# emdgroup/baybe

Measured on AMD Instinct MI355X. Metric: acquisition candidates scored/sec (1e6 discrete grid, n_train=512, qLogEI), higher is better.
Workload: dtype f64; 1 GPU; 1000000 x 20 discrete grid per GPU, n_train=512, Matern-5/2 ARD, qLogEI S=512, fixed-theta, top-8 to host; global_rows=1000000, parallelism=row-shard x1, collective=none

## Files before the change

### baybe_amd/_lib.py

```python

from __future__ import annotations

import ctypes as C
import os
from pathlib import Path

_LIB_NAME = "libbaybe_hip.so"
_lib = None

c_double_p = C.POINTER(C.c_double)
c_int64_p = C.POINTER(C.c_int64)


class HipUnavailableError(RuntimeError):
    """The HIP extension (or a HIP device) is not available; nothing else can run the path."""


class HipError(RuntimeError):
    """A libbaybe_hip call failed."""


class ModelDesc(C.Structure):

    _fields_ = [
# ... 33 lines not shown
    "bbh_create": (C.c_int, [C.c_int, C.POINTER(C.c_void_p)]),
    "bbh_destroy": (C.c_int, [C.c_void_p]),
    "bbh_last_error": (C.c_char_p, [C.c_void_p]),
    "bbh_set_stream": (C.c_int, [C.c_void_p, C.c_void_p]),
    "bbh_version": (C.c_int, []),
    "bbh_selftest": (C.c_int, [C.c_void_p]),
    "bbh_set_rff_weights": (C.c_int, [C.c_void_p, C.POINTER(C.c_double), C.c_int32, C.c_int32]),
    "bbh_set_model": (
        C.c_int,
        [C.c_void_p, C.POINTER(ModelDesc), C.c_int64, c_double_p, c_double_p, c_double_p, c_double_p],
    ),
    "bbh_set_model_ex": (
        C.c_int,
        [C.c_void_p, C.POINTER(ModelDesc), C.c_int64, c_double_p, c_double_p, c_double_p, c_double_p,
         C.POINTER(C.c_uint8), C.c_int, C.c_double, C.c_double],
    ),
    "bbh_set_slice_rows": (C.c_int, [C.c_void_p, C.c_int64]),
    "bbh_trim": (C.c_int, [C.c_void_p, C.c_int64]),
    "bbh_theta_len": (C.c_int64, [C.c_void_p]),
    "bbh_get_standardization": (C.c_int, [C.c_void_p, c_double_p, c_double_p]),
    "bbh_fit_value_grad": (C.c_int, [C.c_void_p, c_double_p, c_double_p, c_double_p]),
    "bbh_factorize": (C.c_int, [C.c_void_p, c_double_p, c_double_p]),
    "bbh_posterior": (C.c_int, [C.c_void_p, C.c_void_p, C.c_int64, C.c_int64, C.c_void_p, C.c_void_p]),
    "bbh_posterior_unfused": (C.c_int, [C.c_void_p, C.c_void_p, C.c_int64, C.c_int64, C.c_void_p, C.c_void_p]),
    "bbh_posterior_joint": (C.c_int, [C.c_void_p, c_double_p, C.c_int64, c_double_p, c_double_p]),
    "bbh_set_mean_columns": (C.c_int, [C.c_void_p, c_double_p, C.c_int64]),
    "bbh_posterior_columns": (C.c_int, [C.c_void_p, C.c_void_p, C.c_int64, C.c_int64, C.c_void_p]),
    "bbh_posterior_columns_sm": (C.c_int, [C.c_void_p, C.c_void_p, C.c_int64, C.c_int64, C.c_void_p]),
    "bbh_train_posterior_mean": (C.c_int, [C.c_void_p, c_double_p]),
    "bbh_qlogei_q1": (
        C.c_int,
        [C.c_void_p, C.c_void_p, C.c_void_p, C.c_int64, c_double_p, C.c_int64, C.c_double, C.c_double,
         C.c_void_p, C.c_void_p],
    ),
    "bbh_qlogei_q1_topk": (
        C.c_int,
        [C.c_void_p, C.c_void_p, C.c_void_p, C.c_int64, c_double_p, C.c_int64, C.c_double, C.c_double,
         C.c_void_p, C.c_void_p, C.c_int64, c_double_p, c_int64_p],
    ),
    "bbh_score_qlogei": (
        C.c_int,
        [C.c_void_p, C.c_void_p, C.c_int64, C.c_int64, c_double_p, C.c_int64, C.c_double, C.c_double, C.c_void_p,
         C.c_void_p, C.c_void_p, C.c_void_p],
    ),
    "bbh_pending_set": (C.c_int, [C.c_void_p, c_double_p, C.c_int64, c_double_p, c_double_p]),
    "bbh_cross_cov": (C.c_int, [C.c_void_p, C.c_void_p, C.c_int64, C.c_int64, C.c_void_p]),
    "bbh_qlogei_pending": (
        C.c_int,
        [C.c_void_p, C.c_void_p, C.c_void_p, C.c_void_p, C.c_int64, c_double_p, C.c_int64, C.c_double,
         C.c_double, C.c_void_p, C.c_void_p],
    ),
    "bbh_qlognehvi": (
        C.c_int,
        [C.c_void_p, C.c_int32, C.c_int64, C.POINTER(C.c_void_p), C.POINTER(C.c_void_p), c_double_p, c_double_p,
         C.c_int64, c_int64_p, c_double_p, c_double_p, C.c_void_p, C.c_void_p],
    ),
    "bbh_qlognehvi_sm": (
        C.c_int,
        [C.c_void_p, C.c_int32, C.c_int64, C.POINTER(C.c_void_p), C.POINTER(C.c_void_p), c_double_p, c_double_p,
         C.c_int64, c_int64_p, c_double_p, c_double_p, C.c_void_p, C.c_void_p],
    ),
    "bbh_qlogei_pending_big": (
        C.c_int,
        [C.c_void_p, C.c_void_p, C.c_void_p, C.c_void_p, C.c_int64, C.c_int64, c_double_p, c_double_p, c_double_p, C.c_int64,
         C.c_double, C.c_double, C.c_void_p, C.c_void_p],
    ),
    "bbh_mc_acq_q1": (
        C.c_int,
        [C.c_void_p, C.c_int32, C.c_void_p, C.c_void_p, C.c_int64, c_double_p, C.c_int64, C.c_double, C.c_double,
         C.c_double, C.c_void_p, C.c_void_p],
    ),
    "bbh_mc_acq_pending": (
        C.c_int,
        [C.c_void_p, C.c_int32, C.c_void_p, C.c_void_p, C.c_void_p, C.c_int64, c_double_p, C.c_int64, C.c_double,
         C.c_double, C.c_double, C.c_void_p, C.c_void_p],
    ),
    "bbh_mc_acq_obj_q1": (
        C.c_int,
        [C.c_void_p, C.c_int32, C.POINTER(ObjectiveProg), C.c_void_p, C.c_void_p, C.c_int64, c_double_p, C.c_int64, C.c_double,
         C.c_double, C.c_void_p, C.c_void_p],
    ),
    "bbh_mc_acq_obj_pending": (
        C.c_int,
        [C.c_void_p, C.c_int32, C.POINTER(ObjectiveProg), C.c_void_p, C.c_void_p, C.c_void_p, C.c_int64, C.c_int64, c_double_p,
         c_double_p, c_double_p, C.c_int64, C.c_double, C.c_double, C.c_void_p, C.c_void_p],
    ),
    "bbh_analytic_acq": (
        C.c_int,
        [C.c_void_p, C.c_int32, C.c_void_p, C.c_void_p, C.c_int64, C.c_double, C.c_double, C.c_double, C.c_int32,
         C.c_void_p, C.c_void_p],
    ),
    "bbh_pareto_frequency": (C.c_int, [C.c_void_p, c_double_p, C.c_int64, C.c_int64, C.c_int32, c_double_p, c_int64_p]),
    "bbh_pareto_frequency_dev": (C.c_int, [C.c_void_p, C.c_void_p, C.c_int64, C.c_int64, C.c_int32, c_double_p, c_int64_p]),
    "bbh_best_frequency_dev": (C.c_int, [C.c_void_p, C.c_void_p, C.c_int64, C.c_int64, c_int64_p]),
    "bbh_sample_best_dev": (C.c_int, [C.c_void_p, C.c_void_p, C.c_int64, C.c_int64, C.c_void_p]),
    "bbh_nei_q1": (C.c_int, [C.c_void_p, C.c_int32, C.c_void_p, C.c_void_p, C.c_int64, c_double_p, C.c_int64, C.c_void_p, C.c_double,
                             C.c_void_p, C.c_void_p]),
    "bbh_score_nei": (C.c_int, [C.c_void_p, C.c_int32, C.c_void_p, C.c_int64, C.c_int64, C.c_void_p, c_double_p, C.c_int64, C.c_void_p,
                                C.c_double, C.c_void_p, C.c_void_p]),
    "bbh_scalarized_best_dev": (C.c_int, [C.c_void_p, C.c_void_p, C.c_int64, C.c_int64, C.c_int32, c_double_p, c_double_p, c_double_p,
                                          C.c_void_p]),
    "bbh_scalarized_best_frequency_dev": (C.c_int, [C.c_void_p, C.c_void_p, C.c_int64, C.c_int64, C.c_int32, c_double_p, c_double_p,
                                                    c_double_p, c_int64_p]),
    "bbh_nparego_q1": (
        C.c_int,
        [C.c_void_p, C.c_int32, C.c_int64, C.POINTER(C.c_void_p), C.POINTER(C.c_void_p), c_double_p, C.c_void_p, C.c_int64,
         c_double_p, c_double_p, c_double_p, C.c_void_p, C.c_void_p, C.c_void_p],
    ),
    "bbh_qnehvi_cells": (
        C.c_int,
        [C.c_void_p, C.c_int32, C.c_int64, C.POINTER(C.c_void_p), C.POINTER(C.c_void_p), c_double_p, c_double_p,
         C.c_int64, C.c_void_p, C.c_void_p],
    ),
    "bbh_qnehvi_sm": (
        C.c_int,
        [C.c_void_p, C.c_int32, C.c_int64, C.POINTER(C.c_void_p), C.POINTER(C.c_void_p), c_double_p, c_double_p,
         C.c_int64, c_int64_p, c_double_p, c_double_p, C.c_void_p, C.c_void_p],
    ),
    "bbh_nehvi_samples": (C.c_int, [C.c_void_p, c_double_p, C.c_int64, C.c_int64, C.c_double, C.c_int32, C.c_int32, C.c_void_p, C.c_int32]),
    "bbh_nehvi_samples_dev": (C.c_int, [C.c_void_p, C.c_void_p, C.c_int64, C.c_void_p, C.c_int64, C.c_int64, C.c_double, C.c_int32, C.c_int32,
                                        C.c_void_p, C.c_int32]),
    "bbh_cells_build_dev": (C.c_int, [C.c_void_p, C.c_void_p, C.c_int64, C.c_int64, C.c_int32, c_double_p, c_int64_p, c_int64_p]),
    "bbh_cells_read_dev": (C.c_int, [C.c_void_p, c_int64_p, c_double_p, c_double_p]),
    "bbh_qlognehvi_cells": (
        C.c_int,
        [C.c_void_p, C.c_int32, C.c_int64, C.POINTER(C.c_void_p), C.POINTER(C.c_void_p), c_double_p, c_double_p,
         C.c_int64, C.c_void_p, C.c_void_p],
    ),
    "bbh_cells_create": (C.c_int, [c_double_p, C.c_int64, C.c_int64, C.c_int32, c_double_p, C.POINTER(C.c_void_p), c_int64_p]),
    "bbh_cells_get": (C.c_int, [C.c_void_p, c_int64_p, c_double_p, c_double_p]),
    "bbh_cells_destroy": (C.c_int, [C.c_void_p]),
    "bbh_sobol_scramble": (C.c_int, [c_int64_p, c_int64_p, C.c_int64]),
    "bbh_sobol_draw": (C.c_int, [c_int64_p, c_int64_p, C.c_int64, C.c_int64, c_double_p]),
    "bbh_sobol_normal": (C.c_int, [c_int64_p, C.c_uint64, C.c_int64, C.c_int64, c_double_p]),
    "bbh_sobol_normal_dev": (C.c_int, [C.c_void_p, c_int64_p, C.c_uint64, C.c_int64, C.c_int64, C.c_void_p]),
    "bbh_content_key": (C.c_uint64, [C.POINTER(C.c_void_p), c_int64_p, C.c_int32, C.c_int32]),
    "bbh_argmax": (C.c_int, [C.c_void_p, C.c_void_p, C.c_int64, c_double_p, c_int64_p]),
    "bbh_topk": (C.c_int, [C.c_void_p, C.c_void_p, C.c_int64, C.c_int64, c_double_p, c_int64_p]),
    "bbh_fps_prepare": (C.c_int, [C.c_void_p, C.c_void_p, C.c_int64, C.c_int32, C.c_int64, c_double_p, c_double_p, C.c_void_p, C.c_int64,
                                  C.c_void_p, C.c_int64]),
    "bbh_fps_farthest_pair": (C.c_int, [C.c_void_p, C.c_void_p, C.c_int64, C.c_int32, C.c_int64, C.c_void_p, c_double_p, c_int64_p,
                                        c_int64_p]),
    "bbh_fps_greedy": (C.c_int, [C.c_void_p, C.c_void_p, C.c_int64, C.c_int32, C.c_int64, C.c_void_p, c_int64_p, C.c_int64, C.c_int64,
                                 C.c_int64, c_int64_p, c_double_p, c_int64_p]),
    "bbh_comm_unique_id": (C.c_int, [C.c_void_p, C.c_int64]),
    "bbh_comm_init": (C.c_int, [C.c_void_p, C.c_int32, C.c_int32, C.c_void_p, C.c_int64]),
    "bbh_comm_destroy": (C.c_int, [C.c_void_p]),
    "bbh_allgather_topk": (C.c_int, [C.c_void_p, C.c_void_p, C.c_int64, C.c_int64, C.c_int64, c_double_p, c_int64_p]),
    "bbh_allgather_argmax": (
        C.c_int,
        [C.c_void_p, C.c_void_p, C.c_int64, C.c_int64, C.c_void_p, C.c_int64, c_double_p, c_int64_p, c_double_p],
    ),
    "bbh_last_posterior_form": (C.c_int, [C.c_void_p]),
    "bbh_last_nei_form": (C.c_int, [C.c_void_p]),
    "bbh_last_fit_form": (C.c_int, [C.c_void_p]),
    "bbh_timing_enable": (C.c_int, [C.c_void_p, C.c_int]),
    "bbh_timing_read": (C.c_int, [C.c_void_p, c_double_p, c_int64_p, C.c_int]),
    "bbh_timing_read_family": (C.c_int, [C.c_void_p, C.c_int32, c_double_p, c_int64_p, C.c_int]),
    "bbh_flow_trace_read": (C.c_int, [C.c_void_p, C.c_void_p, C.c_void_p, C.c_int]),
    "bbh_tiles_trace_read": (C.c_int, [C.c_void_p, C.c_void_p, C.c_int]),
}


def library_path() -> Path:
    env = os.environ.get("BAYBE_AMD_LIB")
    return Path(env) if env else Path(__file__).resolve().parent / _LIB_NAME


def load_library():
    global _lib
    if _lib is not None:
        return _lib
    import torch

    path = library_path()
    if not path.exists():
        raise HipUnavailableError(
            f"{path} not found: build it with `python -c 'import __graft_entry__ as g; g.build()'` "
            f"or `make -C baybe_amd/csrc`. There is no CPU fallback for this path."
        )
    try:
        lib = C.CDLL(str(path))
    except OSError as ex:
        raise HipUnavailableError(f"cannot load {path}: {ex}") from ex
    for name, (restype, argtypes) in SIGNATURES.items():
        fn = getattr(lib, name)
        fn.restype = restype
        fn.argtypes = argtypes
    _lib = lib
    return lib


def is_available() -> bool:
    try:
        lib = load_library()
    except (HipUnavailableError, AttributeError):
        return False
    h = C.c_void_p()
    rc = lib.bbh_create(0, C.byref(h))
    if rc != 0:
        return False
    lib.bbh_destroy(h)
    return True
```

### baybe_amd/csrc/bbh_api.hip

```cpp
#include <math.h>
#include <stdlib.h>
#include <string.h>

#include <algorithm>
#include <map>
#include <mutex>

#include "bbh_common.h"

static const char* kNoHandle = "bbh: null handle";

extern "C" int bbh_version(void) { return 100; }

static bbh_switches bbh_read_switches() {
  enum how { NOT, IS, SET, INT, MB };
  typedef bbh_switches S;
  static const struct {
    const char* name;
    how parse;
    char c;
    bool S::*flag;
    int S::*num;
  } table[] = {
      {"BBH_PIPELINE", NOT, '0', &S::use_pipeline, nullptr},
      {"BBH_MEAN_VALU", NOT, '0', &S::use_mean_valu, nullptr},
      {"BBH_KVCACHE", NOT, '0', &S::use_kvcache, nullptr},
      {"BBH_KV_GLOBAL", NOT, '0', nullptr, &S::kv_global_mode},
      {"BBH_KV_LDS", INT, 0, nullptr, &S::kv_lds_blocks},
      {"BBH_COOP", INT, 0, nullptr, &S::coop_mode},
      {"BBH_COOP_SMALL", NOT, '0', &S::coop_small, nullptr},
      {"BBH_COOPG_CROSS", NOT, '0', &S::coopg_cross_on, nullptr},
      {"BBH_SMALL", NOT, '0', &S::small_on, nullptr},
      {"BBH_SMALL_FORCE", IS, '1', &S::small_force, nullptr},
      {"BBH_COLUMNS_COOP", NOT, '0', &S::columns_coop, nullptr},
      {"BBH_COLUMNS_NT", INT, 0, nullptr, &S::columns_nt},
      {"BBH_PENDING_LDS", NOT, '0', &S::pending_lds_form, nullptr},
      {"BBH_PENDING_SLICES", INT, 0, nullptr, &S::pending_slices},
      {"BBH_QBIG_WS_MB", MB, 0, nullptr, &S::qbig_ws_mb},
      {"BBH_Q1_SLICED", NOT, '0', &S::q1_sliced, nullptr},
      {"BBH_NEHVI_LOG", IS, '1', &S::nehvi_log, nullptr},
      {"BBH_NEHVI_SLICES", INT, 0, nullptr, &S::nehvi_slices},
      {"BBH_NEHVI_PK", NOT, '0', &S::nehvi_pk, nullptr},
      {"BBH_NEI_FUSED", NOT, '0', &S::nei_fused, nullptr},
      {"BBH_SELECT", NOT, '0', &S::select_on, nullptr},
      {"BBH_SELECT_MAPPED", NOT, '0', &S::select_mapped, nullptr},
      {"BBH_FIT_GRAPH", NOT, '0', &S::fit_graph_mode, nullptr},
      {"BBH_FIT_OVERLAP", NOT, '0', &S::fit_overlap, nullptr},
      {"BBH_FIT_SMALL", NOT, '0', &S::fit_small, nullptr},
      {"BBH_FIT_FLOW", INT, 0, nullptr, &S::fit_flow},
      {"BBH_FLOW_SPIN", INT, 0, nullptr, &S::flow_spin_limit},
      {"BBH_FIT_POST1", NOT, '0', &S::fit_post1, nullptr},
      {"BBH_FIT_TAIL1", NOT, '0', &S::fit_tail1, nullptr},
      {"BBH_POTRF_TILES", NOT, '0', &S::potrf_tiles, nullptr},
      {"BBH_POTRF_REG", NOT, '0', &S::potrf_register_form, nullptr},
      {"BBH_TILE_SPIN", INT, 0, nullptr, &S::tile_spin_limit},
      {"BBH_TILE_ACQ", IS, '0', &S::tile_d_sc1, nullptr},
      {"BBH_TILE_WT", NOT, '0', &S::tile_wt, nullptr},
      {"BBH_TILE_MT", NOT, '0', &S::tile_mt, nullptr},
      {"BBH_TILE_MT", IS, 'p', &S::tile_mt_partial, nullptr},
      {"BBH_TILE_GRAM", NOT, '0', &S::tile_gram, nullptr},
      {"BBH_TILE_GRAM_THETA", IS, 'c', &S::tile_gram_theta_copy, nullptr},
      {"BBH_SETMODEL_UPLOAD", IS, 'c', &S::setmodel_upload_copy, nullptr},
      {"BBH_SETMODEL_SYNC", NOT, '0', &S::setmodel_sync, nullptr},
      {"BBH_SETMODEL_SYNC", IS, 'p', &S::setmodel_sync_poll, nullptr},
      {"BBH_SETMODEL_TRACE", SET, 0, &S::setmodel_trace, nullptr},
      {"BBH_SETMODEL_TRACE", IS, '2', &S::setmodel_trace_quiet, nullptr},
      {"BBH_FIT_TRACE", SET, 0, &S::fit_trace, nullptr},
      {"BBH_TILE_TRACE", SET, 0, &S::tile_trace, nullptr},
      {"BBH_FLOW_TRACE", SET, 0, &S::flow_trace, nullptr},
      {"BBH_TILE_STAMPS", SET, 0, &S::tile_stamps, nullptr},
  };
  bbh_switches sw;
  for (const auto& row : table) {
    const char* e = getenv(row.name);
    if (!e) continue;
    long long v = 1;
    if (row.parse == NOT) v = e[0] != row.c;
    if (row.parse == IS) v = e[0] == row.c;
    if (row.parse == INT) v = atoi(e);
    if (row.parse == MB) v = std::min<long long>(std::max(1LL, atoll(e)), INT_MAX);
    if (row.flag) sw.*row.flag = v != 0;
    if (row.num) sw.*row.num = (int)v;
  }
  return sw;
}

hipError_t bbh_allow_lds(int device, const void* kernel, size_t bytes) {
  if (bytes <= BBH_LDS_DEFAULT_LIMIT) return hipSuccess;
  hipError_t e = device < 0 ? hipGetDevice(&device) : hipSuccess;
  if (e != hipSuccess) return e;
  static std::mutex mu;
  static std::map<std::pair<const void*, int>, size_t> granted;
  std::lock_guard<std::mutex> lock(mu);
  size_t& have = granted[{kernel, device}];
  if (bytes <= have) return hipSuccess;
  e = hipFuncSetAttribute(kernel, hipFuncAttributeMaxDynamicSharedMemorySize, (int)bytes);
  if (e == hipSuccess) have = bytes;
  return e;
}

extern "C" int bbh_create(int device_id, bbh_handle** out) {
  if (!out) return -1;
  *out = nullptr;
  int count = 0;
  if (hipGetDeviceCount(&count) != hipSuccess || count <= 0) return -10;
  if (device_id < 0 || device_id >= count) return -11;
  if (hipSetDevice(device_id) != hipSuccess) return -12;
  bbh_handle* h = new bbh_handle();
  h->device = device_id;
  {
    int cus = 0;
    if (hipDeviceGetAttribute(&cus, hipDeviceAttributeMultiprocessorCount, device_id) == hipSuccess && cus > 0) h->num_cu = cus;
  }
  {
    int v = 0;
    if (hipDeviceGetAttribute(&v, hipDeviceAttributeMaxSharedMemoryPerBlock, device_id) == hipSuccess && v > 0) h->lds_per_block = (size_t)v;
  }
  h->sw = bbh_read_switches();
  *out = h;
  return 0;
}

extern "C" int bbh_destroy(bbh_handle* h) {
  if (!h) return -1;
  hipSetDevice(h->device);
  if (h->stream)
    hipStreamSynchronize(h->stream);
  else
    hipDeviceSynchronize();
  for (auto& sp : h->pending_events) {
    hipEventDestroy(sp.e0);
    hipEventDestroy(sp.e1);
  }
  bbh_comm_destroy(h);
  bbh_select_destroy(h);
  bbh_nehvi_destroy(h);
  bbh_sobol_destroy(h);
  bbh_fps_destroy(h);
  bbh_flow_destroy(h);
  bbh_free_model_public(h);
  if (h->d_ws) hipFree(h->d_ws);
  if (h->fit_stream) {
    hipStreamSynchronize(h->fit_stream);
    hipStreamDestroy(h->fit_stream);
  }
  if (h->side_stream) {
    hipStreamSynchronize(h->side_stream);
    hipStreamDestroy(h->side_stream);
  }
  for (auto& e : h->side_events)
    if (e) hipEventDestroy(e);
  if (h->d_rstream) hipFree(h->d_rstream);
  if (h->d_rsmall) hipFree(h->d_rsmall);
  if (h->d_tileflags) hipFree(h->d_tileflags);
  if (h->d_kvcache) hipFree(h->d_kvcache);
  if (h->d_slab_flags) hipFree(h->d_slab_flags);
  if (h->d_z) hipFree(h->d_z);
  if (h->h_zstage) hipHostFree(h->h_zstage);
  if (h->z_evt) hipEventDestroy(h->z_evt);
  if (h->d_red) hipFree(h->d_red);
  if (h->d_redi) hipFree(h->d_redi);
  delete h;
  return 0;
}

extern "C" const char* bbh_last_error(bbh_handle* h) { return h ? h->err.c_str() : kNoHandle; }

extern "C" int bbh_set_stream(bbh_handle* h, void* hip_stream) {
  if (!h) return -1;
  h->stream = (hipStream_t)hip_stream;
  return 0;
}

__global__ void bbh_selftest_kernel(const double* A, const double* B, double* C) {
  const int l = threadIdx.x;
  d4 acc = {0.0, 0.0, 0.0, 0.0};
  for (int ks = 0; ks < 2; ks++) {
    const double a = A[(l & 15) * 8 + 4 * ks + (l >> 4)];
    const double b = B[(4 * ks + (l >> 4)) * 16 + (l & 15)];
    acc = mfma_f64(a, b, acc);
  }
  for (int r = 0; r < 4; r++) C[((l >> 4) + 4 * r) * 16 + (l & 15)] = acc[r];
}

extern "C" int bbh_selftest(bbh_handle* h) {
  if (!h) return -1;
  BBH_HIP_TRY(h, hipSetDevice(h->device));
  double hA[16 * 8], hB[8 * 16], hC[256], ref[256];
  for (int i = 0; i < 16; i++)
    for (int k = 0; k < 8; k++) hA[i * 8 + k] = (double)(3 * i + 7 * k + 1) - 0.5 * (double)(i * k);
  for (int k = 0; k < 8; k++)
    for (int j = 0; j < 16; j++) hB[k * 16 + j] = (double)(5 * k - 2 * j) + 0.25 * (double)(k * j + j);
  for (int i = 0; i < 16; i++)
    for (int j = 0; j < 16; j++) {
      double s = 0.0;
      for (int k = 0; k < 8; k++) s += hA[i * 8 + k] * hB[k * 16 + j];
      ref[i * 16 + j] = s;
    }
  int rc = bbh_ensure_ws(h, sizeof(double) * 1024);
  if (rc) return rc;
  double* dA = h->d_ws;
  double* dB = dA + 128;
  double* dC = dB + 128;
  BBH_HIP_TRY(h, hipMemcpyAsync(dA, hA, sizeof(hA), hipMemcpyHostToDevice, h->stream));
  BBH_HIP_TRY(h, hipMemcpyAsync(dB, hB, sizeof(hB), hipMemcpyHostToDevice, h->stream));
  hipLaunchKernelGGL(bbh_selftest_kernel, dim3(1), dim3(64), 0, h->stream, dA, dB, dC);
  BBH_HIP_TRY(h, hipMemcpyAsync(hC, dC, sizeof(hC), hipMemcpyDeviceToHost, h->stream));
  BBH_HIP_TRY(h, hipStreamSynchronize(h->stream));
  for (int e = 0; e < 256; e++)
    if (fabs(hC[e] - ref[e]) > 1e-9 * (1.0 + fabs(ref[e]))) {
      h->err = "bbh_selftest: v_mfma_f64_16x16x4_f64 fragment layout mismatch at element " + std::to_string(e);
      return -20;
    }
  return 0;
}

static int check_post_args(bbh_handle* h, const double* X_dev, int64_t N, int64_t ldx) {
  if (!h->factorized) {
    h->err = "posterior requested before bbh_factorize";
    return -1;
  }
  if (N < 0 || (N > 0 && !X_dev) || ldx < h->desc.d) {
    h->err = "posterior: bad arguments (need ldx >= d)";
    return -1;
  }
  if (h->dn > 126) {
    h->err = "fused posterior supports at most 126 numerical columns";
    return -1;
  }
  return 0;
}

extern "C" int bbh_posterior(bbh_handle* h, const double* X_dev, int64_t N, int64_t ldx, double* mean_dev,
                             double* var_dev) {
  if (!h) return -1;
  int rc = check_post_args(h, X_dev, N, ldx);
  if (rc) return rc;
  BBH_HIP_TRY(h, hipSetDevice(h->device));
  return bbh_launch_fused(h, X_dev, N, ldx, mean_dev, var_dev, nullptr, true);
}

extern "C" int bbh_posterior_unfused(bbh_handle* h, const double* X_dev, int64_t N, int64_t ldx, double* mean_dev,
                                     double* var_dev) {
  if (!h) return -1;
  int rc = check_post_args(h, X_dev, N, ldx);
  if (rc) return rc;
  BBH_HIP_TRY(h, hipSetDevice(h->device));
  return bbh_launch_unfused(h, X_dev, N, ldx, mean_dev, var_dev);
}

extern "C" int bbh_cross_cov(bbh_handle* h, const double* X_dev, int64_t N, int64_t ldx, double* cross_dev) {
  if (!h) return -1;
  int rc = check_post_args(h, X_dev, N, ldx);
  if (rc) return rc;
  if (h->p < 1 || !cross_dev) {
    h->err = "bbh_cross_cov: no pending points set";
    return -1;
  }
  BBH_HIP_TRY(h, hipSetDevice(h->device));
  return bbh_launch_fused(h, X_dev, N, ldx, nullptr, nullptr, cross_dev, false);
}

extern "C" int bbh_train_posterior_mean(bbh_handle* h, double* mean_host) {
  if (!h) return -1;
  if (!h->factorized || !mean_host) {
    h->err = "bbh_train_posterior_mean: model not factorised";
    return -1;
  }
  BBH_HIP_TRY(h, hipSetDevice(h->device));
  const int64_t n = h->n, d = h->desc.d;
  int rc = 0;
  double* own = nullptr;
  if (bbh_materialised_only(h))
    BBH_HIP_TRY(h, hipMalloc((void**)&own, sizeof(double) * (size_t)(n * d + n)));
  else if ((rc = bbh_ensure_ws(h, sizeof(double) * (size_t)(n * d + n))))
    return rc;
  double* dX = own ? own : h->d_ws;
  double* dm = dX + n * d;
  hipError_t e = hipMemcpyAsync(dX, h->xraw_host.data(), sizeof(double) * n * d, hipMemcpyHostToDevice, h->stream);
  if (e == hipSuccess) rc = bbh_launch_fused(h, dX, n, d, dm, nullptr, nullptr, false);
  if (e == hipSuccess && !rc) e = hipMemcpyAsync(mean_host, dm, sizeof(double) * n, hipMemcpyDeviceToHost, h->stream);
  if (e == hipSuccess) e = hipStreamSynchronize(h->stream);
  if (own) hipFree(own);
  if (rc) return rc;
  BBH_HIP_TRY(h, e);
  return 0;
}

extern "C" int bbh_set_slice_rows(bbh_handle* h, int64_t rows) {
  if (!h || rows < 0) return -1;
  h->slice_rows = rows;
  return 0;
}

extern "C" int bbh_trim(bbh_handle* h, int64_t keep_bytes) {
  if (!h || keep_bytes < 0) return -1;
  BBH_HIP_TRY(h, hipSetDevice(h->device));
  BBH_HIP_TRY(h, hipStreamSynchronize(h->stream));
  bbh_fps_reset(h);
  if (h->d_ws && h->ws_bytes > (size_t)keep_bytes) {
    hipFree(h->d_ws);
    h->d_ws = nullptr;
    h->ws_bytes = 0;
  }
  if (h->d_kvcache && h->kvcache_bytes > (size_t)keep_bytes) {
    hipFree(h->d_kvcache);
    h->d_kvcache = nullptr;
    h->kvcache_bytes = 0;
  }
  if (h->have_model && sizeof(double) * (size_t)h->np * (size_t)h->np * 6 > (size_t)keep_bytes) bbh_free_model_public(h);
  return 0;
}

extern "C" int bbh_last_posterior_form(bbh_handle* h) { return h ? h->last_form : -1; }
extern "C" int bbh_last_fit_form(bbh_handle* h) { return h ? h->last_fit_form : -1; }

extern "C" int bbh_timing_enable(bbh_handle* h, int enable) {
  if (!h) return -1;
  h->timing = enable < 0 ? 0 : enable;
  return 0;
}

extern "C" int bbh_timing_read_family(bbh_handle* h, int32_t family, double* ms_total, int64_t* launches, int reset) {
  if (!h) return -1;
  if (family < 0 || family >= BBH_TIMED_FAMILIES) {
    h->err = "bbh_timing_read_family: unknown kernel family";
    return -1;
  }
  BBH_HIP_TRY(h, hipSetDevice(h->device));
  for (auto& sp : h->pending_events) {
    BBH_HIP_TRY(h, hipEventSynchronize(sp.e1));
    float ms = 0.f;
    BBH_HIP_TRY(h, hipEventElapsedTime(&ms, sp.e0, sp.e1));
    h->timed_ms[sp.family] += (double)ms;
    h->timed_launches[sp.family] += 1;
    hipEventDestroy(sp.e0);
    hipEventDestroy(sp.e1);
  }
  h->pending_events.clear();
  if (ms_total) *ms_total = h->timed_ms[family];
  if (launches) *launches = h->timed_launches[family];
  if (reset) {
    h->timed_ms[family] = 0.0;
    h->timed_launches[family] = 0;
  }
  return 0;
}

extern "C" int bbh_timing_read(bbh_handle* h, double* fused_ms_total, int64_t* fused_launches, int reset) {
  return bbh_timing_read_family(h, BBH_TIMED_POSTERIOR, fused_ms_total, fused_launches, reset);
}
```

### baybe_amd/csrc/bbh_common.h

```cpp
#pragma once

#include <hip/hip_runtime.h>
#include <limits.h>
#include <stdint.h>

#include <string>
#include <vector>

#include "../../include/baybe_hip.h"

typedef double d4 __attribute__((ext_vector_type(4)));

#define BBH_WAVE 64
#define BBH_TB 16
#define BBH_PAD 64
#define BBH_MEANCOLS 16
#define BBH_SQRT3 1.7320508075688772
#define BBH_SQRT5 2.23606797749979

__device__ __forceinline__ d4 mfma_f64(double a, double b, d4 c) {
  return __builtin_amdgcn_mfma_f64_16x16x4f64(a, b, c, 0, 0, 0);
}

#define BBH_HIP_TRY(h, expr)                                                              \
  do {                                                                                    \
    hipError_t _e = (expr);                                                               \
    if (_e != hipSuccess) {                                                               \
      (h)->err = std::string(#expr) + ": " + hipGetErrorString(_e);                       \
      return -2;                                                                          \
    }                                                                                     \
  } while (0)

#define BBH_MAX_FACTORS 4
struct bbh_kern_spec {
  int F;
  int combine;
  int grp[BBH_MAX_FACTORS];
  int kind[BBH_MAX_FACTORS];
  int ls_off[BBH_MAX_FACTORS];
  int fos_off;
  int use_os;
  int jb;
  int alpha_off;
  int per_off;
};
__host__ __device__ inline double bbh_powi(double x, int n) {
  double acc = 1.0;
  for (int i = 0; i < n; i++) acc *= x;
  return acc;
}
__host__ __device__ inline double bbh_piecewise(int q, int jb, double r2, bool want_g) {
  const double r = sqrt(r2 > 1e-30 ? r2 : 1e-30);
  if (!(r < 1.0)) return 0.0;
  const double j = (double)(jb + q), u = 1.0 - r;
  if (!want_g) {
    double P = 1.0;
    if (q == 1) P = fma(j + 1.0, r, 1.0);
    if (q == 2) P = fma(fma((j * j + 4.0 * j + 3.0) / 3.0, r, j + 2.0), r, 1.0);
    if (q == 3)
      P = fma(fma(fma((j * j * j + 9.0 * j * j + 23.0 * j + 15.0) / 15.0, r, (6.0 * j * j + 36.0 * j + 45.0) / 15.0), r, j + 3.0), r, 1.0);
    return bbh_powi(u, jb + 2 * q) * P;
  }
  const double m = bbh_powi(u, jb + 2 * q - 1);
  if (q == 0) return r2 > 1e-30 ? j * m / r : 0.0;
  if (q == 1) return (j + 1.0) * (j + 2.0) * m;
  if (q == 2) return (j + 3.0) * (j + 4.0) * fma(j + 1.0, r, 1.0) / 3.0 * m;
  return (j + 5.0) * (j + 6.0) * fma(fma(j * j + 4.0 * j + 3.0, r, 3.0 * j + 6.0), r, 3.0) / 15.0 * m;
}
#define BBH_KIND_IS_DOT(kind) ((kind) >= BBH_KERNEL_LINEAR && (kind) <= BBH_KERNEL_POLY4)
#define BBH_KIND_IS_POLY(kind) ((kind) >= BBH_KERNEL_POLY1 && (kind) <= BBH_KERNEL_POLY4)
#define BBH_KIND_HAS_ALPHA(kind) ((kind) == BBH_KERNEL_RQ || BBH_KIND_IS_POLY(kind))
__host__ __device__ __forceinline__ double bbh_metric_term(int kind, double xa, double xb, double invw) {
  if (BBH_KIND_IS_DOT(kind)) return (xa * invw) * (xb * invw);
  const double df = (xa - xb) * invw;
  return df * df;
}
__host__ __device__ __forceinline__ double bbh_metric_term_f(const bbh_kern_spec& ks, const double* theta, int f, int j, int dn,
                                                             double xa, double xb, double invw) {
  if (ks.kind[f] == BBH_KERNEL_PERIODIC) {
    const double sn = sin(M_PI * (xa - xb) / theta[ks.per_off + f * dn + j]);
    return sn * sn * invw;
  }
  return bbh_metric_term(ks.kind[f], xa, xb, invw);
}
__host__ __device__ __attribute__((noinline)) inline double bbh_kbase(int kind, double r2, int jb, double alpha = 1.0) {
  if (kind == BBH_KERNEL_LINEAR) return r2;
  if (BBH_KIND_IS_POLY(kind)) return bbh_powi(r2 + alpha, kind - BBH_KERNEL_POLY1 + 1);
  if (kind == BBH_KERNEL_PERIODIC) return exp(-2.0 * r2);
  if (kind == BBH_KERNEL_RBF) return exp(-0.5 * r2);
  if (kind == BBH_KERNEL_RQ) return exp(-alpha * log1p(r2 / (2.0 * alpha)));
  if (kind >= BBH_KERNEL_PIECEWISE0 && kind <= BBH_KERNEL_PIECEWISE3) return bbh_piecewise(kind - BBH_KERNEL_PIECEWISE0, jb, r2, false);
  const double r = sqrt(r2);
  if (kind == BBH_KERNEL_MATERN52) return (1.0 + BBH_SQRT5 * r + (5.0 / 3.0) * r2) * exp(-BBH_SQRT5 * r);
  if (kind == BBH_KERNEL_MATERN32) return (1.0 + BBH_SQRT3 * r) * exp(-BBH_SQRT3 * r);
  return exp(-r);
}
__device__ __forceinline__ double bbh_gfun(int kind, double r2, int jb, double alpha) {
  if (kind == BBH_KERNEL_LINEAR) return -2.0;
  if (BBH_KIND_IS_POLY(kind)) return -2.0 * (double)(kind - BBH_KERNEL_POLY1 + 1) * bbh_powi(r2 + alpha, kind - BBH_KERNEL_POLY1);
  if (kind == BBH_KERNEL_PERIODIC) return 2.0 * exp(-2.0 * r2);
  if (kind == BBH_KERNEL_RBF) return exp(-0.5 * r2);
  if (kind == BBH_KERNEL_RQ) return exp(-(alpha + 1.0) * log1p(r2 / (2.0 * alpha)));
  if (kind >= BBH_KERNEL_PIECEWISE0) return bbh_piecewise(kind - BBH_KERNEL_PIECEWISE0, jb, r2, true);
  const double r = sqrt(r2);
  if (kind == BBH_KERNEL_MATERN52) return (5.0 / 3.0) * (1.0 + BBH_SQRT5 * r) * exp(-BBH_SQRT5 * r);
  if (kind == BBH_KERNEL_MATERN32) return 3.0 * exp(-BBH_SQRT3 * r);
  return r > 0.0 ? exp(-r) / r : 0.0;
}


template <class GRP>
__host__ __device__ __forceinline__ double bbh_combine(int F, int combine, const GRP& grp, const double* u) {
  if (combine == 0) {
    double acc = 1.0;
#pragma unroll
    for (int f = 0; f < BBH_MAX_FACTORS; f++)
      if (f < F) acc *= u[f];
    return acc;
  }
  if (combine == 1) {
    double acc = 0.0;
#pragma unroll
    for (int f = 0; f < BBH_MAX_FACTORS; f++)
      if (f < F) acc += u[f];
    return acc;
  }
  double acc = 0.0;
#pragma unroll
  for (int g = 0; g < BBH_MAX_FACTORS; g++) {
    double term = 1.0;
    bool used = false;
#pragma unroll
    for (int f = 0; f < BBH_MAX_FACTORS; f++)
      if (f < F && grp[f] == g) {
        term *= u[f];
        used = true;
      }
    if (used) acc += term;
  }
  return acc;
}
template <class GRP>
__host__ __device__ __forceinline__ double bbh_combine_weight(int F, int combine, const GRP& grp, const double* u, int f) {
  if (combine == 1) return 1.0;
  double w = 1.0;
#pragma unroll
  for (int g = 0; g < BBH_MAX_FACTORS; g++)
    if (g < F && g != f && (combine == 0 || grp[g] == grp[f])) w *= u[g];
  return w;
}
__device__ __forceinline__ double bbh_kcomp(const bbh_kern_spec& ks, const double* __restrict__ theta,
                                            const double (&r2)[BBH_MAX_FACTORS]) {
  if (ks.F <= 1) return bbh_kbase(ks.kind[0], r2[0], ks.jb, ks.alpha_off >= 0 ? theta[ks.alpha_off] : 1.0);
  double u[BBH_MAX_FACTORS] = {1.0, 1.0, 1.0, 1.0};
#pragma unroll
  for (int f = 0; f < BBH_MAX_FACTORS; f++)
    if (f < ks.F)
      u[f] = theta[ks.fos_off + f] * bbh_kbase(ks.kind[f], r2[f], ks.jb, ks.alpha_off >= 0 ? theta[ks.alpha_off + f] : 1.0);
  return bbh_combine(ks.F, ks.combine, ks.grp, u);
}

struct bbh_switches {
  bool use_pipeline = true;
  bool use_mean_valu = true;
  bool use_kvcache = true;
  int kv_global_mode = -1;
  int kv_lds_blocks = -1;
  int coop_mode = 1;
  bool coop_small = true;
  bool coopg_cross_on = true;
  bool small_on = true;
  bool small_force = false;
  bool columns_coop = true;
  int columns_nt = 2;
  bool pending_lds_form = false;
  int pending_slices = INT_MIN;
  int qbig_ws_mb = 0;
  bool q1_sliced = true;
  bool nehvi_log = false;
  int nehvi_slices = INT_MIN;
  bool nehvi_pk = true;
  bool nei_fused = true;
  bool select_on = true;
  bool select_mapped = true;
  bool fit_graph_mode = false;
  bool fit_overlap = true;
  bool fit_small = true;
  int fit_flow = 1;
  int flow_spin_limit = 1 << 17;
  bool fit_post1 = true;
  bool fit_tail1 = true;
  bool potrf_tiles = true;
  bool potrf_register_form = false;
  int tile_spin_limit = 1 << 17;
  bool tile_d_sc1 = false;
  bool tile_wt = true;
  bool tile_mt = true;
  bool tile_mt_partial = false;
  bool tile_gram = true;
  bool tile_gram_theta_copy = false;
  bool setmodel_upload_copy = false;
  bool setmodel_sync = true;
  bool setmodel_sync_poll = false;
  bool setmodel_trace = false;
  bool setmodel_trace_quiet = false;
  bool fit_trace = false;
  bool tile_trace = false;
  bool flow_trace = false;
  bool tile_stamps = false;
};

struct bbh_handle {
  int device = 0;
  bbh_switches sw;
  hipStream_t stream = nullptr;
  std::string err;

  bbh_model_desc desc{};
  std::string model_sig;
  bool have_model = false;
  bool factorized = false;
  int64_t n = 0;
  int64_t np = 0;
  int64_t nb = 0;
  int dn = 0;
  int kd = 0;
  int T = 1;
  bool hadamard = false;
  int F = 1;
  std::vector<int> numcol;
  std::vector<double> lo, hi;
  double ybar = 0.0, ysd = 1.0;
  std::vector<double> theta;
  std::vector<double> ystd_host;
  std::vector<double> xn_host;
  std::vector<int> task_host;
  std::vector<double> xcenter;

  double* d_xnT = nullptr;
  int* d_task = nullptr;
  double* d_nmask = nullptr;
  double* d_pendT = nullptr;
  double* d_colA = nullptr;
  int64_t colA_elems = 0;
  std::vector<double> nmask_host;
  double* d_ystd = nullptr;
  double* d_theta = nullptr;
  double* d_K = nullptr;
  double* d_X = nullptr;
  double* d_M = nullptr;
  double* d_Mpart = nullptr;
  double* d_Q = nullptr;
  double* d_Q2 = nullptr;
  double* d_D = nullptr;
  double* d_tmp = nullptr;
  double* d_r = nullptr;
  double* d_t = nullptr;
  double* d_alpha = nullptr;
  double* d_u = nullptr;
  double* d_w = nullptr;
  double* d_q = nullptr;
  double* d_partial = nullptr;
  double* d_out = nullptr;
  int* d_info = nullptr;
  double* d_trainfrag = nullptr;
  double* d_rfrag = nullptr;
  double* d_meanB = nullptr;
  double* d_sclofs = nullptr;
  int* d_numcol = nullptr;
  double* d_tasktbl = nullptr;
  int* d_taskext = nullptr;
  int64_t rfrag_elems = 0;
  int64_t* d_pass_off = nullptr;
  int* d_pass_w = nullptr;
  int npass = 0;
  int pass_w_last = 0;
  double* d_kvcache = nullptr;
  size_t kvcache_bytes = 0;
  int* d_slab_flags = nullptr;
  size_t lds_per_block = 65536;
  int num_cu = 256;
  int wmax = 16;
  hipStream_t side_stream = nullptr;
  hipStream_t fit_stream = nullptr;
  bool fit_small_ready = false, fit_small_failed = false;
  bool tiles_ready = false, tiles_gave_up = false;
  int tile_spin_limit_set = -1;
  int tiles_per_device = 0;
  int* d_tileflags = nullptr;
  int tile_epoch = 0;
  hipGraphExec_t fit_exec = nullptr;
  bool fit_graph_failed = false;
  double *pin_theta = nullptr, *pin_out = nullptr;
  int* pin_info = nullptr;
  hipEvent_t side_events[2] = {nullptr, nullptr};
  bool coop_ready = false;
  bool coopg_ready = false;
  double* d_trainfrag_f = nullptr;
  double* d_sclofs_f = nullptr;
  int64_t tf_f_elems = 0;
  bool coop2_ready = false;
  double* d_rstream = nullptr;
  int64_t rstream_frags = 0;
  int coop_g0 = 0;
  int last_form = -1;
  int last_fit_form = -1;
  int last_nei_form = -1;
  int64_t nb_ext = 0;
  int p = 0;
  std::vector<double> pend_host;
  std::vector<double> pend_mean;
  std::vector<double> pend_cov;
  std::vector<double> xraw_host;
  double* d_beta = nullptr;
  double* d_colfrag = nullptr;
  int64_t colfrag_elems = 0;
  int64_t ncols = 0;
  const double* fuse_qz = nullptr;
  int fuse_S = 0;
  double fuse_best_f = 0.0, fuse_sign = 1.0;
  const uint8_t* fuse_alive = nullptr;
  double* fuse_scores = nullptr;
  double* d_ws = nullptr;
  size_t ws_bytes = 0;
  double* d_z = nullptr;
  size_t z_bytes = 0;
  double* h_zstage = nullptr;
  size_t zstage_bytes = 0;
  hipEvent_t z_evt = nullptr;
  double* d_red = nullptr;
  int64_t* d_redi = nullptr;
  void* comm_state = nullptr;
  double* d_rsmall = nullptr;
  int small_nb = 0;
  int64_t slice_rows = 0;
  void* flow_state = nullptr;
  bool flow_gave_up = false;
  bool skip_x_memset = false;
  bool flow_in_flight = false;
  long long* d_tiledbg = nullptr;
  int tiledbg_n = 0;
  int tiles_did_mt = 0;
  int tiles_mt_asked = 0;
  bool potrf_tiles_ran = false;
  bool info_clean = false;
  void* rff_state = nullptr;
  std::vector<double> rff_w_host;
  int rff_w_dn = 0, rff_w_D = 0;
  void* nehvi_state = nullptr;
  void* select_state = nullptr;
  void* sobol_state = nullptr;
  void* fps_state = nullptr;
  int timing = 0;
  hipEvent_t ev0 = nullptr, ev1 = nullptr;
  double timed_ms[BBH_TIMED_FAMILIES] = {};
  int64_t timed_launches[BBH_TIMED_FAMILIES] = {};
  struct TimedSpan {
    hipEvent_t e0, e1;
    int family;
  };
  std::vector<TimedSpan> pending_events;
};

struct bbh_timed_scope {
  bbh_handle* h;
  hipEvent_t e0 = nullptr, e1 = nullptr;
  int family;
  bbh_timed_scope(bbh_handle* h_, int family_, bool wanted = true) : h(h_), family(family_) {
    if ((h->timing == 1 || ((h->timing >> 1) >> family_ & 1)) && wanted) {
      hipEventCreate(&e0);
      hipEventCreate(&e1);
      hipEventRecord(e0, h->stream);
    }
  }
  ~bbh_timed_scope() {
    if (e0) {
      hipEventRecord(e1, h->stream);
      h->pending_events.push_back({e0, e1, family});
    }
  }
};

inline int64_t bbh_round_up(int64_t x, int64_t m) { return (x + m - 1) / m * m; }

#define BBH_LDS_DEFAULT_LIMIT ((size_t)48 * 1024)
__attribute__((visibility("hidden"))) hipError_t bbh_allow_lds(int device, const void* kernel, size_t bytes);

struct bbh_nehvi_state {
  int64_t S = 0, total = 0, cap = 0;
  int m = 0;
  double* d_slots = nullptr;
  size_t slot_bytes = 0;
  double* d_pack = nullptr;
  size_t pack_bytes = 0;
  int* d_cnt = nullptr;
  int64_t cnt_cap = 0;
  double* d_ref = nullptr;
  int64_t* h_status = nullptr;
  const int64_t* off() const { return (const int64_t*)d_pack; }
  const double* lo() const { return d_pack + (S + 1); }
  const double* ll() const { return lo() + S * cap * m; }
  const double* len() const { return ll() + S * cap * m; }
};

void bbh_gemm(hipStream_t s, bool transA, bool transB, int64_t M, int64_t N, int64_t K, double alpha,
              const double* A, int64_t lda, int64_t strideA, const double* B, int64_t ldb,
              int64_t strideB, double beta, double* C, int64_t ldc, int64_t strideC, int batch);
void bbh_potrf_trtri(bbh_handle* h);
bool bbh_potrf_trtri_from_inputs(bbh_handle* h, const double* theta_any, const double* theta_host, const void* mt_args = nullptr);
void bbh_potrf_tiles_mark_unusable(int device);
void bbh_ensure_side_stream(bbh_handle* h);
void bbh_matvec(hipStream_t s, const double* A, int64_t lda, int64_t rows, int64_t cols,
                const double* x, double* y);
void bbh_matvec_t(hipStream_t s, const double* A, int64_t lda, int64_t rows, int64_t cols,
                  const double* x, double* y);

int bbh_upload_theta(bbh_handle* h, const double* theta_host);
void bbh_launch_gram(bbh_handle* h, double jitter, double jitter_latent);
bool bbh_fit_small_launch(bbh_handle* h, double jitter, const double* theta_dev, double* out_dev, int* info_dev);
bbh_kern_spec bbh_kern_spec_of(const bbh_handle* h);
int bbh_hadamard_offset(const bbh_handle* h);
double bbh_prior_base(const bbh_handle* h);
bool bbh_materialised_only(const bbh_handle* h);
bool bbh_has_dot_kind(const bbh_handle* h);
int bbh_launch_unfused_ext(bbh_handle* h, const double* X_dev, int64_t N, int64_t ldx, double* mean_dev, double* var_dev,
                           double* cross_dev);

int bbh_pack_operands(bbh_handle* h);
int bbh_launch_fused(bbh_handle* h, const double* X_dev, int64_t N, int64_t ldx, double* mean_dev,
                     double* var_dev, double* cross_dev, bool with_var);
int bbh_launch_unfused(bbh_handle* h, const double* X_dev, int64_t N, int64_t ldx, double* mean_dev,
                       double* var_dev);

int bbh_ensure_ws(bbh_handle* h, size_t bytes);
void* bbh_stage_pinned(bbh_handle* h, size_t bytes);
int bbh_stage_done(bbh_handle* h);
int bbh_upload_z(bbh_handle* h, const double* z_host, size_t count);
void bbh_select_destroy(bbh_handle* h);
void bbh_nehvi_destroy(bbh_handle* h);
void bbh_sobol_destroy(bbh_handle* h);
void bbh_fps_destroy(bbh_handle* h);
void bbh_fps_reset(bbh_handle* h);
void bbh_flow_destroy(bbh_handle* h);
bool bbh_fit_flow_launch(bbh_handle* h, const double* theta_dev, double* out_dev, int* info_dev, bool tail_only, const double* theta_host = nullptr,
                         bool split = false, int skip_mt = 0, bool prepare_only = false);
bool bbh_fit_flow_mt_args(bbh_handle* h, void* pd_mt_args_out);
bool bbh_fit_flow_eligible(bbh_handle* h);
void bbh_fit_flow_reset(bbh_handle* h);
void bbh_free_model_public(bbh_handle* h);
inline bool bbh_is_rff(const bbh_handle* h) { return h->desc.kernel_kind == BBH_KERNEL_RFF; }
int bbh_rff_setup(bbh_handle* h);
int bbh_rff_fit_enqueue(bbh_handle* h);
int bbh_rff_factorize(bbh_handle* h);
int bbh_rff_posterior_launch(bbh_handle* h, const double* X_dev, int64_t N, int64_t ldx, double* mean_dev, double* var_dev, double* cross_dev);
int bbh_rff_pending_set(bbh_handle* h, const double* Xpend_host, int64_t p, double* mean_p_host, double* cov_pp_host);
int bbh_rff_posterior_joint(bbh_handle* h, const double* Xq_host, int64_t q, double* mean_host, double* cov_host);
void bbh_rff_destroy(bbh_handle* h);
// ... 1 lines not shown
```

### baybe_amd/csrc/bbh_coop.h

```cpp
#pragma once
#define BBH_CANDREG 1
#include "bbh_fused.h"

#define BBH_COOP_ROUNDS 8
#define BBH_COOP_KV_TILE (2 * 4 * 256)
#ifndef BBH_COOP_WAVES
#define BBH_COOP_WAVES 2
#endif
#ifndef BBH_COOP_PAIRS
#define BBH_COOP_PAIRS 4
#endif
#ifndef BBH_COOP_ABLATE_BARRIER
#define BBH_COOP_ABLATE_BARRIER 0
#endif
#ifndef BBH_COOP_ABLATE_MEM
#define BBH_COOP_ABLATE_MEM 0
#endif
#ifndef BBH_COOP_ABLATE_PRO
#define BBH_COOP_ABLATE_PRO 0
#endif
#ifndef BBH_COOP_ABLATE_LOADS
#define BBH_COOP_ABLATE_LOADS 0
#endif
#ifndef BBH_COOP_ABLATE_CHAIN
#define BBH_COOP_ABLATE_CHAIN 0
#endif
#ifndef BBH_COOP_ABLATE_KV
#define BBH_COOP_ABLATE_KV 0
#endif

typedef double d2 __attribute__((ext_vector_type(2)));
template <int IMM>
__device__ __forceinline__ void coop_gload2(d2& dst, const double* sbase, unsigned voff) {
  static_assert(IMM >= 0 && IMM + 16 <= 4096, "13-bit signed immediate offset");
  asm volatile("global_load_dwordx4 %0, %1, %2 offset:%3" : "=v"(dst) : "v"(voff), "s"(sbase), "n"(IMM));
}
template <int N>
__device__ __forceinline__ void coop_vmwait2(d2& slot) {
  asm volatile("s_waitcnt vmcnt(%1)" : "+v"(slot) : "n"(N));
}
template <int IMM>
__device__ __forceinline__ void coop_gload(double& dst, const double* sbase, unsigned voff) {
  static_assert(IMM >= 0 && IMM < 4096, "13-bit signed immediate offset");
  asm volatile("global_load_dwordx2 %0, %1, %2 offset:%3" : "=v"(dst) : "v"(voff), "s"(sbase), "n"(IMM));
}
template <int N>
__device__ __forceinline__ void coop_vmwait(double& slot) {
  asm volatile("s_waitcnt vmcnt(%1)" : "+v"(slot) : "n"(N));
}

struct CoopArgs {
  FusedArgs f;
  const double* rstream;
  int64_t frags;
  int g0;
};

__host__ __device__ constexpr int coop_frags_before(int G) { return 16 * (G * BBH_COOP_ROUNDS - (G * (G - 1)) / 2); }

template <int G, int KD, int KVF, bool PRODUCE, int NT, bool OPEN = false>
__device__ __forceinline__ void coop_group(const WaveCtx (&c)[NT], const double* rs, const double* tfn, const bbh_lds_double* kv_cur,
                                           bbh_lds_double* kv_mine_next, const bbh_lds_double* alpha_next, int tbn, int cw,
                                           d4 (&acc)[NT][BBH_COOP_ROUNDS], d2 (&ring)[BBH_COOP_PAIRS], double (&accm)[NT]) {
  constexpr int NP = BBH_COOP_PAIRS;
  constexpr int CNT = BBH_COOP_ROUNDS - G;
  constexpr int FULL = CNT - 1;
  constexpr int TOT = 16 * CNT;
  constexpr int REM = OPEN ? (1 << 20) : coop_frags_before(BBH_COOP_ROUNDS) - coop_frags_before(G + 1);
  constexpr int HOSTS = 12 * FULL;
  constexpr int STEPS = NT * BBH_KV_STEPS;
  const unsigned lane8 = (unsigned)c[0].l * 8u, lane16 = (unsigned)c[0].l * 16u;
  double tfv[KD];
  d4 dsa[NT], dsb[NT];
  KvState<BBH_KV_NU> P;
  double kv[NT][4], kvx[NT][4], kvn[NT][4], alv[4];
  if constexpr (PRODUCE) {
    static_for<0, KD>([&](auto kc) __attribute__((always_inline)) {
      constexpr int k = decltype(kc)::value;
      coop_gload<(k % 8) * 512>(tfv[k], tfn + (k / 8) * 512, lane8);
    });
  }
#pragma unroll
  for (int t = 0; t < NT; t++)
#pragma unroll
    for (int r = 0; r < 4; r++) kv[t][r] = kv_cur[t * BBH_COOP_KV_TILE + r * 64];
  __builtin_amdgcn_sched_barrier(0);
  static_for<0, 4>([&](auto ic) __attribute__((always_inline)) {
    constexpr int i = decltype(ic)::value;
    if constexpr (i < 3) {
#pragma unroll
      for (int t = 0; t < NT; t++)
#pragma unroll
        for (int r = 0; r < 4; r++) kvx[t][r] = kv_cur[t * BBH_COOP_KV_TILE + (i + 1) * 256 + r * 64];
    } else if constexpr (PRODUCE) {
#pragma unroll
      for (int r = 0; r < 4; r++) alv[r] = alpha_next[4 * r];
    }
    static_for<0, 4>([&](auto rc) __attribute__((always_inline)) {
      constexpr int r = decltype(rc)::value;
      static_for<0, CNT>([&](auto sc) __attribute__((always_inline)) {
        constexpr int s = decltype(sc)::value;
        constexpr int f = (i * 4 + r) * CNT + s;
        constexpr int pr = f / 2;
        if constexpr (f % 2 == 0 && !BBH_COOP_ABLATE_LOADS) {
          constexpr int BEHIND = ((TOT + REM) / 2 - 1 - pr) < (NP - 1) ? ((TOT + REM) / 2 - 1 - pr) : (NP - 1);
          coop_vmwait2<BEHIND + ((PRODUCE && pr < NP) ? KD : 0)>(ring[pr % NP]);
        }
#if BBH_COOP_ABLATE_CHAIN
        static_for<0, NT>([&](auto tc_) __attribute__((always_inline)) {
          constexpr int t = decltype(tc_)::value;
          if constexpr (s == 0) {
            if (cw >= i) acc[t][f % 8] = mfma_f64(kv[t][r], ring[pr % NP][f % 2], acc[t][f % 8]);
          } else {
            acc[t][f % 8] = mfma_f64(kv[t][r], ring[pr % NP][f % 2], acc[t][f % 8]);
          }
        });
#else
        static_for<0, NT>([&](auto tc_) __attribute__((always_inline)) {
          constexpr int t = decltype(tc_)::value;
          if constexpr (s == 0) {
            if (cw >= i) acc[t][G] = mfma_f64(kv[t][r], ring[pr % NP][f % 2], acc[t][G]);
          } else {
            acc[t][G + s] = mfma_f64(kv[t][r], ring[pr % NP][f % 2], acc[t][G + s]);
          }
        });
#endif
        if constexpr (f % 2 == 1 && 2 * (pr + NP) < TOT + REM && !BBH_COOP_ABLATE_LOADS) {
          constexpr int np = pr + NP;
          coop_gload2<(np % 4) * 1024>(ring[pr % NP], BBH_COOP_ABLATE_MEM ? rs : rs + (np / 4) * 512, lane16);
        }
        if constexpr (PRODUCE && i >= 1 && s >= 1 && !BBH_COOP_ABLATE_KV) {
          constexpr int m = ((i - 1) * 4 + r) * FULL + (s - 1);
          static_for<(m * STEPS) / HOSTS, ((m + 1) * STEPS) / HOSTS>([&](auto st) __attribute__((always_inline)) {
            constexpr int tile = decltype(st)::value / BBH_KV_STEPS, micro = decltype(st)::value % BBH_KV_STEPS;
            kv_micro<KVF, BBH_KV_NU, micro>(P, c[tile], tbn, 0, dsa[tile], dsb[tile], kvn[tile]);
          });
        }
        __builtin_amdgcn_sched_barrier(0);
      });
      if constexpr (PRODUCE && i == 0 && r == 3) {
        coop_vmwait<NP>(tfv[KD - 1]);
        __builtin_amdgcn_sched_barrier(0);
        if constexpr (!BBH_COOP_ABLATE_KV) {
          static_for<0, NT>([&](auto tc_) __attribute__((always_inline)) {
            constexpr int t = decltype(tc_)::value;
            kvp_dist<KD>(c[t], tfv, dsa[t], dsb[t]);
          });
        }
      }
    });
    if constexpr (i < 3) {
#pragma unroll
      for (int t = 0; t < NT; t++)
#pragma unroll
        for (int r = 0; r < 4; r++) kv[t][r] = kvx[t][r];
    }
  });
  if constexpr (PRODUCE) {
#pragma unroll
    for (int t = 0; t < NT; t++)
#pragma unroll
      for (int r = 0; r < 4; r++) {
        if constexpr (BBH_COOP_ABLATE_KV) kvn[t][r] = tfv[r];
        kv_mine_next[t * BBH_COOP_KV_TILE + r * 64] = kvn[t][r];
        accm[t] = fma(kvn[t][r], alv[r], accm[t]);
      }
  }
}

template <int KD, int KVF, int NT, int GMIN = 0>
__global__ __launch_bounds__(256, (GMIN >= 6 ? 5 : GMIN >= 4 ? 4 : BBH_COOP_WAVES)) void bbh_coop_posterior_kernel(const CoopArgs ca) {
  const FusedArgs& a = ca.f;
  extern __shared__ __attribute__((aligned(16))) double s_mem[];
  const int l = threadIdx.x & 63, w = __builtin_amdgcn_readfirstlane(threadIdx.x >> 6);
  const int cnd = l & 15, q = l >> 4;
  double* s_alpha = s_mem;
  double* s_kv = s_alpha + 16 * a.nb;
  double* s_red = s_kv + NT * BBH_COOP_KV_TILE;
  const int64_t tile0 = (int64_t)blockIdx.x * (16 * NT);

  WaveCtx c[NT];
  int tcs[NT];
  int xcol[KD];
  double xval[NT][KD], xscl[KD], xofs[KD];
  const double* xr[NT];
  double tfv0[KD];
  kvp_load<KD>(a.trainfrag + l, w, tfv0);
#pragma unroll
  for (int t = 0; t < NT; t++) {
    const int64_t row = (tile0 + 16 * t + cnd < a.N) ? tile0 + 16 * t + cnd : a.N - 1;
    xr[t] = a.X + row * a.ldx;
  }
  if (a.numcol_identity) {
#pragma unroll
    for (int k = 0; k < KD; k++) xcol[k] = (4 * k + q < a.dn) ? 4 * k + q : a.dn - 1;
  } else {
#pragma unroll
    for (int k = 0; k < KD; k++) xcol[k] = a.numcol[(4 * k + q < a.dn) ? 4 * k + q : a.dn - 1];
  }
#pragma unroll
  for (int k = 0; k < KD; k++) {
    const int dimc = (4 * k + q < a.dn) ? 4 * k + q : a.dn - 1;
#pragma unroll
    for (int t = 0; t < NT; t++) xval[t][k] = xr[t][xcol[k]];
    xscl[k] = a.scl[dimc];
    xofs[k] = a.ofs[dimc];
  }
  if (!(BBH_COOP_ABLATE_PRO & 1))
    for (int s = threadIdx.x; s < 16 * a.nb; s += 256) s_alpha[s] = a.meanB[(int64_t)s * 16];
#pragma unroll
  for (int t = 0; t < NT; t++) {
    double nbsum = 0.0;
#pragma unroll
    for (int k = 0; k < KD; k++) {
      const int dim = 4 * k + q;
      double v = 0.0;
      if (dim < a.dn) {
        v = (BBH_COOP_ABLATE_PRO & 2) ? 0.01 * (double)(dim + cnd) : fma(xval[t][k], xscl[k], xofs[k]);
        nbsum = fma(v, v, nbsum);
      }
      c[t].cf[k] = v;
    }
    nbsum += __shfl_xor(nbsum, 16, 64);
    nbsum += __shfl_xor(nbsum, 32, 64);
#pragma unroll
    for (int k = 0; k < KD; k++) {
      if (4 * k + q == a.dn) c[t].cf[k] = 1.0;
      if (4 * k + q == a.dn + 1) c[t].cf[k] = nbsum;
    }
    int tc = 0;
    if constexpr ((KVF & 1) != 0) {
      if (a.task_col >= 0) {
        tc = (int)xr[t][a.task_col];
        tc = tc < 0 ? 0 : (tc >= a.T ? a.T - 1 : tc);
      }
    }
    tcs[t] = tc;
    c[t].tf = a.trainfrag + l;
    c[t].candl = nullptr;
    c[t].mb = nullptr;
    c[t].tbl = a.tasktbl;
    c[t].taskext = a.taskext;
    c[t].kvc = nullptr;
    c[t].kvl = (bbh_lds_double*)nullptr;
    c[t].nl = 0;
    c[t].ncache = 0;
    c[t].al = (const bbh_lds_double*)nullptr;
    c[t].kd = KD;
    c[t].kind = a.kind;
    c[t].T = a.T;
    c[t].tc = tc;
    c[t].q = q;
    c[t].l = l;
    c[t].dn = a.dn;
  }

  bbh_lds_double* kvb = (bbh_lds_double*)(s_kv + l);
  const bbh_lds_double* alq = (const bbh_lds_double*)(s_alpha + q);
  const int g0 = ca.g0;
  double accm[NT];
  d4 acc[NT][BBH_COOP_ROUNDS];
#pragma unroll
  for (int t = 0; t < NT; t++) {
    accm[t] = 0.0;
#pragma unroll
    for (int s = 0; s < BBH_COOP_ROUNDS; s++) acc[t][s] = (d4){0.0, 0.0, 0.0, 0.0};
  }
  const double* rs = ca.rstream + (int64_t)w * ca.frags * 64;
  d2 ring[BBH_COOP_PAIRS];
  static_for<0, BBH_COOP_PAIRS>([&](auto ic) __attribute__((always_inline)) {
    constexpr int i = decltype(ic)::value;
    coop_gload2<(i % 4) * 1024>(ring[i], rs + (i / 4) * 512, (unsigned)l * 16u);
  });
  {
    double tfv[KD], kv0[NT][4];
    if constexpr (BBH_COOP_ABLATE_PRO & 4) {
      for (int t = 0; t < NT; t++)
        for (int r = 0; r < 4; r++) kv0[t][r] = 0.5 + 0.001 * (double)(l + r);
    } else {
#pragma unroll
      for (int k = 0; k < KD; k++) tfv[k] = tfv0[k];
#pragma unroll
      for (int t = 0; t < NT; t++) {
        d4 dsa, dsb;
        kvp_dist<KD>(c[t], tfv, dsa, dsb);
        kv_all<KVF>(c[t], w, dsa, dsb, kv0[t]);
      }
    }
    __syncthreads();
#pragma unroll
    for (int t = 0; t < NT; t++)
#pragma unroll
      for (int r = 0; r < 4; r++) {
        kvb[t * BBH_COOP_KV_TILE + ((g0 & 1) * 4 + w) * 256 + r * 64] = kv0[t][r];
        accm[t] = fma(kv0[t][r], alq[16 * w + 4 * r], accm[t]);
      }
  }
  __syncthreads();

  static_for<GMIN, BBH_COOP_ROUNDS>([&](auto gc) __attribute__((always_inline)) {
    constexpr int G = decltype(gc)::value;
    if (G >= g0) {
      const int cw = (G & 1) ? 3 - w : w;
      const int tbn = 4 * (G + 1 - g0) + w;
      constexpr bool PRODUCE = G + 1 < BBH_COOP_ROUNDS;
      coop_group<G, KD, KVF, PRODUCE, NT>(c, rs, a.trainfrag + (int64_t)tbn * KD * 64, kvb + (G & 1) * 4 * 256,
                                          kvb + (((G + 1) & 1) * 4 + w) * 256, alq + 16 * tbn, tbn, cw, acc, ring, accm);
      rs += (int64_t)16 * (BBH_COOP_ROUNDS - G) * 64;
#if !BBH_COOP_ABLATE_BARRIER
      if constexpr (PRODUCE) __syncthreads();
#endif
    }
  });

  if constexpr (BBH_COOP_ABLATE_PRO & 8) {
    double keep = 0.0;
#pragma unroll
    for (int t = 0; t < NT; t++) {
      keep += accm[t];
#pragma unroll
      for (int s = 0; s < BBH_COOP_ROUNDS; s++) keep += (acc[t][s][0] + acc[t][s][1]) + (acc[t][s][2] + acc[t][s][3]);
    }
    if (l == 0 && w == 0) a.var[tile0] = keep;
    return;
  }
#pragma unroll
  for (int t = 0; t < NT; t++) {
    double ss[4] = {0.0, 0.0, 0.0, 0.0};
#pragma unroll
    for (int s = 0; s < BBH_COOP_ROUNDS; s++)
#pragma unroll
      for (int r = 0; r < 4; r++) ss[r] = fma(acc[t][s][r], acc[t][s][r], ss[r]);
#pragma unroll
    for (int r = 0; r < 4; r++) {
      double v = ss[r];
      v += __shfl_xor(v, 1, 64);
      v += __shfl_xor(v, 2, 64);
      v += __shfl_xor(v, 4, 64);
      v += __shfl_xor(v, 8, 64);
      ss[r] = v;
    }
    double mp = accm[t];
    mp += __shfl_xor(mp, 16, 64);
    mp += __shfl_xor(mp, 32, 64);
    double* red_v = s_red + t * 128;
    double* red_m = red_v + 64;
    if (cnd == 0) {
#pragma unroll
      for (int r = 0; r < 4; r++) red_v[w * 16 + q + 4 * r] = ss[r];
    }
    if (q == 0) red_m[w * 16 + cnd] = mp;
  }
  __syncthreads();
  if (threadIdx.x < 16 * NT) {
    const int m = threadIdx.x & 15, t = threadIdx.x >> 4;
    const int64_t gi = tile0 + 16 * t + m;
    const double* red_v = s_red + t * 128;
    const double* red_m = red_v + 64;
    const double sv = (red_v[m] + red_v[16 + m]) + (red_v[32 + m] + red_v[48 + m]);
    const double sm = (red_m[m] + red_m[16 + m]) + (red_m[32 + m] + red_m[48 + m]);
    double pv = a.prior_scale, mc = a.mean_const;
    if constexpr ((KVF & 1) != 0) {
      int tcm = __shfl(tcs[0], m, 64);
      if constexpr (NT > 1) {
        const int tcm1 = __shfl(tcs[NT - 1], m, 64);
        tcm = t ? tcm1 : tcm;
      }
      pv = a.tasktbl[tcm * a.T + tcm];
      if (a.taskmean) mc = a.taskmean[tcm];
    }
    if (gi < a.N) {
      if (a.mean) a.mean[gi] = a.ybar + a.ysd * (mc + sm);
      if (a.var) a.var[gi] = a.ysd * a.ysd * (pv - sv);
    }
  }
}

bool bbh_coop_launch(int kd, int kind, bool has_tbl, dim3 grid, size_t lds, hipStream_t s, const CoopArgs& a, bool small_ok);
bool bbh_coop_launch_a(int kd, int kind, bool has_tbl, dim3 grid, size_t lds, hipStream_t s, const CoopArgs& a);
bool bbh_coop_launch_b(int kd, int kind, bool has_tbl, dim3 grid, size_t lds, hipStream_t s, const CoopArgs& a);
bool bbh_coop_launch_small(int kd, int kind, bool has_tbl, dim3 grid, size_t lds, hipStream_t s, const CoopArgs& a);

#define BBH_COOP_DISPATCH_KD(KDV, NTV)                                                                                        \
  if (kd == KDV) {                                                                                                       \
    const bool m52 = kind == BBH_KERNEL_MATERN52, rbf = kind == BBH_KERNEL_RBF, plain = kind == BBH_KERNEL_MATERN32 && !has_tbl; \
    if (!m52 && !rbf && !plain) return false;                                                                            \
    if (grid.x == 0) return true;                                                                                        \
    if (rbf && has_tbl)                                                       \
      hipLaunchKernelGGL((bbh_coop_posterior_kernel<KDV, 3, NTV>), grid, dim3(256), lds, s, a);                               \
    else if (rbf)                                                                                                        \
      hipLaunchKernelGGL((bbh_coop_posterior_kernel<KDV, 2, NTV>), grid, dim3(256), lds, s, a);                               \
    else if (kind == BBH_KERNEL_MATERN32)                                                                                \
      hipLaunchKernelGGL((bbh_coop_posterior_kernel<KDV, 4, NTV>), grid, dim3(256), lds, s, a);                               \
    else if (has_tbl)                                                                                                    \
      hipLaunchKernelGGL((bbh_coop_posterior_kernel<KDV, 1, NTV>), grid, dim3(256), lds, s, a);                               \
    else                                                                                                                 \
      hipLaunchKernelGGL((bbh_coop_posterior_kernel<KDV, 0, NTV>), grid, dim3(256), lds, s, a);                               \
    return true;                                                                                                         \
  }
```

### baybe_amd/csrc/bbh_fused.h

```cpp
#pragma once
#include <math.h>
#include <string.h>

#include <type_traits>

#include "bbh_common.h"

#define BBH_MAX_PASS 64
#ifndef BBH_W32_REMAINDERS
#define BBH_W32_REMAINDERS 0
#endif

__device__ __forceinline__ double bbh_kfun_p(int kind, double r2) {
  if (kind == BBH_KERNEL_RBF) return exp(-0.5 * r2);
  const double r = sqrt(r2);
  if (kind == BBH_KERNEL_MATERN52) return (1.0 + BBH_SQRT5 * r + (5.0 / 3.0) * r2) * exp(-BBH_SQRT5 * r);
  if (kind == BBH_KERNEL_MATERN32) return (1.0 + BBH_SQRT3 * r) * exp(-BBH_SQRT3 * r);
  return exp(-r);
}

struct FusedArgs {
  const double* X;
  int64_t N, ldx;
  const double* trainfrag;
  const double* rfrag;
  const double* meanB;
  const double* scl;
  const double* ofs;
  const int* numcol;
  const double* tasktbl;
  const double* taskmean;
  const int* taskext;
  double* mean;
  double* var;
  double* cross;
  const int64_t* pass_off;
  const int* pass_w;
  int npass;
  int kind, dn, kd, nb, nb_ext, task_col, T, p, with_var;
  double ybar, ysd, mean_const, prior_scale;
  const double* qz;
  int qS;
  double q_best_f, q_sign;
  const uint8_t* q_alive;
  double* q_scores;
  double* kvcache;
  int* slab_flags;
  int nslab, nxcc;
  int ncache;
  int64_t nblk;
  int nl;
  int has_tbl;
  int mean_valu;
  int numcol_identity;
};

typedef __attribute__((address_space(3))) double bbh_lds_double;

struct WaveCtx {
  const double* tf;
  const double* candl;
  const double* mb;
  const double* tbl;
  const int* taskext;
  double* kvc;
  bbh_lds_double* kvl;
  int nl, ncache;
  const bbh_lds_double* al;
  int kd, kind, T, tc, q, l, dn;
  double cf[16];
};

#ifndef BBH_CANDREG
#define BBH_CANDREG 0
#endif
#ifndef BBH_DIST_ASM
#define BBH_DIST_ASM 0
#endif
#ifndef BBH_MEAN_VALU_ONLY
#define BBH_MEAN_VALU_ONLY 0
#endif

template <bool HAS_TBL, int KIND>
__device__ __forceinline__ void compute_kv(const WaveCtx& c, int tb, double (&kv)[4]) {
  d4 da = {0.0, 0.0, 0.0, 0.0}, db = {0.0, 0.0, 0.0, 0.0};
  const double* tf = c.tf + (int64_t)tb * c.kd * 64;
  int k = 0;
  for (; k + 3 < c.kd; k += 4) {
    const double t0 = tf[k * 64], t1 = tf[(k + 1) * 64], t2 = tf[(k + 2) * 64], t3 = tf[(k + 3) * 64];
    const double c0 = c.candl[k * 64], c1 = c.candl[(k + 1) * 64], c2 = c.candl[(k + 2) * 64],
                 c3 = c.candl[(k + 3) * 64];
    da = mfma_f64(t0, c0, da);
    db = mfma_f64(t1, c1, db);
    da = mfma_f64(t2, c2, da);
    db = mfma_f64(t3, c3, db);
  }
  for (; k < c.kd; k++) da = mfma_f64(tf[k * 64], c.candl[k * 64], da);
#pragma unroll
  for (int r = 0; r < 4; r++) {
    const double r2 = fmax(da[r] + db[r], 0.0);
    double v;
    if (KIND == BBH_KERNEL_MATERN52) {
      const double rr = sqrt(r2);
      v = (1.0 + BBH_SQRT5 * rr + (5.0 / 3.0) * r2) * exp(-BBH_SQRT5 * rr);
    } else if (c.kind == BBH_KERNEL_MATERN12) {
      double d2 = r2;
      const bool nearp = r2 < 1e-2;
      if (__builtin_amdgcn_ballot_w64(nearp) != 0) {
        if (nearp) {
          const double* tfb = tf - c.l;
          const double* cb = c.candl - c.l;
          const int il = c.q + 4 * r, cl = c.l & 15;
          d2 = 0.0;
          for (int dim = 0; dim < c.dn; dim++) {
            const int o = (dim >> 2) * 64 + (dim & 3) * 16;
            const double df = cb[o + cl] + 0.5 * tfb[o + il];
            d2 = fma(df, df, d2);
          }
        }
      }
      v = (r2 > 1e7) ? 0.0 : exp(-sqrt(d2));
    } else {
      v = bbh_kfun_p(c.kind, r2);
    }
    if (HAS_TBL) v *= c.tbl[c.tc * c.T + c.taskext[16 * tb + 4 * r + c.q]];
    kv[r] = v;
  }
}

template <int W, int D, int TT, bool HAS_TBL, bool DO_MEAN, int KIND>
__device__ __forceinline__ void diag_steps(const WaveCtx& c, const double* rf, int j0, d4 (&acc)[W], double (&ring)[D],
                                           d4& accm) {
  if constexpr (TT < W) {
    constexpr int TOTAL = 2 * W * (W + 1);
    constexpr int BASE = 4 * (TT * W - (TT * (TT - 1)) / 2);
    constexpr int CNT = W - TT;
    double kv[4];
    double mbv[4];
    if (DO_MEAN) {
#pragma unroll
      for (int r = 0; r < 4; r++) mbv[r] = c.mb[(int64_t)(4 * (j0 + TT) + r) * 64];
    }
    compute_kv<HAS_TBL, KIND>(c, j0 + TT, kv);
    if (DO_MEAN) {
#pragma unroll
      for (int r = 0; r < 4; r++) accm = mfma_f64(kv[r], mbv[r], accm);
      __builtin_amdgcn_sched_barrier(0);
    }
#pragma unroll
    for (int r = 0; r < 4; r++)
#pragma unroll
      for (int jj = 0; jj < CNT; jj++) {
        const int i = BASE + r * CNT + jj;
        acc[TT + jj] = mfma_f64(kv[r], ring[i % D], acc[TT + jj]);
        if (i + D < TOTAL) ring[i % D] = rf[(i + D) * 64];
        if (i % D == D - 1) __builtin_amdgcn_sched_barrier(0);
      }
    diag_steps<W, D, TT + 1, HAS_TBL, DO_MEAN, KIND>(c, rf, j0, acc, ring, accm);
  }
}

template <int W, int D, bool HAS_TBL, bool DO_MEAN, int KIND>
__device__ __forceinline__ void pass_body(const WaveCtx& c, const double* rf, int j0, double (&ss)[4], d4& accm) {
  static_assert((4 * W) % D == 0 && (2 * W * (W + 1)) % D == 0, "ring depth must divide the stream");
  d4 acc[W];
#pragma unroll
  for (int jj = 0; jj < W; jj++) acc[jj] = (d4){0.0, 0.0, 0.0, 0.0};
  double ring[D];
#pragma unroll
  for (int i = 0; i < D; i++) ring[i] = rf[i * 64];
  for (int tb = 0; tb < j0; tb++) {
    double kv[4];
    double mbv[4];
    if (DO_MEAN) {
#pragma unroll
      for (int r = 0; r < 4; r++) mbv[r] = c.mb[(int64_t)(4 * tb + r) * 64];
    }
    compute_kv<HAS_TBL, KIND>(c, tb, kv);
    if (DO_MEAN) {
#pragma unroll
      for (int r = 0; r < 4; r++) accm = mfma_f64(kv[r], mbv[r], accm);
      __builtin_amdgcn_sched_barrier(0);
    }
#pragma unroll
    for (int i = 0; i < 4 * W; i++) {
      acc[i % W] = mfma_f64(kv[i / W], ring[i % D], acc[i % W]);
      ring[i % D] = rf[(i + D) * 64];
      if (i % D == D - 1) __builtin_amdgcn_sched_barrier(0);
    }
    rf += 4 * W * 64;
  }
  diag_steps<W, D, 0, HAS_TBL, DO_MEAN, KIND>(c, rf, j0, acc, ring, accm);
#pragma unroll
  for (int jj = 0; jj < W; jj++)
#pragma unroll
    for (int r = 0; r < 4; r++) ss[r] = fma(acc[jj][r], acc[jj][r], ss[r]);
}

template <int KD>
__device__ __forceinline__ void kvp_load(const double* tf_lane, int tb, double (&tfv)[KD]) {
  const double* tf = tf_lane + (int64_t)tb * KD * 64;
#pragma unroll
  for (int k = 0; k < KD; k++) tfv[k] = tf[k * 64];
}
template <int KD>
__device__ __forceinline__ void kvp_load(const WaveCtx& c, int tb, double (&tfv)[KD]) {
  kvp_load<KD>(c.tf, tb, tfv);
}

#if BBH_DIST_ASM
__device__ __forceinline__ void mfma_f64_v0(d4& acc, double a, double b) {
  asm volatile("v_mfma_f64_16x16x4_f64 %0, %1, %2, 0" : "=&v"(acc) : "v"(a), "v"(b));
}
__device__ __forceinline__ void mfma_f64_v(d4& acc, double a, double b) {
  asm volatile("v_mfma_f64_16x16x4_f64 %0, %1, %2, %0" : "+v"(acc) : "v"(a), "v"(b));
}
#endif

template <int KD>
__device__ __forceinline__ void kvp_dist(const WaveCtx& c, const double (&tfv)[KD], d4& da, d4& db) {
#if BBH_CANDREG && !BBH_DIST_ASM
  da = (d4){0.0, 0.0, 0.0, 0.0};
  db = (d4){0.0, 0.0, 0.0, 0.0};
#pragma unroll
  for (int k = 0; k < KD; k += 2) {
    da = mfma_f64(tfv[k], c.cf[k], da);
    if (k + 1 < KD) db = mfma_f64(tfv[k + 1], c.cf[k + 1], db);
  }
#elif BBH_CANDREG
  static_assert(KD >= 2, "two accumulator chains");
  mfma_f64_v0(da, tfv[0], c.cf[0]);
  mfma_f64_v0(db, tfv[1], c.cf[1]);
#pragma unroll
  for (int k = 2; k < KD; k += 2) {
    mfma_f64_v(da, tfv[k], c.cf[k]);
    if (k + 1 < KD) mfma_f64_v(db, tfv[k + 1], c.cf[k + 1]);
  }
#else
  da = (d4){0.0, 0.0, 0.0, 0.0};
  db = (d4){0.0, 0.0, 0.0, 0.0};
#pragma unroll
  for (int k = 0; k < KD; k += 2) {
    da = mfma_f64(tfv[k], c.candl[k * 64], da);
    if (k + 1 < KD) db = mfma_f64(tfv[k + 1], c.candl[(k + 1) * 64], db);
  }
#endif
}

#define BBH_KV_STEPS 18
#ifndef BBH_KV_SQRT_NR
#define BBH_KV_SQRT_NR 1
#endif
#ifndef BBH_KV_NU
#define BBH_KV_NU 4
#endif
template <int NU>
struct KvState {
  double t[NU], y[NU], g[NU], h[NU], kf[NU], q[NU], tv[NU];
  int ki[NU], te[NU];
};

#define BBH_KV_EACH for (int u = 0; u < NU; u++)
template <int I, int N, class F>
__device__ __forceinline__ void static_for(F&& f) {
  if constexpr (I < N) {
    f(std::integral_constant<int, I>{});
    static_for<I + 1, N>(f);
  }
}

template <int KVF, int NU, int step>
__device__ __forceinline__ void kv_micro(KvState<NU>& P, const WaveCtx& c, int tb, int r0, const d4& da, const d4& db,
                                         double (&out)[4]) {
  constexpr bool HAS_TBL = (KVF & 1) != 0, RBFK = (KVF & 2) != 0;
  constexpr bool M32K = (KVF & 4) != 0;
  constexpr double KC1 = M32K ? 3.0 : 5.0, KC2 = M32K ? 0.0 : 1.0 / 3.0;
  constexpr double LOG2E = 1.4426950408889634074, LN2_HI = 6.93147180369123816490e-01,
                   LN2_LO = 1.90821492927058770002e-10;
  switch (step) {
    case 0:
#if BBH_DIST_ASM
      asm volatile("s_nop 15");
      asm volatile("s_nop 3");
#endif
#pragma unroll
      BBH_KV_EACH {
        const double r2 = da[r0 + u] + db[r0 + u];
        if (RBFK)
          P.g[u] = __builtin_fmin(__builtin_fmax(0.5 * r2, 0.0), 800.0);
        else
          P.t[u] = __builtin_fmax(KC1 * r2, 1e-300);
        if (HAS_TBL) P.te[u] = c.taskext[16 * tb + 4 * (r0 + u) + c.q];
      }
      break;
    case 1:
      if (RBFK) break;
#pragma unroll
      BBH_KV_EACH P.y[u] = __builtin_amdgcn_rsq(P.t[u]);
      break;
#if BBH_KV_SQRT_NR
    case 2:
      if (RBFK) break;
#pragma unroll
      BBH_KV_EACH P.g[u] = P.t[u] * P.y[u];
      break;
    case 3:
      if (RBFK) break;
#pragma unroll
      BBH_KV_EACH P.y[u] = fma(-P.g[u], P.y[u], 1.0);
      break;
    case 4:
      if (RBFK) break;
#pragma unroll
      BBH_KV_EACH P.h[u] = 0.5 * P.g[u];
      break;
    case 5: break;
    case 6:
      if (RBFK) break;
#pragma unroll
      BBH_KV_EACH P.g[u] = fma(P.h[u], P.y[u], P.g[u]);
      break;
#else
    case 2:
#pragma unroll
      BBH_KV_EACH P.g[u] = P.t[u] * P.y[u];
#pragma unroll
      BBH_KV_EACH P.h[u] = 0.5 * P.y[u];
      break;
    case 3:
#pragma unroll
      BBH_KV_EACH P.y[u] = fma(-P.h[u], P.g[u], 0.5);
      break;
    case 4:
#pragma unroll
      BBH_KV_EACH P.g[u] = fma(P.g[u], P.y[u], P.g[u]);
#pragma unroll
      BBH_KV_EACH P.h[u] = fma(P.h[u], P.y[u], P.h[u]);
      break;
    case 5:
#pragma unroll
      BBH_KV_EACH P.y[u] = fma(-P.g[u], P.g[u], P.t[u]);
      break;
    case 6:
#pragma unroll
      BBH_KV_EACH P.g[u] = __builtin_fmin(fma(P.y[u], P.h[u], P.g[u]), 800.0);
      break;
#endif
    case 7:
#pragma unroll
      BBH_KV_EACH P.kf[u] = __builtin_rint(P.g[u] * -LOG2E);
      if (!RBFK) {
#pragma unroll
        BBH_KV_EACH P.q[u] = M32K ? 1.0 : fma(P.g[u], KC2, 1.0);
      }
      break;
    case 8:
#pragma unroll
      BBH_KV_EACH P.t[u] = fma(P.kf[u], -LN2_HI, -P.g[u]);
      if (!RBFK) {
#pragma unroll
        BBH_KV_EACH P.q[u] = fma(P.q[u], P.g[u], 1.0);
      }
      break;
    case 9:
#pragma unroll
      BBH_KV_EACH P.t[u] = fma(P.kf[u], -LN2_LO, P.t[u]);
#pragma unroll
      BBH_KV_EACH {
        P.ki[u] = (int)P.kf[u];
        if (HAS_TBL) P.tv[u] = c.tbl[c.tc * c.T + P.te[u]];
      }
      break;
    case 10:
#pragma unroll
      BBH_KV_EACH P.h[u] = fma(2.4994304884701822e-08, P.t[u], 2.763229327960932e-07);
      break;
#define BBH_KV_HORNER2(CA, CB)                      \
  _Pragma("unroll") BBH_KV_EACH P.h[u] = fma(P.h[u], P.t[u], CA); \
  _Pragma("unroll") BBH_KV_EACH P.h[u] = fma(P.h[u], P.t[u], CB);
    case 11: BBH_KV_HORNER2(2.7557622530873466e-06, 2.4801486521427063e-05) break;
    case 12: BBH_KV_HORNER2(0.00019841269432679235, 0.001388888895122399) break;
    case 13: BBH_KV_HORNER2(0.00833333333355927, 0.04166666666649277) break;
    case 14: BBH_KV_HORNER2(0.1666666666666617, 0.5000000000000018) break;
    case 15: BBH_KV_HORNER2(1.0, 1.0) break;
#undef BBH_KV_HORNER2
    case 16:
      if (!RBFK) {
#pragma unroll
        BBH_KV_EACH P.h[u] *= P.q[u];
      }
      break;
    default:
#pragma unroll
      BBH_KV_EACH {
        double v = __builtin_ldexp(P.h[u], P.ki[u]);
        if (HAS_TBL) v *= P.tv[u];
        out[r0 + u] = v;
      }
      break;
  }
}
#undef BBH_KV_EACH

template <int KVF>
__device__ __forceinline__ void kv_all(const WaveCtx& c, int tb, const d4& da, const d4& db, double (&out)[4]) {
  KvState<4> P;
  static_for<0, BBH_KV_STEPS>([&](auto st) __attribute__((always_inline)) {
    kv_micro<KVF, 4, decltype(st)::value>(P, c, tb, 0, da, db, out);
  });
}

#ifndef BBH_RING
#define BBH_RING 8
#endif
#define BBH_NEXT_NONE 0
#define BBH_NEXT_COMPUTE 1
#define BBH_NEXT_LOAD 2
template <int W, int CNT, int TT, int KD, int KVF, bool DO_MEAN, int NEXT, int BASE, int REM>
__device__ __forceinline__ void kblock_p(const WaveCtx& c, const double* rf, int tb, const double (&kv)[4],
                                         double (&kvn)[4], d4 (&acc)[W], d4& accm, double (&ring)[BBH_RING], bool store) {
  constexpr int D = BBH_RING;
  constexpr int TOT = 4 * CNT;
  double tfv[KD];
  d4 dsa, dsb;
  double mbv[4];
  KvState<BBH_KV_NU> P;
  if (NEXT == BBH_NEXT_COMPUTE) kvp_load<KD>(c, tb + 1, tfv);
  if (NEXT == BBH_NEXT_LOAD) {
    if (tb + 1 < c.nl) {
#pragma unroll
      for (int rr = 0; rr < 4; rr++) kvn[rr] = c.kvl[(tb + 1) * 256 + rr * 64];
    } else {
#pragma unroll
      for (int rr = 0; rr < 4; rr++) kvn[rr] = c.kvc[(int64_t)(tb + 1) * 256 + rr * 64];
    }
  }
  if (store && tb < c.ncache) {
#pragma unroll
    for (int rr = 0; rr < 4; rr++) {
      if (tb < c.nl)
        c.kvl[tb * 256 + rr * 64] = kv[rr];
      else
        c.kvc[(int64_t)tb * 256 + rr * 64] = kv[rr];
    }
  }
  __builtin_amdgcn_sched_barrier(0);
  static_for<0, 4>([&](auto rc) __attribute__((always_inline)) {
    constexpr int r = decltype(rc)::value;
    if (DO_MEAN && r == 3) {
      if (BBH_MEAN_VALU_ONLY || c.al) {
#pragma unroll
        for (int rr = 0; rr < 4; rr++) mbv[rr] = c.al[16 * tb + 4 * rr];
      } else {
#pragma unroll
        for (int rr = 0; rr < 4; rr++) mbv[rr] = c.mb[(int64_t)(4 * tb + rr) * 64];
      }
    }
    static_for<0, CNT>([&](auto jc) __attribute__((always_inline)) {
      constexpr int jj = decltype(jc)::value;
      constexpr int i = r * CNT + jj;
      acc[TT + jj] = mfma_f64(kv[r], ring[(BASE + i) % D], acc[TT + jj]);
      if (i + D < TOT + REM) ring[(BASE + i) % D] = rf[(i + D) * 64];
      if constexpr (NEXT == BBH_NEXT_COMPUTE && (r == 1 || r == 2)) {
        if constexpr (BBH_KV_NU == 4) {
          constexpr int m = (r - 1) * CNT + jj;
          static_for<(m * BBH_KV_STEPS) / (2 * CNT), ((m + 1) * BBH_KV_STEPS) / (2 * CNT)>(
              [&](auto st) __attribute__((always_inline)) {
                kv_micro<KVF, BBH_KV_NU, decltype(st)::value>(P, c, tb + 1, 0, dsa, dsb, kvn);
              });
        } else {
          static_for<(jj * BBH_KV_STEPS) / CNT, ((jj + 1) * BBH_KV_STEPS) / CNT>(
              [&](auto st) __attribute__((always_inline)) {
                kv_micro<KVF, BBH_KV_NU, decltype(st)::value>(P, c, tb + 1, 2 * (r - 1), dsa, dsb, kvn);
              });
        }
      }
      __builtin_amdgcn_sched_barrier(0);
    });
    if (NEXT == BBH_NEXT_COMPUTE && r == 0) kvp_dist<KD>(c, tfv, dsa, dsb);
    if (DO_MEAN && r == 3) {
      if (BBH_MEAN_VALU_ONLY || c.al) {
#pragma unroll
        for (int rr = 0; rr < 4; rr++) accm[0] = fma(kv[rr], mbv[rr], accm[0]);
      } else {
#pragma unroll
        for (int rr = 0; rr < 4; rr++) accm = mfma_f64(kv[rr], mbv[rr], accm);
      }
    }
    __builtin_amdgcn_sched_barrier(0);
  });
}

template <int W, int TT, int KD, int KVF, bool DO_MEAN>
__device__ __forceinline__ void diag_steps_p(const WaveCtx& c, const double* rf, int j0, double (&kv)[4], d4 (&acc)[W],
                                             d4& accm, double (&ring)[BBH_RING], bool store) {
  if constexpr (TT < W) {
    double kvn[4];
    constexpr int NEXT = (TT + 1 < W) ? BBH_NEXT_COMPUTE : BBH_NEXT_NONE;
    constexpr int BASE = (4 * (TT * W - (TT * (TT - 1)) / 2)) % BBH_RING;
    constexpr int REM = 2 * (W - TT) * (W - TT - 1);
    kblock_p<W, W - TT, TT, KD, KVF, DO_MEAN, NEXT, BASE, REM>(c, rf, j0 + TT, kv, kvn, acc, accm, ring, store);
    if (NEXT) {
#pragma unroll
      for (int r = 0; r < 4; r++) kv[r] = kvn[r];
    }
    diag_steps_p<W, TT + 1, KD, KVF, DO_MEAN>(c, rf + 4 * (W - TT) * 64, j0, kv, acc, accm, ring, store);
  }
}

template <int W, int KD, int KVF, bool DO_MEAN>
__device__ __forceinline__ void pass_body_p(const WaveCtx& c, const double* rf, int j0, double (&ss)[4], d4& accm,
                                            bool cache) {
  d4 acc[W];
#pragma unroll
  for (int jj = 0; jj < W; jj++) acc[jj] = (d4){0.0, 0.0, 0.0, 0.0};
  double kv[4], kvn[4], ring[BBH_RING];
#pragma unroll
  for (int i = 0; i < BBH_RING; i++) ring[i] = rf[i * 64];
  if (cache && j0 > 0) {
#pragma unroll
    for (int r = 0; r < 4; r++) {
      if (c.nl > 0)
// ... 302 lines not shown
```

### baybe_amd/csrc/bbh_fused_coop_s.hip

```cpp
#include "bbh_coop.h"

#define BBH_COOP_SMALL_KD(KDV)                                                                              \
  if (kd == KDV) {                                                                                          \
    if (grid.x == 0) return true;                                                                           \
    if (a.g0 >= 6 && has_tbl)                                                                 \
      hipLaunchKernelGGL((bbh_coop_posterior_kernel<KDV, 1, 1, 6>), grid, dim3(256), lds, s, a);             \
    else if (a.g0 >= 6)                                                                                     \
      hipLaunchKernelGGL((bbh_coop_posterior_kernel<KDV, 0, 1, 6>), grid, dim3(256), lds, s, a);             \
    else if (has_tbl)                                                                                       \
      hipLaunchKernelGGL((bbh_coop_posterior_kernel<KDV, 1, 1, 4>), grid, dim3(256), lds, s, a);             \
    else                                                                                                    \
      hipLaunchKernelGGL((bbh_coop_posterior_kernel<KDV, 0, 1, 4>), grid, dim3(256), lds, s, a);             \
    return true;                                                                                            \
  }

bool bbh_coop_launch_small(int kd, int kind, bool has_tbl, dim3 grid, size_t lds, hipStream_t s, const CoopArgs& a) {
  if (kind != BBH_KERNEL_MATERN52) return false;
  BBH_COOP_SMALL_KD(2)
  BBH_COOP_SMALL_KD(4)
  BBH_COOP_SMALL_KD(6)
  BBH_COOP_SMALL_KD(8)
  return false;
}
```

### baybe_amd/csrc/bbh_model.hip

```cpp
#include <math.h>
#include <stdio.h>
#include <stdlib.h>
#include <string.h>

#include <chrono>

#include "bbh_common.h"

struct bbh_scatter_args {
  const unsigned char* src;
  unsigned char* dst[4];
  size_t off[4], bytes[4];
  unsigned char* zero;
  size_t zero_bytes;
  int* flag;
  int flag_value;
};
__global__ __launch_bounds__(256) void bbh_scatter_kernel(const bbh_scatter_args a) {
  const int r = blockIdx.y;
  const size_t i = ((size_t)blockIdx.x * 256 + threadIdx.x) * 8;
  if (a.flag && r == 0 && blockIdx.x == 0 && threadIdx.x == 0) __hip_atomic_store(a.flag, a.flag_value, __ATOMIC_RELAXED, __HIP_MEMORY_SCOPE_SYSTEM);
  if (r == 4) {
    if (i + 8 <= a.zero_bytes) *(unsigned long long*)(a.zero + i) = 0ull;
    return;
// ... 172 lines not shown
  {
    double uf[BBH_MAX_FACTORS] = {1.0, 1.0, 1.0, 1.0};
    for (int f = 0; f < ks.F; f++) uf[f] = (ks.F > 1 ? theta[ks.fos_off + f] : 1.0) * kf[f];
    for (int f = 0; f < ks.F; f++) wf[f] = ks.F > 1 ? bbh_combine_weight(ks.F, ks.combine, ks.grp, uf, f) : 1.0;
  }
  const double kb = bbh_kcomp(ks, theta, r2);
  double* prow = partial + ((int64_t)(a * gridDim.y + blockIdx.y) * 4 + wave) * nslots;
  {
    double v = (a == bb) ? G * nmask[a] : 0.0;
#pragma unroll
    for (int o = 32; o > 0; o >>= 1) v += __shfl_down(v, o, 64);
    if (lane == 0) {
      prow[TH_NOISE] = hoff >= 0 ? 0.0 : v;
      if (hoff >= 0)
        for (int t = 0; t < T; t++) {
          prow[hoff + t] = (t == ta) ? v : 0.0;
          prow[hoff + T + t] = 0.0;
        }
    }
  }
  {
    double v = ks.use_os ? G * kb * Bab : 0.0;
#pragma unroll
    for (int o = 32; o > 0; o >>= 1) v += __shfl_down(v, o, 64);
    if (lane == 0) {
      prow[TH_OS] = v;
      prow[TH_MEAN] = 0.0;
    }
  }
  for (int f = 0; f < ks.F; f++) {
    const double fos = ks.F > 1 ? theta[ks.fos_off + f] : 1.0;
    const double Gg = G * bbh_gfun(ks.kind[f], r2[f], ks.jb, al[f]) * os * Bab * wf[f] * fos;
    for (int j = 0; j < dn; j++) {
      const double l = theta[ks.ls_off[f] + j];
      const double xa = xnT[(int64_t)j * np + a], xb = xnT[(int64_t)j * np + bb];
      double v, vp = 0.0;
      if (ks.kind[f] == BBH_KERNEL_PERIODIC) {
        const double pl = theta[ks.per_off + f * dn + j], u = M_PI * (xa - xb) / pl, sn = sin(u);
        v = Gg * sn * sn / (l * l);
        vp = Gg * sin(2.0 * u) * M_PI * (xa - xb) / (l * pl * pl);
      } else {
        v = Gg * (BBH_KIND_IS_DOT(ks.kind[f]) ? xa * xb : (xa - xb) * (xa - xb)) / (l * l * l);
      }
#pragma unroll
      for (int o = 32; o > 0; o >>= 1) v += __shfl_down(v, o, 64);
      if (lane == 0) prow[ks.ls_off[f] + j] = v;
      if (ks.per_off >= 0) {
#pragma unroll
        for (int o = 32; o > 0; o >>= 1) vp += __shfl_down(vp, o, 64);
        if (lane == 0) prow[ks.per_off + f * dn + j] = vp;
      }
    }
    if (ks.F > 1) {
      double v = G * os * Bab * wf[f] * kf[f];
#pragma unroll
      for (int o = 32; o > 0; o >>= 1) v += __shfl_down(v, o, 64);
      if (lane == 0) prow[ks.fos_off + f] = v;
    }
    if (ks.alpha_off >= 0) {
      double v = 0.0;
      if (ks.kind[f] == BBH_KERNEL_RQ) {
        const double u = r2[f] / (2.0 * al[f]);
        v = G * os * Bab * wf[f] * fos * kf[f] * (u / (1.0 + u) - log1p(u));
      } else if (BBH_KIND_IS_POLY(ks.kind[f])) {
        const int pw = ks.kind[f] - BBH_KERNEL_POLY1 + 1;
        v = G * os * Bab * wf[f] * fos * (double)pw * bbh_powi(r2[f] + al[f], pw - 1);
      }
#pragma unroll
      for (int o = 32; o > 0; o >>= 1) v += __shfl_down(v, o, 64);
      if (lane == 0) prow[ks.alpha_off + f] = v;
    }
  }
  if (T > 1) {
    const double gk = G * kb * os;
    for (int c = 0; c < T * T; c++) {
      double v = (c == ta * T + tb) ? gk : 0.0;
#pragma unroll
      for (int o = 32; o > 0; o >>= 1) v += __shfl_down(v, o, 64);
      if (lane == 0) prow[TH_LS + dn + c] = v;
    }
  }
}

__global__ __launch_bounds__(256) void bbh_grad_reduce_kernel(const double* __restrict__ partial, int64_t rows,
                                                              int nslots, int mean_lo, int mean_hi,
                                                              double* __restrict__ out) {
  __shared__ double sm[4];
  const int slot = blockIdx.x;
  if (slot == TH_MEAN || (slot >= mean_lo && slot < mean_hi)) return;
  double v = 0.0;
  for (int64_t r = threadIdx.x; r < rows; r += 256) v += partial[r * nslots + slot];
  v = bbh_block_sum_256(v, sm);
  if (threadIdx.x == 0) out[1 + slot] = v;
}

static bool bbh_has_rq(const bbh_handle* h) {
  if (h->F <= 1) return BBH_KIND_HAS_ALPHA(h->desc.kernel_kind);
  for (int f = 0; f < h->F; f++)
    if (BBH_KIND_HAS_ALPHA(h->desc.factor_kind[f])) return true;
  return false;
}

bool bbh_has_dot_kind(const bbh_handle* h) {
  if (h->F <= 1) return BBH_KIND_IS_DOT(h->desc.kernel_kind);
  for (int f = 0; f < h->F; f++)
    if (BBH_KIND_IS_DOT(h->desc.factor_kind[f])) return true;
  return false;
}

static bool bbh_has_periodic(const bbh_handle* h) {
  if (h->F <= 1) return h->desc.kernel_kind == BBH_KERNEL_PERIODIC;
  for (int f = 0; f < h->F; f++)
    if (h->desc.factor_kind[f] == BBH_KERNEL_PERIODIC) return true;
  return false;
}

static int64_t bbh_theta_len_of(const bbh_handle* h) {
  return 3 + h->dn + (h->T > 1 ? (int64_t)h->T * h->T : 0) + (h->hadamard ? 2 * (int64_t)h->T : 0) +
         (h->F > 1 ? (int64_t)(h->F - 1) * h->dn + h->F : 0) + (bbh_has_rq(h) ? h->F : 0) +
         (bbh_has_periodic(h) ? (int64_t)h->F * h->dn : 0);
}

extern "C" int64_t bbh_theta_len(bbh_handle* h) {
  if (!h || !h->have_model) return -1;
  return bbh_theta_len_of(h);
}

bbh_kern_spec bbh_kern_spec_of(const bbh_handle* h) {
  bbh_kern_spec ks{};
  ks.F = h->F;
  ks.combine = h->desc.combine;
  for (int f = 0; f < BBH_MAX_FACTORS; f++) {
    const int g = h->desc.combine == 0 ? 0 : h->desc.combine == 1 ? f : h->desc.factor_group[f];
    ks.grp[f] = (g < 0 || g >= BBH_MAX_FACTORS) ? 0 : g;
  }
  ks.use_os = h->desc.use_outputscale;
  ks.jb = h->dn / 2 + 1;
  const int base = 3 + h->dn + (h->T > 1 ? h->T * h->T : 0) + (h->hadamard ? 2 * h->T : 0);
  for (int f = 0; f < BBH_MAX_FACTORS; f++) {
    ks.kind[f] = (f == 0 || h->F <= 1) ? h->desc.kernel_kind : h->desc.factor_kind[f];
    ks.ls_off[f] = (f == 0 || f >= h->F) ? 3 : base + (f - 1) * h->dn;
  }
  ks.fos_off = h->F > 1 ? base + (h->F - 1) * h->dn : -1;
  ks.alpha_off = bbh_has_rq(h) ? base + (h->F > 1 ? (h->F - 1) * h->dn + h->F : 0) : -1;
  ks.per_off = bbh_has_periodic(h) ? base + (h->F > 1 ? (h->F - 1) * h->dn + h->F : 0) + (bbh_has_rq(h) ? h->F : 0) : -1;
  return ks;
}

int bbh_hadamard_offset(const bbh_handle* h) { return h->hadamard ? 3 + h->dn + h->T * h->T : -1; }

static void bbh_reset_model_state(bbh_handle* h) {
  h->coopg_ready = false;
  h->coop_ready = false;
  h->coop2_ready = false;
  h->small_nb = 0;
  if (h->fit_exec) hipGraphExecDestroy(h->fit_exec);
  h->fit_exec = nullptr;
  h->fit_graph_failed = false;
  h->ncols = 0;
  h->have_model = false;
  h->factorized = false;
}

static void bbh_free_model(bbh_handle* h) {
  void* ptrs[] = {h->d_xnT,   h->d_task,    h->d_ystd,      h->d_theta, h->d_K,     h->d_X,       h->d_M,
                  h->d_Q,     h->d_Q2,      h->d_D,         h->d_tmp,   h->d_r,     h->d_t,       h->d_alpha,
                  h->d_u,     h->d_w,       h->d_q,         h->d_partial, h->d_out, h->d_info,    h->d_trainfrag,
                  h->d_rfrag, h->d_meanB,   h->d_sclofs,    h->d_numcol, h->d_tasktbl, h->d_taskext, h->d_beta, h->d_pass_off, h->d_pass_w, h->d_nmask, h->d_colfrag, h->d_pendT, h->d_colA, h->d_Mpart, h->d_trainfrag_f, h->d_sclofs_f};
  for (void* p : ptrs)
    if (p) hipFree(p);
  bbh_rff_destroy(h);
  h->d_xnT = h->d_ystd = h->d_theta = h->d_K = h->d_X = h->d_M = h->d_Q = h->d_Q2 = h->d_D = h->d_tmp = nullptr;
  h->d_r = h->d_t = h->d_alpha = h->d_u = h->d_w = h->d_q = h->d_partial = h->d_out = nullptr;
  h->d_trainfrag = h->d_rfrag = h->d_meanB = h->d_sclofs = h->d_tasktbl = h->d_beta = nullptr;
  h->d_task = h->d_info = h->d_numcol = h->d_taskext = h->d_pass_w = nullptr;
  h->d_pass_off = nullptr;
  h->d_nmask = nullptr;
  h->d_pendT = h->d_colA = h->d_Mpart = nullptr;
  h->d_trainfrag_f = h->d_sclofs_f = nullptr;
  h->tf_f_elems = 0;
  h->coopg_ready = false;
  h->colA_elems = 0;
  if (h->fit_exec) hipGraphExecDestroy(h->fit_exec);
  h->fit_exec = nullptr;
  h->fit_graph_failed = false;
  if (h->pin_theta) hipHostFree(h->pin_theta);
  if (h->pin_out) hipHostFree(h->pin_out);
  if (h->pin_info) hipHostFree(h->pin_info);
  h->pin_theta = h->pin_out = nullptr;
  h->pin_info = nullptr;
  h->d_colfrag = nullptr;
  h->colfrag_elems = 0;
  h->ncols = 0;
  h->rfrag_elems = 0;
  h->have_model = false;
  h->factorized = false;
  h->model_sig.clear();
}

void bbh_free_model_public(bbh_handle* h) { bbh_free_model(h); }

extern "C" int bbh_set_model(bbh_handle* h, const bbh_model_desc* desc, int64_t n, const double* X_train_host,
                             const double* y_train_host, const double* lo_host, const double* hi_host) {
  return bbh_set_model_ex(h, desc, n, X_train_host, y_train_host, lo_host, hi_host, nullptr, 0, 0.0, 1.0);
}

extern "C" int bbh_set_model_ex(bbh_handle* h, const bbh_model_desc* desc, int64_t n, const double* X_train_host,
                                const double* y_train_host, const double* lo_host, const double* hi_host,
                                const uint8_t* noise_mask_host, int use_given_std, double ybar_in, double ysd_in) {
  if (!h) return -1;
  if (!desc || n < 1 || !X_train_host || !y_train_host || !lo_host || !hi_host) {
    h->err = "bbh_set_model: bad arguments";
    return -1;
  }
  if (desc->kernel_kind < 0 || desc->kernel_kind > BBH_KERNEL_RFF || desc->d < 1 || desc->n_tasks < 1 ||
      (desc->n_tasks > 1 && (desc->task_col < 0 || desc->task_col >= desc->d)) ||
      (desc->criterion != BBH_CRITERION_MLL && desc->criterion != BBH_CRITERION_LOO)) {
    h->err = "bbh_set_model: invalid model description";
    return -1;
  }
  if (desc->n_factors > 1) {
    bool ok = desc->n_factors <= BBH_MAX_FACTORS && (desc->combine == 0 || desc->combine == 1 || desc->combine == 2) &&
              desc->factor_kind[0] == desc->kernel_kind;
    for (int f = 0; ok && desc->combine == 2 && f < desc->n_factors; f++) ok = desc->factor_group[f] >= 0 && desc->factor_group[f] < BBH_MAX_FACTORS;
    for (int f = 0; ok && f < desc->n_factors; f++) ok = desc->factor_kind[f] >= 0 && desc->factor_kind[f] <= BBH_KERNEL_PERIODIC;
    if (!ok) {
      h->err = "bbh_set_model: invalid composite kernel (2..4 factors, combine 0 | 1 | 2 with factor_group in 0..3, factor_kind[0] == kernel_kind)";
      return -1;
    }
  }
  BBH_HIP_TRY(h, hipSetDevice(h->device));
  const bool sm_trace = h->sw.setmodel_trace, sm_quiet = h->sw.setmodel_trace_quiet;
  const auto sm_t0 = std::chrono::steady_clock::now();
  struct sm_rec { const char* what; double us; };
  sm_rec sm_log[16];
  int sm_n = 0;
  auto sm_stamp = [&](const char* what) {
    if (!sm_trace) return;
    const double us = std::chrono::duration<double, std::micro>(std::chrono::steady_clock::now() - sm_t0).count();
    if (sm_quiet) {
      if (sm_n < 16) sm_log[sm_n++] = {what, us};
    } else {
      fprintf(stderr, "bbh_set_model %-10s %8.1f us\n", what, us);
    }
  };
  struct sm_flush_t {
    sm_rec* log; int* n;
    ~sm_flush_t() {
      if (*n == 0) return;
      char buf[1024]; int o = 0;
      for (int k = 0; k < *n && o < 900; k++) o += snprintf(buf + o, sizeof(buf) - o, " %s %.1f", log[k].what, log[k].us);
      fprintf(stderr, "bbh_set_model stages (us):%s\n", buf);
    }
  } sm_flush{sm_log, &sm_n};
  {
    int dn_new = 0;
    const int tc0 = (desc->n_tasks > 1 || desc->task_col >= 0) ? desc->task_col : -1;
    for (int c = 0; c < desc->d; c++) dn_new += (c != tc0);
    char sig[256];
    snprintf(sig, sizeof(sig), "%lld/%d/%d/%d/%d/%d/%d/%d/%d/%d/%d:%d,%d,%d,%d:%d,%d,%d,%d", (long long)bbh_round_up(n, BBH_PAD), desc->d, dn_new,
             desc->criterion, desc->kernel_kind, desc->task_col, desc->n_tasks, desc->use_outputscale, desc->hadamard, desc->n_factors, desc->combine,
             desc->factor_kind[0], desc->factor_kind[1], desc->factor_kind[2], desc->factor_kind[3], desc->factor_scaled[0],
             desc->factor_scaled[1], desc->factor_scaled[2], desc->factor_scaled[3]);
    if (desc->kernel_kind == BBH_KERNEL_RFF) snprintf(sig + strlen(sig), sizeof(sig) - strlen(sig), ":rff%d", h->rff_w_D);
    if (desc->combine == 2)
      snprintf(sig + strlen(sig), sizeof(sig) - strlen(sig), ":g%d%d%d%d", desc->factor_group[0], desc->factor_group[1], desc->factor_group[2],
               desc->factor_group[3]);
    if (h->have_model && h->model_sig == sig) {
      bbh_reset_model_state(h);
    } else {
      bbh_free_model(h);
      h->model_sig = sig;
    }
  }
  sm_stamp("reset");
  h->desc = *desc;
  h->n = n;
  h->np = bbh_round_up(n, BBH_PAD);
  h->nb = h->np / BBH_TB;
  h->T = desc->n_tasks;
  h->hadamard = (desc->hadamard != 0 && desc->n_tasks > 1);
  h->F = desc->n_factors > 1 ? desc->n_factors : 1;
  const int d = desc->d;
  const int tc = (desc->n_tasks > 1 || desc->task_col >= 0) ? desc->task_col : -1;
  h->numcol.clear();
  h->lo.clear();
  h->hi.clear();
  for (int c = 0; c < d; c++)
    if (c != tc) {
      h->numcol.push_back(c);
      h->lo.push_back(lo_host[c]);
      h->hi.push_back(hi_host[c]);
      if (!(hi_host[c] > lo_host[c])) {
        h->err = "bbh_set_model: scaling bounds need hi > lo for every numerical column";
        return -1;
      }
    }
  h->dn = (int)h->numcol.size();
  if (h->dn < 1) {
    h->err = "bbh_set_model: no numerical column";
    return -1;
  }
  h->kd = (h->dn + 2 + 3) / 4;
  if (h->kd <= 2)
    h->kd = 2;
  else if (h->kd <= 4)
    h->kd = 4;
  else if (h->kd <= 6)
    h->kd = 6;
  else if (h->kd <= 8)
    h->kd = 8;
  else if (h->kd <= 12)
    h->kd = 12;
  else if (h->kd <= 16)
    h->kd = 16;
  double ybar = 0.0;
  for (int64_t i = 0; i < n; i++) ybar += y_train_host[i];
  ybar /= (double)n;
  double ss = 0.0;
  for (int64_t i = 0; i < n; i++) ss += (y_train_host[i] - ybar) * (y_train_host[i] - ybar);
  double sd = (n > 1) ? sqrt(ss / (double)(n - 1)) : NAN;
  if (!(sd >= 1e-8)) sd = 1.0;
  if (use_given_std) {
    ybar = ybar_in;
    sd = ysd_in;
    if (!(sd > 0.0)) {
      h->err = "bbh_set_model_ex: ysd must be positive";
      return -1;
    }
  }
  h->ybar = ybar;
  h->ysd = sd;
// ... 434 lines not shown
```

### baybe_amd/csrc/bbh_panel.hip

```cpp
#include "bbh_coop2.h"
#include "bbh_coopg.h"
#include "bbh_small.h"
#include "bbh_coopcols.h"

__global__ void bbh_pack_rfrag_kernel(const double* __restrict__ X, int64_t np, int j0, int W, double* __restrict__ out) {
  const int tb = blockIdx.x, r = blockIdx.y, l = threadIdx.x;
  const int j1 = j0 + W;
  const int lo = tb > j0 ? tb : j0;
  const int cnt = j1 - lo;
  int64_t off;
  if (tb <= j0)
    off = (int64_t)4 * W * tb;
  else
    off = (int64_t)4 * (W * (int64_t)j0 + (int64_t)(tb - j0) * j1 - ((int64_t)(j0 + tb - 1) * (tb - j0)) / 2);
  off += (int64_t)r * cnt;
  const int64_t k = 16 * (int64_t)tb + 4 * r + (l >> 4);
  for (int jb = lo; jb < j1; jb++) {
    const int64_t j = 16 * (int64_t)jb + (l & 15);
    out[(off + (jb - lo)) * 64 + l] = (k <= j) ? X[j * np + k] : 0.0;
  }
}

__global__ void bbh_pack_coop_kernel(const double* __restrict__ X, int64_t np, int g0, int64_t frags, double* __restrict__ out) {
  const int w = blockIdx.z, G = g0 + blockIdx.y, ir = blockIdx.x, l = threadIdx.x;
  const int i = ir >> 2, r = ir & 3;
  const int cnt = BBH_COOP_ROUNDS - G;
  const int64_t base = (int64_t)(coop_frags_before(G) - coop_frags_before(g0)) + (int64_t)ir * cnt;
  const int64_t k = 16 * (int64_t)(4 * (G - g0) + i) + 4 * r + (l >> 4);
  for (int s = 0; s < cnt; s++) {
    const int rho = G + s;
    const int64_t jb = 4 * (rho - g0) + ((rho & 1) ? 3 - w : w);
    const int64_t j = 16 * jb + (l & 15);
    const int64_t fr = base + s;
    out[((int64_t)w * frags + (fr & ~(int64_t)1)) * 64 + 2 * l + (fr & 1)] = (k <= j) ? X[j * np + k] : 0.0;
  }
}

__global__ void bbh_pack_coop2_kernel(const double* __restrict__ X, int64_t np, int g0, int64_t frags, double* __restrict__ out) {
  const int w = blockIdx.y, l = threadIdx.x;
  int64_t f = blockIdx.x;
  const int64_t fr = f;
  int tb = -1, jb = 0, r = 0;
  const int RA = BBH_COOP_ROUNDS - g0;
  bool done = false;
  for (int G = g0; G < BBH_COOP_ROUNDS && !done; G++) {
    const int cnt = BBH_COOP_ROUNDS - G;
    if (f < 16 * cnt) {
      const int ir = (int)(f / cnt), s = (int)(f % cnt), rho = G + s;
      tb = 4 * (G - g0) + (ir >> 2);
      r = ir & 3;
      jb = 4 * (rho - g0) + ((rho & 1) ? 3 - w : w);
      done = true;
    } else {
      f -= 16 * cnt;
    }
  }
  for (int kg = 0; kg < RA && !done; kg++) {
    if (f < 16 * BBH_COOP_ROUNDS) {
      const int ir = (int)(f / BBH_COOP_ROUNDS), s = (int)(f % BBH_COOP_ROUNDS);
      tb = 4 * kg + (ir >> 2);
      r = ir & 3;
      jb = 4 * (RA + s) + ((s & 1) ? 3 - w : w);
      done = true;
    } else {
      f -= 16 * BBH_COOP_ROUNDS;
    }
  }
  for (int G = 0; G < BBH_COOP_ROUNDS && !done; G++) {
    const int cnt = BBH_COOP_ROUNDS - G;
    if (f < 16 * cnt) {
      const int ir = (int)(f / cnt), s = (int)(f % cnt), rho = G + s;
      tb = 4 * (RA + G) + (ir >> 2);
      r = ir & 3;
      jb = 4 * (RA + rho) + ((rho & 1) ? 3 - w : w);
      done = true;
    } else {
      f -= 16 * cnt;
    }
  }
  double v = 0.0;
  if (done) {
    const int64_t k = 16 * (int64_t)tb + 4 * r + (l >> 4), j = 16 * (int64_t)jb + (l & 15);
    if (k <= j) v = X[j * np + k];
  }
  out[((int64_t)w * frags + (fr & ~(int64_t)1)) * 64 + 2 * l + (fr & 1)] = v;
}

__global__ void bbh_init_meanB_kernel(const double* __restrict__ alpha, int64_t np, int64_t rows, double* __restrict__ Bm) {
  const int64_t e = (int64_t)blockIdx.x * blockDim.x + threadIdx.x;
  if (e >= rows * 16) return;
  const int64_t i = e >> 4;
  const int c = (int)(e & 15);
  Bm[e] = (c == 0 && i < np) ? alpha[i] : 0.0;
}

__global__ void bbh_set_beta_kernel(const double* __restrict__ betaT, int64_t ldb, int64_t np, int p, double* __restrict__ Bm) {
  const int64_t i = (int64_t)blockIdx.x * blockDim.x + threadIdx.x;
  if (i >= np + 16) return;
  for (int j = 0; j < p; j++) {
    double v;
    if (i < np)
      v = -betaT[(int64_t)j * ldb + i];
    else
      v = (i - np == j) ? 1.0 : 0.0;
    Bm[i * 16 + 1 + j] = v;
  }
}

static void host_pack_trainfrag(const bbh_handle* h, const double* pts, int64_t cnt, int64_t tb0, int64_t tb1,
                                std::vector<double>& out, const double* ls = nullptr) {
  const int dn = h->dn, kd = h->kd;
  if (!ls) ls = h->theta.data() + 3;
  out.assign((size_t)(tb1 - tb0) * kd * 64, 0.0);
  std::vector<double> a(dn);
  for (int64_t tb = tb0; tb < tb1; tb++)
    for (int c16 = 0; c16 < 16; c16++) {
      const int64_t i = (tb - tb0) * 16 + c16;
      const bool real = i < cnt;
      double na = 0.0;
      if (real)
        for (int j = 0; j < dn; j++) {
          a[j] = (pts[i * dn + j] - h->xcenter[j]) / ls[j];
          na += a[j] * a[j];
        }
      for (int k = 0; k < kd; k++)
        for (int qq = 0; qq < 4; qq++) {
          const int dim = 4 * k + qq;
          double v = 0.0;
          if (real) {
            if (dim < dn)
              v = -2.0 * a[dim];
            else if (dim == dn)
              v = na;
            else if (dim == dn + 1)
              v = 1.0;
          } else if (dim == dn) {
            v = 1e8;
          }
          out[((size_t)(tb - tb0) * kd + k) * 64 + qq * 16 + c16] = v;
        }
    }
}

static int bbh_coopg_kd(const bbh_handle* h) {
  const bbh_kern_spec ks = bbh_kern_spec_of(h);
  int feats = h->dn + 2;
  for (int f = 0; f < ks.F; f++)
    if (ks.kind[f] == BBH_KERNEL_PERIODIC && 2 * h->dn + 1 > feats) feats = 2 * h->dn + 1;
  const int kd = (feats + 3) / 4;
  for (int c : {2, 4, 6, 8})
    if (kd <= c) return c;
  return 0;
}

static bool bbh_coopg_model(const bbh_handle* h) {
  if (!bbh_materialised_only(h) || h->sw.coop_mode <= 0 || !h->sw.use_pipeline) return false;
  if (h->nb > 4 * BBH_COOP_ROUNDS || h->nb % 4 != 0) return false;
  const bbh_kern_spec ks = bbh_kern_spec_of(h);
  for (int f = 0; f < ks.F; f++)
    if (ks.kind[f] == BBH_KERNEL_MATERN12 || ks.kind[f] == BBH_KERNEL_PIECEWISE0) return false;
  const int kd = bbh_coopg_kd(h);
  return kd > 0 && bbh_coopg_launch(kd, ks.F, dim3(0), 0, nullptr, CoopGArgs{});
}

static void host_pack_trainfrag_generic(const bbh_handle* h, const bbh_kern_spec& ks, int f, int kd, int64_t nblocks, std::vector<double>& out,
                                        const double* pts = nullptr, int64_t cnt = -1) {
  const int dn = h->dn, kind = ks.kind[f];
  const double* th = h->theta.data();
  const double* ls = th + ks.ls_off[f];
  if (!pts) {
    pts = h->xn_host.data();
    cnt = h->n;
  }
  out.assign((size_t)nblocks * kd * 64, 0.0);
  std::vector<double> row((size_t)4 * kd);
  for (int64_t tb = 0; tb < nblocks; tb++)
    for (int c16 = 0; c16 < 16; c16++) {
      const int64_t i = tb * 16 + c16;
      const bool real = i < cnt;
      std::fill(row.begin(), row.end(), 0.0);
      const double* x = real ? pts + i * dn : nullptr;
      if (kind == BBH_KERNEL_PERIODIC) {
        double c0 = 0.0;
        for (int j = 0; j < dn; j++) c0 += 0.5 / ls[j];
        if (real)
          for (int j = 0; j < dn; j++) {
            const double al = 2.0 * M_PI * x[j] / th[ks.per_off + f * dn + j];
            row[j] = -cos(al) * 0.5 / ls[j];
            row[dn + j] = -sin(al) * 0.5 / ls[j];
          }
        row[2 * dn] = real ? c0 : 1e8;
      } else if (BBH_KIND_IS_DOT(kind)) {
        if (real)
          for (int j = 0; j < dn; j++) row[j] = x[j] / ls[j];
        row[dn] = real ? 0.0 : 1e8;
      } else {
        double na = 0.0;
        if (real)
          for (int j = 0; j < dn; j++) {
            const double a = (x[j] - h->xcenter[j]) / ls[j];
            row[j] = -2.0 * a;
            na += a * a;
          }
        row[dn] = real ? na : 1e8;
        row[dn + 1] = real ? 1.0 : 0.0;
      }
      for (int k = 0; k < kd; k++)
        for (int qq = 0; qq < 4; qq++) out[((size_t)tb * kd + k) * 64 + qq * 16 + c16] = row[4 * k + qq];
    }
}

static void host_feature_map(const bbh_handle* h, const bbh_kern_spec& ks, int f, int kd, CoopGFeat* out) {
  const int dn = h->dn, kind = ks.kind[f];
  const double* th = h->theta.data();
  const double* ls = th + ks.ls_off[f];
  for (int e = 0; e < 4 * kd; e++) out[e] = CoopGFeat{0.0, 0.0, -1, 5};
  for (int j = 0; j < dn; j++) {
    const double rng = h->hi[j] - h->lo[j];
    if (kind == BBH_KERNEL_PERIODIC) {
      const double per = th[ks.per_off + f * dn + j];
      out[j] = CoopGFeat{2.0 * M_PI / (rng * per), -2.0 * M_PI * h->lo[j] / (rng * per), j, 1};
      out[dn + j] = CoopGFeat{2.0 * M_PI / (rng * per), -2.0 * M_PI * h->lo[j] / (rng * per), j, 2};
    } else if (BBH_KIND_IS_DOT(kind)) {
      out[j] = CoopGFeat{1.0 / (rng * ls[j]), -h->lo[j] / (rng * ls[j]), j, 0};
    } else {
      out[j] = CoopGFeat{1.0 / (rng * ls[j]), -(h->lo[j] / rng + h->xcenter[j]) / ls[j], j, 0};
    }
  }
  if (kind == BBH_KERNEL_PERIODIC) {
    out[2 * dn] = CoopGFeat{0.0, 1.0, -1, 3};
  } else {
    out[dn] = CoopGFeat{0.0, 1.0, -1, 3};
    out[dn + 1] = CoopGFeat{0.0, 0.0, -1, 4};
  }
}

int bbh_pack_operands(bbh_handle* h) {
  hipStream_t s = h->stream;
  const int64_t np = h->np, nb = h->nb;
  const int dn = h->dn, kd = h->kd, T = h->T;
  const double* th = h->theta.data();
  std::vector<int> widths;
  {
    h->wmax = 16;
    int64_t left = nb;
    while (left >= h->wmax) {
      widths.push_back(h->wmax);
      left -= h->wmax;
    }
    if (left > 0) widths.push_back((int)left);
  }
  if ((int)widths.size() > BBH_MAX_PASS) {
    h->err = "n_train too large for the fused kernel (max 16384)";
    return -5;
  }
  int64_t total_frags = 0;
  std::vector<int64_t> pass_off(widths.size());
  {
    int j0 = 0;
    for (size_t ps = 0; ps < widths.size(); ps++) {
      pass_off[ps] = total_frags * 64;
      const int W = widths[ps], j1 = j0 + W;
      total_frags += (int64_t)4 * W * j0;
      for (int tb = j0; tb < j1; tb++) total_frags += 4 * (j1 - tb);
      j0 = j1;
    }
  }
  if (!h->d_pass_off) BBH_HIP_TRY(h, hipMalloc((void**)&h->d_pass_off, sizeof(int64_t) * BBH_MAX_PASS));
  if (!h->d_pass_w) BBH_HIP_TRY(h, hipMalloc((void**)&h->d_pass_w, sizeof(int) * BBH_MAX_PASS));
  BBH_HIP_TRY(h, hipMemcpyAsync(h->d_pass_off, pass_off.data(), sizeof(int64_t) * pass_off.size(), hipMemcpyHostToDevice, s));
  BBH_HIP_TRY(h, hipMemcpyAsync(h->d_pass_w, widths.data(), sizeof(int) * widths.size(), hipMemcpyHostToDevice, s));
  h->npass = (int)widths.size();
  h->pass_w_last = widths.back();
  if (!h->d_rfrag || h->rfrag_elems != total_frags * 64) {
    if (h->d_rfrag) hipFree(h->d_rfrag);
    h->d_rfrag = nullptr;
    BBH_HIP_TRY(h, hipMalloc((void**)&h->d_rfrag, sizeof(double) * total_frags * 64));
    h->rfrag_elems = total_frags * 64;
  }
  if (!h->d_trainfrag) BBH_HIP_TRY(h, hipMalloc((void**)&h->d_trainfrag, sizeof(double) * (nb + 1) * kd * 64));
  if (!h->d_meanB) BBH_HIP_TRY(h, hipMalloc((void**)&h->d_meanB, sizeof(double) * (np + 16) * 16));
  if (!h->d_sclofs) BBH_HIP_TRY(h, hipMalloc((void**)&h->d_sclofs, sizeof(double) * 2 * dn));
  if (!h->d_numcol) BBH_HIP_TRY(h, hipMalloc((void**)&h->d_numcol, sizeof(int) * dn));
  if (!h->d_tasktbl) BBH_HIP_TRY(h, hipMalloc((void**)&h->d_tasktbl, sizeof(double) * T * T));
  if (!h->d_taskext) BBH_HIP_TRY(h, hipMalloc((void**)&h->d_taskext, sizeof(int) * (np + 16)));
  {
    int j0 = 0;
    for (size_t ps = 0; ps < widths.size(); ps++) {
      const int W = widths[ps];
      hipLaunchKernelGGL(bbh_pack_rfrag_kernel, dim3((unsigned)(j0 + W), 4), dim3(64), 0, s, h->d_X, np, j0, W,
                         h->d_rfrag + pass_off[ps]);
      j0 += W;
    }
  }
  h->small_nb = 0;
  if (h->sw.small_on && h->sw.use_pipeline && nb <= 8 && h->n >= 1) {
    const int NB = (int)((h->n + 15) / 16);
    const bool has_tbl0 = (T > 1) || h->desc.use_outputscale;
    if (bbh_small_launch(h->kd, h->desc.kernel_kind, has_tbl0, NB, 0, h->num_cu, nullptr, SmallArgs{})) {
      if (!h->d_rsmall) BBH_HIP_TRY(h, hipMalloc((void**)&h->d_rsmall, sizeof(double) * 36 * 4 * 64));
      hipLaunchKernelGGL(bbh_pack_small_kernel, dim3((unsigned)NB, (unsigned)NB, 4), dim3(64), 0, s, h->d_X, np, NB, h->d_rsmall);
      h->small_nb = NB;
    }
  }
  h->coop_ready = false;
  {
    const bool has_tbl0 = (T > 1) || h->desc.use_outputscale;
    if (h->sw.coop_mode > 0 && h->sw.use_pipeline && nb <= 4 * BBH_COOP_ROUNDS && nb % 4 == 0 &&
        bbh_coop_launch(h->kd, h->desc.kernel_kind, has_tbl0, dim3(0), 0, nullptr, CoopArgs{}, h->sw.coop_small)) {
      const int g0 = BBH_COOP_ROUNDS - (int)(nb / 4);
      const int64_t frags = coop_frags_before(BBH_COOP_ROUNDS) - coop_frags_before(g0);
      if (!h->d_rstream || h->rstream_frags != frags) {
        if (h->d_rstream) hipFree(h->d_rstream);
        h->d_rstream = nullptr;
        BBH_HIP_TRY(h, hipMalloc((void**)&h->d_rstream, sizeof(double) * 4 * frags * 64));
        h->rstream_frags = frags;
      }
      hipLaunchKernelGGL(bbh_pack_coop_kernel, dim3(16, (unsigned)(BBH_COOP_ROUNDS - g0), 4), dim3(64), 0, s, h->d_X, np, g0, frags,
                         h->d_rstream);
      h->coop_g0 = g0;
      h->coop_ready = true;
    }
  }
  h->coopg_ready = false;
  if (bbh_coopg_model(h)) {
    const bbh_kern_spec ks = bbh_kern_spec_of(h);
    const int g0 = BBH_COOP_ROUNDS - (int)(nb / 4);
    const int64_t frags = coop_frags_before(BBH_COOP_ROUNDS) - coop_frags_before(g0);
    if (!h->d_rstream || h->rstream_frags != frags) {
      if (h->d_rstream) hipFree(h->d_rstream);
      h->d_rstream = nullptr;
      BBH_HIP_TRY(h, hipMalloc((void**)&h->d_rstream, sizeof(double) * 4 * frags * 64));
      h->rstream_frags = frags;
    }
    hipLaunchKernelGGL(bbh_pack_coop_kernel, dim3(16, (unsigned)(BBH_COOP_ROUNDS - g0), 4), dim3(64), 0, s, h->d_X, np, g0, frags,
                       h->d_rstream);
    h->coop_g0 = g0;
    const int kdg = bbh_coopg_kd(h);
    const int64_t per = (nb + 1) * (int64_t)kdg * 64;
    if (!h->d_trainfrag_f || h->tf_f_elems != per * ks.F) {
      if (h->d_trainfrag_f) hipFree(h->d_trainfrag_f);
      if (h->d_sclofs_f) hipFree(h->d_sclofs_f);
      h->d_trainfrag_f = h->d_sclofs_f = nullptr;
      BBH_HIP_TRY(h, hipMalloc((void**)&h->d_trainfrag_f, sizeof(double) * per * ks.F));
      BBH_HIP_TRY(h, hipMalloc((void**)&h->d_sclofs_f, sizeof(CoopGFeat) * 4 * 8 * BBH_MAX_FACTORS));
      h->tf_f_elems = per * ks.F;
    }
    std::vector<double> tff;
    std::vector<CoopGFeat> feat((size_t)ks.F * 4 * kdg);
    for (int f = 0; f < ks.F; f++) {
      std::vector<double> one;
      host_pack_trainfrag_generic(h, ks, f, kdg, nb + 1, one);
      tff.insert(tff.end(), one.begin(), one.end());
      host_feature_map(h, ks, f, kdg, feat.data() + (size_t)f * 4 * kdg);
    }
    BBH_HIP_TRY(h, hipMemcpyAsync(h->d_trainfrag_f, tff.data(), sizeof(double) * tff.size(), hipMemcpyHostToDevice, s));
    BBH_HIP_TRY(h, hipMemcpyAsync(h->d_sclofs_f, feat.data(), sizeof(CoopGFeat) * feat.size(), hipMemcpyHostToDevice, s));
    BBH_HIP_TRY(h, hipStreamSynchronize(s));
    h->coopg_ready = true;
  }
  h->coop2_ready = false;
  {
    const bool has_tbl0 = (T > 1) || h->desc.use_outputscale;
    if (h->sw.coop_mode > 0 && h->sw.use_pipeline && nb > 4 * BBH_COOP_ROUNDS && nb <= 8 * BBH_COOP_ROUNDS && nb % 4 == 0 &&
        bbh_coop2_launch(h->kd, h->desc.kernel_kind, has_tbl0, dim3(0), 0, nullptr, CoopArgs{})) {
      const int g0 = 2 * BBH_COOP_ROUNDS - (int)(nb / 4);
      const int64_t frags = coop2_frags(g0);
      if (!h->d_rstream || h->rstream_frags != frags) {
        if (h->d_rstream) hipFree(h->d_rstream);
        h->d_rstream = nullptr;
        BBH_HIP_TRY(h, hipMalloc((void**)&h->d_rstream, sizeof(double) * 4 * frags * 64));
        h->rstream_frags = frags;
      }
      hipLaunchKernelGGL(bbh_pack_coop2_kernel, dim3((unsigned)frags, 4), dim3(64), 0, s, h->d_X, np, g0, frags, h->d_rstream);
      h->coop_g0 = g0;
      h->coop2_ready = true;
    }
  }
  std::vector<double> tf;
  host_pack_trainfrag(h, h->xn_host.data(), h->n, 0, nb + 1, tf);
  BBH_HIP_TRY(h, hipMemcpyAsync(h->d_trainfrag, tf.data(), sizeof(double) * tf.size(), hipMemcpyHostToDevice, s));
  std::vector<double> so(2 * dn);
  for (int j = 0; j < dn; j++) {
    const double rng = h->hi[j] - h->lo[j];
    so[j] = 1.0 / (rng * th[3 + j]);
    so[dn + j] = -(h->lo[j] / rng + h->xcenter[j]) / th[3 + j];
  }
  BBH_HIP_TRY(h, hipMemcpyAsync(h->d_sclofs, so.data(), sizeof(double) * 2 * dn, hipMemcpyHostToDevice, s));
  BBH_HIP_TRY(h, hipMemcpyAsync(h->d_numcol, h->numcol.data(), sizeof(int) * dn, hipMemcpyHostToDevice, s));
  const double os = h->desc.use_outputscale ? th[2] : 1.0;
  std::vector<double> tbl((size_t)T * T, os);
  if (T > 1)
    for (int i = 0; i < T * T; i++) tbl[i] = os * th[3 + dn + i];
  BBH_HIP_TRY(h, hipMemcpyAsync(h->d_tasktbl, tbl.data(), sizeof(double) * T * T, hipMemcpyHostToDevice, s));
  std::vector<int> te(np + 16, 0);
  for (int64_t i = 0; i < h->n; i++) te[i] = h->task_host[i];
  BBH_HIP_TRY(h, hipMemcpyAsync(h->d_taskext, te.data(), sizeof(int) * (np + 16), hipMemcpyHostToDevice, s));
  hipLaunchKernelGGL(bbh_init_meanB_kernel, dim3((unsigned)(((np + 16) * 16 + 255) / 256)), dim3(256), 0, s, h->d_alpha,
                     np, np + 16, h->d_meanB);
  BBH_HIP_TRY(h, hipStreamSynchronize(s));
  h->nb_ext = nb;
  h->p = 0;
  return 0;
}

void bbh_fill_fused_args(bbh_handle* h, FusedArgs& a, const double* X_dev, int64_t N, int64_t ldx) {
  a.numcol_identity = 0;
  a.X = X_dev;
  a.N = N;
  a.ldx = ldx;
  a.trainfrag = h->d_trainfrag;
  a.rfrag = h->d_rfrag;
  a.meanB = h->d_meanB;
  a.scl = h->d_sclofs;
  a.ofs = h->d_sclofs + h->dn;
  a.numcol = h->d_numcol;
  a.tasktbl = h->d_tasktbl;
  a.taskmean = h->hadamard ? h->d_theta + bbh_hadamard_offset(h) + h->T : nullptr;
  a.taskext = h->d_taskext;
  a.mean = nullptr;
  a.var = nullptr;
  a.cross = nullptr;
  a.pass_off = h->d_pass_off;
  a.pass_w = h->d_pass_w;
  a.npass = h->npass;
  a.kind = h->desc.kernel_kind;
  a.dn = h->dn;
  a.kd = h->kd;
  a.nb = (int)h->nb;
  a.nb_ext = (int)h->nb;
  a.task_col = h->desc.task_col;
  a.T = h->T;
  a.p = 0;
  a.with_var = 0;
  a.ybar = h->ybar;
  a.ysd = h->ysd;
  a.mean_const = h->theta[1];
  a.prior_scale = h->desc.use_outputscale ? h->theta[2] : 1.0;
  a.qz = nullptr;
  a.qS = 0;
  a.q_best_f = 0.0;
  a.q_sign = 1.0;
  a.q_alive = nullptr;
  a.q_scores = nullptr;
  a.kvcache = nullptr;
  a.slab_flags = nullptr;
  a.nslab = 0;
  a.nxcc = 1;
  a.ncache = 0;
  a.nblk = (N + 63) / 64;
}

int bbh_launch_fused(bbh_handle* h, const double* X_dev, int64_t N, int64_t ldx, double* mean_dev, double* var_dev,
                     double* cross_dev, bool with_var) {
  if (N <= 0) return 0;
  if (bbh_is_rff(h)) return bbh_rff_posterior_launch(h, X_dev, N, ldx, mean_dev, with_var ? var_dev : nullptr, cross_dev);
  const bool coopg = h->coopg_ready && with_var && h->p == 0 && !cross_dev && !h->fuse_qz && h->sw.use_mean_valu;
  const bool coopg_cross = h->coopg_ready && !with_var && !h->fuse_qz && h->sw.coopg_cross_on;
  if (bbh_materialised_only(h) && !coopg && !coopg_cross)
    return bbh_launch_unfused_ext(h, X_dev, N, ldx, mean_dev, with_var ? var_dev : nullptr, cross_dev);
  FusedArgs a;
  bbh_fill_fused_args(h, a, X_dev, N, ldx);
  a.mean = mean_dev;
  a.var = var_dev;
  a.cross = cross_dev;
  a.nb_ext = (int)h->nb_ext;
  a.p = h->p;
  a.with_var = with_var ? 1 : 0;
  if (h->fuse_qz && with_var) {
    a.qz = h->fuse_qz;
    a.qS = h->fuse_S;
    a.q_best_f = h->fuse_best_f;
    a.q_sign = h->fuse_sign;
    a.q_alive = h->fuse_alive;
    a.q_scores = h->fuse_scores;
  }
  const bool has_tbl = (h->T > 1) || h->desc.use_outputscale;
  const bool m52 = (a.kind == BBH_KERNEL_MATERN52);
  const bool rbf = (a.kind == BBH_KERNEL_RBF), m32 = (a.kind == BBH_KERNEL_MATERN32);
  a.has_tbl = has_tbl ? 1 : 0;
  a.numcol_identity = 1;
  for (int j = 0; j < h->dn; j++)
    if (h->numcol[j] != j) a.numcol_identity = 0;
  const int kdp = ((m52 || ((rbf || m32) && !has_tbl)) && h->sw.use_pipeline && (h->kd == 2 || h->kd == 4 || h->kd == 6 || h->kd == 8 || h->kd == 12 || h->kd == 16)) ? h->kd : 0;
  dim3 grid((unsigned)a.nblk), block(256);
  a.mean_valu = (kdp && h->p == 0 && !cross_dev && h->sw.use_mean_valu && h->nb <= 256) ? 1 : 0;
  size_t lds = sizeof(double) * (4 * h->kd * 64 + (a.qz ? a.qS : 0) + (a.mean_valu ? 16 * h->nb : 0));
  a.nl = 0;
  if (kdp && with_var && h->npass > 1 && h->sw.use_kvcache) {
    a.ncache = (int)(h->nb - h->pass_w_last);
    const size_t lds_wg = h->lds_per_block / 2;
    const size_t budget = lds_wg > lds ? lds_wg - lds : 0;
    int nl = (int)(budget / (4 * 256 * sizeof(double)));
    if (h->sw.kv_lds_blocks >= 0 && nl > h->sw.kv_lds_blocks) nl = h->sw.kv_lds_blocks;
    a.nl = nl < a.ncache ? nl : a.ncache;
    const int rest = a.ncache - a.nl;
    const bool global_part = h->sw.kv_global_mode == 1 || (h->sw.kv_global_mode < 0 && rest >= 24);
    if (!global_part) a.ncache = a.nl;
    lds += sizeof(double) * 4 * 256 * (size_t)a.nl;
  }
  if (a.ncache > a.nl) {
    a.nslab = 2 * 8 * h->num_cu;
    a.nxcc = (h->num_cu % 8 == 0 && h->num_cu >= 64) ? 8 : 1;
    const size_t need = sizeof(double) * (size_t)a.nslab * (size_t)(a.ncache - a.nl) * 256;
    if (need > h->kvcache_bytes) {
      if (h->d_kvcache) BBH_HIP_TRY(h, hipFree(h->d_kvcache));
      h->d_kvcache = nullptr;
      h->kvcache_bytes = 0;
      BBH_HIP_TRY(h, hipMalloc((void**)&h->d_kvcache, need));
      h->kvcache_bytes = need;
    }
    if (!h->d_slab_flags) {
      BBH_HIP_TRY(h, hipMalloc((void**)&h->d_slab_flags, sizeof(int) * (size_t)a.nslab));
      BBH_HIP_TRY(h, hipMemsetAsync(h->d_slab_flags, 0, sizeof(int) * (size_t)a.nslab, h->stream));
    }
    a.kvcache = h->d_kvcache;
    a.slab_flags = h->d_slab_flags;
  }
  bbh_timed_scope timed(h, with_var ? BBH_TIMED_POSTERIOR : BBH_TIMED_CROSS);
  if (coopg || coopg_cross) {
    const bbh_kern_spec ks = bbh_kern_spec_of(h);
    const double* th = h->theta.data();
    CoopGArgs g;
    g.c.f = a;
    g.c.f.mean_valu = 1;
    g.c.rstream = h->d_rstream;
    g.c.frags = h->rstream_frags;
    g.c.g0 = h->coop_g0;
    g.F = ks.F;
    g.combine = ks.combine;
    g.has_tbl = has_tbl ? 1 : 0;
    g.jb = ks.jb;
    g.has_dot = 0;
    for (int f = 0; f < BBH_MAX_FACTORS; f++) {
      g.kind[f] = ks.kind[f < ks.F ? f : 0];
      g.grp[f] = ks.grp[f];
      g.fos[f] = (ks.F > 1 && f < ks.F) ? th[ks.fos_off + f] : 1.0;
      g.alpha[f] = (ks.alpha_off >= 0 && f < ks.F) ? th[ks.alpha_off + f] : 1.0;
      if (f < ks.F && BBH_KIND_IS_DOT(ks.kind[f])) g.has_dot = 1;
    }
    g.prior_k0 = ks.F > 1 ? bbh_combine(ks.F, ks.combine, ks.grp, g.fos) : 1.0;
    const int kdg = bbh_coopg_kd(h);
    g.trainfrag_f = h->d_trainfrag_f;
    g.tf_stride = (h->nb + 1) * (int64_t)kdg * 64;
    g.feat = (const CoopGFeat*)h->d_sclofs_f;
    if (coopg_cross) {
      if (!bbh_coopg_cross_launch(kdg, ks.F, dim3((unsigned)((N + 63) / 64)), h->stream, g)) {
        h->err = "generic cross-covariance pass: no instantiation for this model although its operands were packed";
        return -6;
      }
      BBH_HIP_TRY(h, hipGetLastError());
      return 0;
    }
    const size_t clds = sizeof(double) * (16 * (size_t)h->nb + (2 * 4 * 256 + 128));
    bbh_coopg_launch(kdg, ks.F, dim3((unsigned)((N + 15) / 16)), clds, h->stream, g);
    h->last_form = 4;
    BBH_HIP_TRY(h, hipGetLastError());
    return 0;
  }
  const int64_t small_min_rows[9] = {0, 0, 0, 0, 0, 20000, 60000, 120000, 300000};
  if (h->small_nb > 0 && h->sw.small_on && with_var && h->p == 0 && !cross_dev && !a.qz && h->sw.use_mean_valu &&
      (h->sw.small_force || N >= small_min_rows[h->small_nb])) {
    SmallArgs sa;
    sa.f = a;
    sa.rsmall = h->d_rsmall;
    const int NB = h->small_nb;
    if (!bbh_small_launch(h->kd, a.kind, has_tbl, NB, (N + 15) / 16, h->num_cu, h->stream, sa)) {
      h->err = "register-resident posterior form: no instantiation for this model although its operands were packed";
      return -6;
    }
    h->last_form = 5;
    BBH_HIP_TRY(h, hipGetLastError());
    return 0;
  }
  const int kdc = (h->sw.use_pipeline && (h->kd == 2 || h->kd == 4 || h->kd == 6 || h->kd == 8 || h->kd == 12 || h->kd == 16)) ? h->kd : 0;
  const bool coop_mean_valu = h->p == 0 && !cross_dev && h->sw.use_mean_valu && h->nb <= 256;
  if (h->coop_ready && kdc && with_var && coop_mean_valu && !a.qz) {
    CoopArgs ca;
    ca.f = a;
    ca.rstream = h->d_rstream;
    ca.frags = h->rstream_frags;
    ca.g0 = h->coop_g0;
    const size_t clds = sizeof(double) * (16 * (size_t)h->nb + (2 * 4 * 256 + 128));
    const dim3 cgrid((unsigned)((N + 15) / 16));
    bbh_coop_launch(kdc, a.kind, has_tbl, cgrid, clds, h->stream, ca, h->sw.coop_small);
    h->last_form = 1;
    BBH_HIP_TRY(h, hipGetLastError());
    return 0;
  }
  if (h->coop2_ready && kdc && with_var && coop_mean_valu && !a.qz) {
    CoopArgs ca;
    ca.f = a;
    ca.rstream = h->d_rstream;
    ca.frags = h->rstream_frags;
    ca.g0 = h->coop_g0;
    const int ra = BBH_COOP_ROUNDS - ca.g0;
    const size_t clds = sizeof(double) * (16 * (size_t)h->nb + (size_t)(ra > 2 ? ra : 2) * 4 * 256 + 128);
    bbh_coop2_launch(kdc, a.kind, has_tbl, dim3((unsigned)((N + 15) / 16)), clds, h->stream, ca);
    h->last_form = 3;
    BBH_HIP_TRY(h, hipGetLastError());
    return 0;
  }
  if (with_var) h->last_form = 0;
  if (kdp == 2)
    bbh_fused_launch_kd2(a.kind, has_tbl, grid, block, lds, h->stream, a);
  else if (kdp == 4)
    bbh_fused_launch_kd4(a.kind, has_tbl, grid, block, lds, h->stream, a);
  else if (kdp == 6)
    bbh_fused_launch_kd6(a.kind, has_tbl, grid, block, lds, h->stream, a);
  else if (kdp == 8)
    bbh_fused_launch_kd8(a.kind, has_tbl, grid, block, lds, h->stream, a);
  else if (kdp == 12)
    bbh_fused_launch_kd12(a.kind, has_tbl, grid, block, lds, h->stream, a);
  else if (kdp == 16)
    bbh_fused_launch_kd16(a.kind, has_tbl, grid, block, lds, h->stream, a);
  else
    bbh_fused_launch_kd0(has_tbl, m52, grid, block, lds, h->stream, a);
  BBH_HIP_TRY(h, hipGetLastError());
  return 0;
}

#define BBH_KSTAR_CB 8
__global__ __launch_bounds__(256) void bbh_kstar_kernel(const double* __restrict__ X, int64_t Nc, int64_t ldx,
                                                        const double* __restrict__ xnT, const int* __restrict__ task,
                                                        const double* __restrict__ theta, const int* __restrict__ numcol,
                                                        const double* __restrict__ lo, const double* __restrict__ hi,
                                                        int n, int64_t np, int dn, const bbh_kern_spec ks, int T,
                                                        int task_col, int64_t ldk, double* __restrict__ Kst) {
  extern __shared__ double s_ks[];
  double* s_il = s_ks;
  double* s_xc = s_ks + ks.F * dn;
  const int64_t cand0 = (int64_t)blockIdx.y * BBH_KSTAR_CB;
  const int64_t i = (int64_t)blockIdx.x * 256 + threadIdx.x;
  for (int e = threadIdx.x; e < ks.F * dn; e += 256) s_il[e] = 1.0 / theta[ks.ls_off[e / dn] + e % dn];
  for (int e = threadIdx.x; e < BBH_KSTAR_CB * dn; e += 256) {
    const int64_t cand = cand0 + e / dn;
    const int j = e % dn;
    s_xc[e] = cand < Nc ? (X[cand * ldx + numcol[j]] - lo[j]) / (hi[j] - lo[j]) : 0.0;
  }
  __syncthreads();
  if (i >= np) return;
  double r2[BBH_KSTAR_CB][BBH_MAX_FACTORS];
#pragma unroll
  for (int c = 0; c < BBH_KSTAR_CB; c++)
#pragma unroll
    for (int f = 0; f < BBH_MAX_FACTORS; f++) r2[c][f] = 0.0;
  if (i < n)
    for (int j = 0; j < dn; j++) {
      const double x = xnT[(int64_t)j * np + i];
#pragma unroll
      for (int c = 0; c < BBH_KSTAR_CB; c++) {
        const double xc = s_xc[c * dn + j];
#pragma unroll
        for (int f = 0; f < BBH_MAX_FACTORS; f++)
          if (f < ks.F) r2[c][f] += bbh_metric_term_f(ks, theta, f, j, dn, xc, x, s_il[f * dn + j]);
      }
    }
  const int ti = (T > 1 && i < n) ? task[i] : 0;
#pragma unroll
  for (int c = 0; c < BBH_KSTAR_CB; c++) {
    const int64_t cand = cand0 + c;
    double v = 0.0;
    if (cand < Nc && i < n) {
      v = bbh_kcomp(ks, theta, r2[c]);
      if (ks.use_os) v *= theta[2];
      if (T > 1) {
        int tcand = (int)X[cand * ldx + task_col];
        tcand = tcand < 0 ? 0 : (tcand >= T ? T - 1 : tcand);
        v *= theta[3 + dn + tcand * T + ti];
      }
    }
    Kst[cand * ldk + i] = v;
  }
}

__global__ __launch_bounds__(256) void bbh_kdiag_kernel(const double* __restrict__ X, int64_t Nc, int64_t ldx,
                                                        const double* __restrict__ theta, const int* __restrict__ numcol,
                                                        const double* __restrict__ lo, const double* __restrict__ hi, int dn,
                                                        const bbh_kern_spec ks, double* __restrict__ out) {
  const int64_t i = (int64_t)blockIdx.x * 256 + threadIdx.x;
  if (i >= Nc) return;
  double r2[BBH_MAX_FACTORS] = {0.0, 0.0, 0.0, 0.0};
  for (int j = 0; j < dn; j++) {
    const double x = (X[i * ldx + numcol[j]] - lo[j]) / (hi[j] - lo[j]);
    for (int f = 0; f < ks.F; f++) r2[f] += bbh_metric_term_f(ks, theta, f, j, dn, x, x, 1.0 / theta[ks.ls_off[f] + j]);
  }
  out[i] = bbh_kcomp(ks, theta, r2);
}

__global__ __launch_bounds__(256) void bbh_rowreduce_kernel(const double* __restrict__ Kst, const double* __restrict__ V,
                                                            const double* __restrict__ alpha,
                                                            const double* __restrict__ X, int64_t ldx, int64_t Nc,
                                                            int64_t np, const double* __restrict__ theta, int dn,
                                                            double prior_base, int T, int task_col, int hoff, double ybar, double ysd,
                                                            double* __restrict__ mean, double* __restrict__ var,
                                                            const double* __restrict__ kdiag, double os) {
  const int lane = threadIdx.x & 63;
  const int64_t cand = (int64_t)blockIdx.x * 4 + (threadIdx.x >> 6);
  if (cand >= Nc) return;
  double sm = 0.0, sv = 0.0;
  for (int64_t i = lane; i < np; i += 64) {
    sm = fma(Kst[cand * np + i], alpha[i], sm);
    const double v = V[cand * np + i];
    sv = fma(v, v, sv);
  }
#pragma unroll
  for (int o = 32; o > 0; o >>= 1) {
    sm += __shfl_down(sm, o, 64);
    sv += __shfl_down(sv, o, 64);
  }
  if (lane == 0) {
    double pv = kdiag ? os * kdiag[cand] : prior_base, mc = theta[1];
    if (T > 1) {
      int tcand = (int)X[cand * ldx + task_col];
      tcand = tcand < 0 ? 0 : (tcand >= T ? T - 1 : tcand);
      pv *= theta[3 + dn + tcand * T + tcand];
      if (hoff >= 0) mc = theta[hoff + T + tcand];
    }
    if (mean) mean[cand] = ybar + ysd * (mc + sm);
    if (var) var[cand] = ysd * ysd * (pv - sv);
  }
}

static int bbh_unfused_chunk(bbh_handle* h, const double* X_dev, int64_t Nc, int64_t ldx, double* Kst, double* V,
                             const double* d_lo, const double* d_hi) {
  const int64_t np = h->np;
  const int64_t Ncpad = bbh_round_up(Nc, 64);
  dim3 grid((unsigned)((np + 255) / 256), (unsigned)(Ncpad / BBH_KSTAR_CB)), block(256);
  hipLaunchKernelGGL(bbh_kstar_kernel, grid, block, sizeof(double) * h->dn * (BBH_KSTAR_CB + h->F), h->stream, X_dev, Nc, ldx, h->d_xnT, h->d_task, h->d_theta,
                     h->d_numcol, d_lo, d_hi, (int)h->n, np, h->dn, bbh_kern_spec_of(h), h->T, h->desc.task_col, np, Kst);
  if (V) bbh_gemm(h->stream, false, true, Ncpad, np, np, 1.0, Kst, np, 0, h->d_X, np, 0, 0.0, V, np, 0, 1);
  BBH_HIP_TRY(h, hipGetLastError());
  return 0;
}

bool bbh_materialised_only(const bbh_handle* h) { return h->F > 1 || h->desc.kernel_kind > BBH_KERNEL_RBF; }

double bbh_prior_base(const bbh_handle* h) {
// ... 699 lines not shown
```

### baybe_amd/engine.py

```python

from __future__ import annotations

import contextlib
import ctypes as C
import math
import os
import threading
from dataclasses import dataclass

import numpy as np
from scipy import optimize as sopt

from baybe_amd import _lib
from baybe_amd._lib import HipError, HipUnavailableError
from baybe_amd.gp_spec import (
    FastObjective,
    GPParams,
    GPSpec,
    initial_params,
    sample_params_from_priors,
    objective_from_data_term,
    pack_raw,
    raw_bounds,
    theta_from_params,
# ... 748 lines not shown
        P = np.ascontiguousarray(X_pending, dtype=np.float64)
        p = P.shape[0]
        if p > MAX_PENDING:
            raise ValueError(f"at most {MAX_PENDING} pending points are supported by the HIP path")
        mp = np.empty(p)
        cpp = np.empty((p, p))
        self._check(self._lib.bbh_pending_set(self._h, _dp(P), p, _dp(mp), _dp(cpp)), "bbh_pending_set")
        self._p = p
        self._pend_stats = (mp, cpp)
        return mp, cpp

    def cross_cov(self, X):
        torch = self._torch()
        X = self._as_dev(X)
        N = X.shape[0]
        cross = torch.empty((N, getattr(self, "_p", 0)), dtype=torch.float64, device=X.device)
        self._check(self._lib.bbh_cross_cov(self._h, X.data_ptr(), N, X.stride(0), cross.data_ptr()), "bbh_cross_cov")
        return cross

    def cross_cov_many(self, X, X_pending: np.ndarray):
        torch = self._torch()
        P = np.ascontiguousarray(np.atleast_2d(X_pending), dtype=np.float64)
        cols = []
        for c0 in range(0, len(P), MAX_PENDING):
            self.set_pending(P[c0 : c0 + MAX_PENDING])
            cols.append(self.cross_cov(X))
        return cols[0] if len(cols) == 1 else torch.cat(cols, dim=1).contiguous()

    def qlogei_pending_big(self, mean, var, cross, X_pending: np.ndarray, z: np.ndarray, best_f: float, sign: float = 1.0,
                           alive=None, stats=None):
        torch = self._torch()
        P = np.ascontiguousarray(np.atleast_2d(X_pending), dtype=np.float64)
        p = P.shape[0]
        if not 1 <= p <= MAX_PENDING_BIG or cross.shape[1] != p:
            raise ValueError(f"qlogei_pending_big handles 1 ... {MAX_PENDING_BIG} pending points")
        mp, cpp = stats if stats is not None else self.posterior_joint(P)
        z = np.ascontiguousarray(z, dtype=np.float64)
        N = mean.shape[0]
        scores = torch.empty(N, dtype=torch.float64, device=mean.device)
        cpp = np.ascontiguousarray(cpp, dtype=np.float64)
        self._check(
            self._lib.bbh_qlogei_pending_big(
                self._h, mean.data_ptr(), var.data_ptr(), cross.data_ptr(), N, p, _dp(np.ascontiguousarray(mp)), _dp(cpp), _dp(z),
                z.shape[0], float(best_f), float(sign), alive.data_ptr() if alive is not None else None, scores.data_ptr(),
            ),
            "bbh_qlogei_pending_big",
        )
        return scores

    def qlogei_pending(self, mean, var, cross, z: np.ndarray, best_f: float, sign: float = 1.0, alive=None):
        torch = self._torch()
        z = np.ascontiguousarray(z, dtype=np.float64)
        S = z.shape[0]
        N = mean.shape[0]
        scores = torch.empty(N, dtype=torch.float64, device=mean.device)
        self._check(
            self._lib.bbh_qlogei_pending(
                self._h, mean.data_ptr(), var.data_ptr(), cross.data_ptr(), N, _dp(z), S, float(best_f), float(sign),
                alive.data_ptr() if alive is not None else None, scores.data_ptr(),
            ),
            "bbh_qlogei_pending",
        )
        return scores

    def sobol_normal_dev(self, S: int, q: int, seed: int):
        torch = self._torch()
        out = torch.empty((S, q), dtype=torch.float64, device=self._dev())
        state0 = _sobol_state0(q)
        self._check(self._lib.bbh_sobol_normal_dev(self._h, state0.ctypes.data_as(_lib.c_int64_p), int(seed) & 0xFFFFFFFFFFFFFFFF, S, q,
                                                   out.data_ptr()), "bbh_sobol_normal_dev")
        return out

    def argmax(self, scores):
        v, i = C.c_double(), C.c_int64()
        self._check(self._lib.bbh_argmax(self._h, scores.data_ptr(), scores.shape[0], C.byref(v), C.byref(i)), "bbh_argmax")
        return v.value, i.value

    def topk(self, scores, k: int):
        vals = np.empty(k)
        idx = np.empty(k, dtype=np.int64)
        self._check(
            self._lib.bbh_topk(self._h, scores.data_ptr(), scores.shape[0], k, _dp(vals), idx.ctypes.data_as(_lib.c_int64_p)),
            "bbh_topk",
        )
        return vals, idx

    def fps_prepare(self, X, mean: np.ndarray, scale: np.ndarray, order=None):
        torch = self._torch()
        N, d = X.shape
        M = N if order is None else int(order.shape[0])
        ldp = -(-M // 256) * 256
        P = torch.empty((d, ldp), dtype=torch.float64, device=X.device)
        mean = np.ascontiguousarray(mean, dtype=np.float64)
        scale = np.ascontiguousarray(scale, dtype=np.float64)
        self._check(self._lib.bbh_fps_prepare(self._h, X.data_ptr(), N, d, X.stride(0), _dp(mean), _dp(scale),
                                              None if order is None else order.data_ptr(), M, P.data_ptr(), ldp), "bbh_fps_prepare")
        return P

    def fps_farthest_pair(self, P, M: int, alive=None):
        v, a, b = C.c_double(), C.c_int64(), C.c_int64()
        self._check(self._lib.bbh_fps_farthest_pair(self._h, P.data_ptr(), M, P.shape[0], P.stride(0),
                                                    None if alive is None else alive.data_ptr(), C.byref(v), C.byref(a), C.byref(b)),
                    "bbh_fps_farthest_pair")
        return v.value, a.value, b.value

    def fps_greedy(self, P, M: int, alive=None, starts=None, n_picks: int = 0, k: int = -1, want_count: bool = False):
        ranks = np.empty(max(n_picks, 1), dtype=np.int64)
        d2 = np.empty(max(n_picks, 1))
        count = C.c_int64(-1)
        st = None if starts is None else np.ascontiguousarray(starts, dtype=np.int64)
        self._check(self._lib.bbh_fps_greedy(
            self._h, P.data_ptr(), M, P.shape[0], P.stride(0), None if alive is None else alive.data_ptr(),
            None if st is None else st.ctypes.data_as(_lib.c_int64_p), 0 if st is None else len(st), n_picks, k,
            ranks.ctypes.data_as(_lib.c_int64_p), _dp(d2), C.byref(count) if want_count else None), "bbh_fps_greedy")
        return ranks[:n_picks], d2[:n_picks], count.value

    def comm_unique_id(self) -> bytes:
        buf = C.create_string_buffer(256)
        n = self._lib.bbh_comm_unique_id(buf, 256)
        if n <= 0:
            raise HipError("bbh_comm_unique_id failed: RCCL (librccl.so.1) could not be loaded")
        return buf.raw[:n]

    def comm_init(self, rank: int, world: int, unique_id: bytes):
        self._check(self._lib.bbh_comm_init(self._h, int(rank), int(world), unique_id, len(unique_id)), "bbh_comm_init")
        self._comm = (int(rank), int(world))

    def allgather_topk(self, scores, row_offset: int, k: int):
        vals, idx = np.empty(k), np.empty(k, dtype=np.int64)
        self._check(
            self._lib.bbh_allgather_topk(self._h, scores.data_ptr() if scores.shape[0] else None, scores.shape[0],
                                         int(row_offset), int(k), _dp(vals), idx.ctypes.data_as(_lib.c_int64_p)),
            "bbh_allgather_topk",
        )
        return vals, idx

    def allgather_argmax(self, scores, row_offset: int, X):
        val, gidx, row = C.c_double(), C.c_int64(), np.empty(self.spec.d)
        N = scores.shape[0]
        self._check(
            self._lib.bbh_allgather_argmax(self._h, scores.data_ptr() if N else None, N, int(row_offset),
                                           X.data_ptr() if N else None, X.stride(0) if N else self.spec.d, C.byref(val),
                                           C.byref(gidx), _dp(row)),
            "bbh_allgather_argmax",
        )
        return val.value, gidx.value, row

    def set_slice_rows(self, rows: int):
        self._check(self._lib.bbh_set_slice_rows(self._h, int(rows)), "bbh_set_slice_rows")

    def posterior_kernel_form(self) -> str:
        return {0: "windowed", 1: "cooperative", 2: "materialised", 3: "cooperative-2sweep", 4: "cooperative-generic",
                5: "register-resident", 6: "feature-space"}.get(self._lib.bbh_last_posterior_form(self._h), "none")

    def fit_evaluation_form(self) -> str:
        return {0: "launch", 1: "small", 2: "tiles+mt", 3: "tiles+mt-partial", 4: "tiles", 5: "gram+tiles", 6: "one-launch",
                7: "split", 8: "rff", 9: "steps+tail"}.get(self._lib.bbh_last_fit_form(self._h), "none")

    def timing(self, enable, families=None):
        code = 0
        if enable:
            code = 1 if not families else 2 * sum(1 << _lib.TIMED_FAMILIES[f] for f in families)
        self._check(self._lib.bbh_timing_enable(self._h, code), "bbh_timing_enable")

    def timing_read(self, reset: bool = True, family: str = "posterior"):
        ms, cnt = C.c_double(), C.c_int64()
        self._check(self._lib.bbh_timing_read_family(self._h, _lib.TIMED_FAMILIES[family], C.byref(ms), C.byref(cnt),
                                                     1 if reset else 0), "bbh_timing_read_family")
        return ms.value, cnt.value

    def greedy_qlogei(self, *args, **kwargs) -> "GreedyResult":
        import inspect

        shard = inspect.signature(self._greedy_qlogei).bind(*args, **kwargs).arguments.get("shard")
        repro = shard is not None and getattr(shard, "reproducible", False)
        if repro:
            self.set_slice_rows(shard.N_total)
        try:
            return self._greedy_qlogei(*args, **kwargs)
        finally:
            if repro:
                self.set_slice_rows(0)

    def _greedy_qlogei(
        self,
        X,
        q: int,
        S: int = 512,
        seed: int | None = None,
        sign: float = 1.0,
        X_pending: np.ndarray | None = None,
        best_f: float | None = None,
        z_by_q: dict | None = None,
        shard=None,
        kind: str = "qLogEI",
        beta: float = 0.2,
        alive=None,
        speculate: bool = True,
        objective=None,
    ) -> GreedyResult:
        torch = self._torch()
        X = self._as_dev(X)
        N = X.shape[0]
        d = self.spec.d
        if seed is None and z_by_q is None:
            seed = draw_sampler_seed()
        if best_f is None:
            best_f = self.best_f(sign) if objective is None else self.best_f(1.0, objective)
        okw = {} if objective is None else {"objective": objective}
        base = np.zeros((0, d)) if X_pending is None or len(X_pending) == 0 else np.atleast_2d(np.asarray(X_pending, dtype=np.float64))
        alive = torch.ones(N, dtype=torch.uint8, device=X.device) if alive is None else alive.clone()
        mean = var = None
        chosen_rows: list[np.ndarray] = []
        indices, values = [], []

        def get_z(qp: int) -> np.ndarray:
            return z_by_q[qp] if z_by_q is not None else sobol_normal_base_samples(S, qp, seed)

        if q > 0 and N > 0:
            self.set_pending(None)
            mean, var = self.posterior(X)
        z_next = get_z(1 + base.shape[0])
        spec_rows, spec_pos, cross_spec, big_cross, spec_stats = None, {}, None, None, None
        first_vals = first_top = None
        b0 = base.shape[0]
        for _step in range(q):
            pend = np.vstack([base] + chosen_rows) if chosen_rows else base
            p = pend.shape[0]
            z = z_next
            if p == 0:
                if mean is None:
                    self.set_pending(None)
                    mean, var = self.posterior(X)
                if kind == "qLogEI" and shard is None and N > 0 and objective is None:
                    m_spec = min(MAX_PENDING - b0, N, 4 * q) if (q > 1 and speculate and N > 1 and b0 < MAX_PENDING) else 1
                    scores, first_vals, first_top = self.qlogei_topk(mean, var, z[:, 0], best_f, sign, max(1, m_spec), alive)
                else:
                    scores = self.mc_acq(kind, mean, var, z[:, 0], best_f, sign, beta, alive, **okw)
            else:
                if mean is None:
                    mean, var = self.posterior(X)
                if p > MAX_PENDING and objective is not None:
                    raise ValueError(f"joint q-batches beyond {MAX_PENDING + 1} points are not available with a transformed target")
                if p > MAX_PENDING:
                    if kind != "qLogEI":
                        raise ValueError(f"joint q-batches beyond {MAX_PENDING + 1} points are available for qLogEI only")
                    if p > MAX_PENDING_BIG:
                        raise ValueError(f"at most {MAX_PENDING_BIG} pending points (batch size + pending experiments <= "
                                         f"{MAX_PENDING_BIG + 1}) are supported by the HIP path")
                    if big_cross is None or big_cross.shape[1] != p - 1:
                        big_cross = self.cross_cov_many(X, pend)
                    else:
                        big_cross = torch.cat([big_cross, self.cross_cov_many(X, pend[-1:])], dim=1).contiguous()
                    scores = self.qlogei_pending_big(mean, var, big_cross, pend, z, best_f, sign, alive)
                else:
                    cols = None
                    if cross_spec is not None:
                        cols = [spec_pos.get(ix) for ix in indices]
                        cols = None if any(c is None for c in cols) else list(range(b0)) + cols
                    if cols is not None and kind == "qLogEI" and spec_stats is not None and objective is None:
                        cross = cross_spec[:, cols].contiguous() if len(cols) != cross_spec.shape[1] else cross_spec
                        ix = np.asarray(cols)
                        scores = self.qlogei_pending_big(mean, var, cross, pend, z, best_f, sign, alive,
                                                         stats=(spec_stats[0][ix], spec_stats[1][np.ix_(ix, ix)]))
                    else:
                        self.set_pending(pend)
                        if cols is not None:
                            cross = cross_spec[:, cols].contiguous() if len(cols) != cross_spec.shape[1] else cross_spec
                        else:
                            cross = self.cross_cov(X)
                        scores = self.mc_acq(kind, mean, var, z, best_f, sign, beta, alive, cross=cross, **okw)
                    if p == MAX_PENDING:
                        big_cross = cross
            step0_global = None
            if _step == 0 and q > 1 and speculate and b0 < MAX_PENDING and (N > 1 or shard is not None):
                if shard is None:
                    m_spec = min(MAX_PENDING - b0, N, 4 * q)
                    tv, top = (first_vals, first_top) if first_top is not None and len(first_top) == m_spec else self.topk(scores, m_spec)
                    keep = [j for j, (t, v) in enumerate(zip(top, tv)) if t >= 0 and v > -math.inf]
                    top = [int(top[j]) for j in keep]
                    spec_rows = X[torch.as_tensor(top, device=X.device), :d].cpu().numpy() if top else None
                else:
                    m_spec = min(MAX_PENDING - b0, shard.N_total, 4 * q)
                    lv, li = self.topk(scores, min(m_spec, N)) if N > 0 else (np.empty(0), np.empty(0, dtype=np.int64))
                    tv, top, rows = shard.global_topk_rows(lv, li, m_spec, X, d)
                    if len(top):
                        step0_global = (float(tv[0]), int(top[0]), rows[0].copy())
                    keep = [j for j, v in enumerate(tv) if v > -math.inf]
                    top = [int(top[j]) for j in keep]
                    spec_rows = rows[keep] if keep else None
                if top:
                    spec_stats = self.set_pending(np.vstack([base, spec_rows]))
                    cross_spec = self.cross_cov(X) if N > 0 else torch.empty((0, b0 + len(top)), dtype=torch.float64, device=X.device)
                    spec_pos = {ix: b0 + j for j, ix in enumerate(top)}
            if _step + 1 < q:
                z_next = get_z(2 + p)
            if step0_global is not None:
                val, gidx, row = step0_global
                if shard.owns(gidx):
                    alive[shard.to_local(gidx)] = 0
                idx = gidx
            elif shard is not None and shard.rccl_bound(self):
                val, gidx, row = self.allgather_argmax(scores, shard.start, X)
                if shard.owns(gidx):
                    alive[shard.to_local(gidx)] = 0
                idx = gidx
# ... 22 lines not shown
```

### include/baybe_hip.h

```cpp
#ifndef BAYBE_HIP_H
#define BAYBE_HIP_H

#include <stdint.h>

#ifdef __cplusplus
extern "C" {
#endif

typedef struct bbh_handle bbh_handle;

enum bbh_kernel_kind {
  BBH_KERNEL_MATERN12 = 0,
  BBH_KERNEL_MATERN32 = 1,
  BBH_KERNEL_MATERN52 = 2,
  BBH_KERNEL_RBF = 3,
  BBH_KERNEL_PIECEWISE0 = 4,
  BBH_KERNEL_PIECEWISE1 = 5,
  BBH_KERNEL_PIECEWISE2 = 6,
  BBH_KERNEL_PIECEWISE3 = 7,
  BBH_KERNEL_RQ = 8,
  BBH_KERNEL_LINEAR = 9,
  BBH_KERNEL_POLY1 = 10,
  BBH_KERNEL_POLY2 = 11,
  BBH_KERNEL_POLY3 = 12,
// ... 57 lines not shown

int bbh_qlogei_q1(bbh_handle* h, const double* mean_dev, const double* var_dev, int64_t N,
                  const double* z_host, int64_t S, double best_f, double sign,
                  const uint8_t* alive_dev, double* scores_dev);

int bbh_qlogei_q1_topk(bbh_handle* h, const double* mean_dev, const double* var_dev, int64_t N,
                       const double* z_host, int64_t S, double best_f, double sign,
                       const uint8_t* alive_dev, double* scores_dev, int64_t k, double* vals_host, int64_t* idx_host);

int bbh_score_qlogei(bbh_handle* h, const double* X_dev, int64_t N, int64_t ldx, const double* z_host,
                     int64_t S, double best_f, double sign, const uint8_t* alive_dev, double* mean_dev,
                     double* var_dev, double* scores_dev);

#define BBH_MAX_PENDING 15
int bbh_pending_set(bbh_handle* h, const double* Xpend_host, int64_t p, double* mean_p_host,
                    double* cov_pp_host);
int bbh_cross_cov(bbh_handle* h, const double* X_dev, int64_t N, int64_t ldx, double* cross_dev);
int bbh_qlogei_pending(bbh_handle* h, const double* mean_dev, const double* var_dev,
                       const double* cross_dev, int64_t N, const double* z_host, int64_t S,
                       double best_f, double sign, const uint8_t* alive_dev, double* scores_dev);

enum bbh_acq_kind {
  BBH_ACQ_QLOGEI = 0, BBH_ACQ_QEI = 1, BBH_ACQ_QPI = 2, BBH_ACQ_QSR = 3, BBH_ACQ_QUCB = 4, BBH_ACQ_QPSTD = 5,
  BBH_ACQ_PM = 10, BBH_ACQ_PSTD = 11, BBH_ACQ_UCB = 12, BBH_ACQ_EI = 13, BBH_ACQ_LOGEI = 14, BBH_ACQ_PI = 15,
  BBH_ACQ_QNEI = 6, BBH_ACQ_QLOGNEI = 7
};
int bbh_mc_acq_q1(bbh_handle* h, int32_t kind, const double* mean_dev, const double* var_dev, int64_t N,
                  const double* z_host, int64_t S, double best_f, double sign, double beta,
                  const uint8_t* alive_dev, double* scores_dev);
int bbh_mc_acq_pending(bbh_handle* h, int32_t kind, const double* mean_dev, const double* var_dev,
                       const double* cross_dev, int64_t N, const double* z_host, int64_t S, double best_f,
                       double sign, double beta, const uint8_t* alive_dev, double* scores_dev);
int bbh_qlogei_pending_big(bbh_handle* h, const double* mean_dev, const double* var_dev, const double* cross_dev,
                           int64_t N, int64_t p, const double* mean_p_host, const double* cov_pp_host,
                           const double* z_host, int64_t S, double best_f, double sign, const uint8_t* alive_dev,
                           double* scores_dev);
enum bbh_objective_op {
  BBH_OBJ_AFFINE = 0,
  BBH_OBJ_CLAMP = 1,
  BBH_OBJ_TWOSIDED = 2,
  BBH_OBJ_BELL = 3,
  BBH_OBJ_LOG = 4,
  BBH_OBJ_EXP = 5,
  BBH_OBJ_POW = 6,
  BBH_OBJ_SIGMOID = 7
};
#define BBH_OBJ_MAX_OPS 8
typedef struct bbh_objective_prog {
  int32_t n_ops;
  int32_t op[BBH_OBJ_MAX_OPS];
  double p[BBH_OBJ_MAX_OPS][3];
} bbh_objective_prog;
int bbh_mc_acq_obj_q1(bbh_handle* h, int32_t kind, const bbh_objective_prog* prog, const double* mean_dev, const double* var_dev,
                      int64_t N, const double* z_host, int64_t S, double best_f, double beta, const uint8_t* alive_dev,
                      double* scores_dev);
int bbh_mc_acq_obj_pending(bbh_handle* h, int32_t kind, const bbh_objective_prog* prog, const double* mean_dev,
                           const double* var_dev, const double* cross_dev, int64_t N, int64_t p, const double* mean_p_host,
                           const double* cov_pp_host, const double* z_host, int64_t S, double best_f, double beta,
                           const uint8_t* alive_dev, double* scores_dev);
int bbh_analytic_acq(bbh_handle* h, int32_t kind, const double* mean_dev, const double* var_dev, int64_t N,
                     double best_f, double sign, double beta, int32_t maximize, const uint8_t* alive_dev,
                     double* scores_dev);

#define BBH_MAX_OBJECTIVES 4
int bbh_qlognehvi(bbh_handle* h, int32_t m, int64_t N, const double* const* tmat_dev,
                  const double* const* var_dev, const double* sign_host, const double* zx_host, int64_t S,
                  const int64_t* cell_off_host, const double* cell_lo_host, const double* cell_loglen_host,
                  const uint8_t* alive_dev, double* scores_dev);
int bbh_qlognehvi_sm(bbh_handle* h, int32_t m, int64_t N, const double* const* tmat_dev,
                  const double* const* var_dev, const double* sign_host, const double* zx_host, int64_t S,
                  const int64_t* cell_off_host, const double* cell_lo_host, const double* cell_loglen_host,
                  const uint8_t* alive_dev, double* scores_dev);

int bbh_pareto_frequency(bbh_handle* h, const double* obj_host, int64_t S, int64_t n, int32_t m,
                         const double* ref_host, int64_t* counts_host);

int bbh_pareto_frequency_dev(bbh_handle* h, const double* obj_dev, int64_t S, int64_t n, int32_t m,
                             const double* ref_host, int64_t* counts_host);

int bbh_nehvi_samples(bbh_handle* h, const double* z_host, int64_t S, int64_t nb, double sign, int32_t o, int32_t m,
                      double* Fb_dev, int32_t want_columns);
int bbh_nehvi_samples_dev(bbh_handle* h, const double* z_dev, int64_t ld, const int32_t* cols_dev, int64_t S, int64_t nb, double sign,
                          int32_t o, int32_t m, double* Fb_dev, int32_t want_columns);

int bbh_cells_build_dev(bbh_handle* h, const double* Fb_dev, int64_t S, int64_t nb, int32_t m, const double* ref_host,
                        int64_t* total_out, int64_t* overflow_out);
int bbh_cells_read_dev(bbh_handle* h, int64_t* off_host, double* lo_host, double* loglen_host);
int bbh_qlognehvi_cells(bbh_handle* h, int32_t m, int64_t N, const double* const* tmat_dev,
                        const double* const* var_dev, const double* sign_host, const double* zx_host, int64_t S,
                        const uint8_t* alive_dev, double* scores_dev);

int bbh_best_frequency_dev(bbh_handle* h, const double* obj_dev, int64_t S, int64_t nb, int64_t* counts_host);
int bbh_sample_best_dev(bbh_handle* h, const double* obj_dev, int64_t S, int64_t nb, double* best_dev);
int bbh_nei_q1(bbh_handle* h, int32_t kind, const double* tmat_sm_dev, const double* var_dev, int64_t N, const double* zx_host,
               int64_t S, const double* best_dev, double sign, const uint8_t* alive_dev, double* scores_dev);
int bbh_score_nei(bbh_handle* h, int32_t kind, const double* X_dev, int64_t N, int64_t ldx, const double* var_dev,
                  const double* zx_host, int64_t S, const double* best_dev, double sign, const uint8_t* alive_dev,
                  double* scores_dev);

int bbh_scalarized_best_dev(bbh_handle* h, const double* Fb_dev, int64_t S, int64_t nb, int32_t m, const double* w_host,
                            const double* hi_host, const double* inv_range_host, double* best_dev);
int bbh_scalarized_best_frequency_dev(bbh_handle* h, const double* Fb_dev, int64_t S, int64_t nb, int32_t m, const double* w_host,
                                      const double* hi_host, const double* inv_range_host, int64_t* counts_host);
int bbh_nparego_q1(bbh_handle* h, int32_t m, int64_t N, const double* const* tmat_sm_dev, const double* const* var_dev,
                   const double* sign_host, const double* zx_dev, int64_t S, const double* w_host, const double* hi_host,
                   const double* inv_range_host, const double* best_dev, const uint8_t* alive_dev, double* scores_dev);

int bbh_qnehvi_cells(bbh_handle* h, int32_t m, int64_t N, const double* const* tmat_dev, const double* const* var_dev,
                     const double* sign_host, const double* zx_host, int64_t S, const uint8_t* alive_dev, double* scores_dev);
int bbh_qnehvi_sm(bbh_handle* h, int32_t m, int64_t N, const double* const* tmat_dev, const double* const* var_dev,
                  const double* sign_host, const double* zx_host, int64_t S, const int64_t* cell_off_host, const double* cell_lo_host,
                  const double* cell_loglen_host, const uint8_t* alive_dev, double* scores_dev);

int bbh_cells_create(const double* obj_host, int64_t S, int64_t n, int32_t m, const double* ref_host,
                     void** cells_out, int64_t* total_out);
int bbh_cells_get(void* cells, int64_t* off_host, double* lo_host, double* loglen_host);
int bbh_cells_destroy(void* cells);

int bbh_sobol_scramble(int64_t* state, const int64_t* ltm, int64_t dim);
int bbh_sobol_draw(const int64_t* state, const int64_t* shift, int64_t n, int64_t dim, double* out);
int bbh_sobol_normal(const int64_t* state0, uint64_t seed, int64_t n, int64_t dim, double* out_host);
int bbh_sobol_normal_dev(bbh_handle* h, const int64_t* state0, uint64_t seed, int64_t n, int64_t dim, double* out_dev);

uint64_t bbh_content_key(const void* const* bufs, const int64_t* lens, int32_t nbuf, int32_t threads);

int bbh_argmax(bbh_handle* h, const double* scores_dev, int64_t N, double* best_val_host,
               int64_t* best_idx_host);
int bbh_topk(bbh_handle* h, const double* scores_dev, int64_t N, int64_t k, double* vals_host,
             int64_t* idx_host);

int bbh_fps_prepare(bbh_handle* h, const double* X_dev, int64_t N, int32_t d, int64_t ldx, const double* mean_host,
                    const double* scale_host, const int64_t* order_dev, int64_t M, double* P_dev, int64_t ldp);
int bbh_fps_farthest_pair(bbh_handle* h, const double* P_dev, int64_t M, int32_t d, int64_t ldp, const uint8_t* alive_dev,
                          double* d2_host, int64_t* a_host, int64_t* b_host);
int bbh_fps_greedy(bbh_handle* h, const double* P_dev, int64_t M, int32_t d, int64_t ldp, const uint8_t* alive_dev,
                   const int64_t* start_ranks_host, int64_t n_start, int64_t n_picks, int64_t k, int64_t* ranks_host,
                   double* d2_host, int64_t* count_host);

int bbh_set_slice_rows(bbh_handle* h, int64_t rows);

int bbh_trim(bbh_handle* h, int64_t keep_bytes);

int bbh_comm_unique_id(void* id_out, int64_t bytes);
int bbh_comm_init(bbh_handle* h, int32_t rank, int32_t world, const void* unique_id, int64_t bytes);
int bbh_comm_destroy(bbh_handle* h);
int bbh_allgather_topk(bbh_handle* h, const double* scores_dev, int64_t N, int64_t row_offset, int64_t k,
                       double* vals_host, int64_t* idx_host);
int bbh_allgather_argmax(bbh_handle* h, const double* scores_dev, int64_t N, int64_t row_offset, const double* X_dev,
                         int64_t ldx, double* val_host, int64_t* gidx_host, double* row_host);

int bbh_timing_enable(bbh_handle* h, int enable);
int bbh_timing_read(bbh_handle* h, double* fused_ms_total, int64_t* fused_launches, int reset);
int bbh_last_posterior_form(bbh_handle* h);
int bbh_last_nei_form(bbh_handle* h);
enum bbh_fit_form {
  BBH_FIT_FORM_LAUNCH = 0,
  BBH_FIT_FORM_SMALL = 1,
  BBH_FIT_FORM_TILES_MT = 2,
  BBH_FIT_FORM_TILES_MT_PARTIAL = 3,
  BBH_FIT_FORM_TILES = 4,
  BBH_FIT_FORM_GRAM_TILES = 5,
  BBH_FIT_FORM_ONE_LAUNCH = 6,
  BBH_FIT_FORM_SPLIT = 7,
  BBH_FIT_FORM_RFF = 8,
  BBH_FIT_FORM_STEPS_TAIL = 9
};
int bbh_last_fit_form(bbh_handle* h);
enum bbh_timed_family {
  BBH_TIMED_POSTERIOR = 0, BBH_TIMED_CROSS = 1, BBH_TIMED_PENDING = 2,
  BBH_TIMED_COLUMNS = 3,
  BBH_TIMED_NEHVI = 4,
  BBH_TIMED_Q1 = 5,
  BBH_TIMED_SELECT = 6,
  BBH_TIMED_FAMILIES = 7
};
int bbh_timing_read_family(bbh_handle* h, int32_t family, double* ms_total, int64_t* launches, int reset);

int bbh_flow_trace_read(bbh_handle* h, long long* stamps_host, int* roles_host, int cap);
int bbh_tiles_trace_read(bbh_handle* h, long long* stamps_host, int cap);

#ifdef __cplusplus
}
#endif
#endif
```

Before: 208.8 million candidates/s.

## Seed cooperative posterior distance GEMM with precomputed train norms and prescaled candidates

Adds a seeded variant of the cooperative posterior kernel for Matern-5/2. Train points are packed on the host with sqrt(5)-scaled, -2-multiplied fragments plus a per-point squared-norm vector. The distance MFMA accumulator then starts from (train norm + candidate norm) instead of carrying the 1 and norm columns in the K dimension, which can lower the fragment count (kds < kd). Candidates are prescaled by sqrt(5) so the kernel can skip the 5*r2 multiply. The exp range reduction also switches to a magic-constant rounding trick instead of rint plus an int cast. The cost is extra LDS for the norm vector, more kernel instantiations, and a host repack of the training data at model setup.

```diff
diff --git a/baybe_amd/_lib.py b/baybe_amd/_lib.py
--- a/baybe_amd/_lib.py
+++ b/baybe_amd/_lib.py
@@ -209,6 +209,7 @@
         [C.c_void_p, C.c_void_p, C.c_int64, C.c_int64, C.c_void_p, C.c_int64, c_double_p, c_int64_p, c_double_p],
     ),
     "bbh_last_posterior_form": (C.c_int, [C.c_void_p]),
+    "bbh_last_posterior_seeded": (C.c_int, [C.c_void_p]),
     "bbh_last_nei_form": (C.c_int, [C.c_void_p]),
     "bbh_last_fit_form": (C.c_int, [C.c_void_p]),
     "bbh_timing_enable": (C.c_int, [C.c_void_p, C.c_int]),
diff --git a/baybe_amd/csrc/bbh_api.hip b/baybe_amd/csrc/bbh_api.hip
--- a/baybe_amd/csrc/bbh_api.hip
+++ b/baybe_amd/csrc/bbh_api.hip
@@ -29,6 +29,7 @@
       {"BBH_KV_LDS", INT, 0, nullptr, &S::kv_lds_blocks},
       {"BBH_COOP", INT, 0, nullptr, &S::coop_mode},
       {"BBH_COOP_SMALL", NOT, '0', &S::coop_small, nullptr},
+      {"BBH_COOP_SEED", NOT, '0', &S::coop_seed, nullptr},
       {"BBH_COOPG_CROSS", NOT, '0', &S::coopg_cross_on, nullptr},
       {"BBH_SMALL", NOT, '0', &S::small_on, nullptr},
       {"BBH_SMALL_FORCE", IS, '1', &S::small_force, nullptr},
@@ -313,6 +314,7 @@
 }
 
 extern "C" int bbh_last_posterior_form(bbh_handle* h) { return h ? h->last_form : -1; }
+extern "C" int bbh_last_posterior_seeded(bbh_handle* h) { return h ? (h->last_form == 1 && h->last_seeded) : -1; }
 extern "C" int bbh_last_fit_form(bbh_handle* h) { return h ? h->last_fit_form : -1; }
 
 extern "C" int bbh_timing_enable(bbh_handle* h, int enable) {
diff --git a/baybe_amd/csrc/bbh_common.h b/baybe_amd/csrc/bbh_common.h
--- a/baybe_amd/csrc/bbh_common.h
+++ b/baybe_amd/csrc/bbh_common.h
@@ -167,6 +167,7 @@
   int kv_global_mode = -1;
   int kv_lds_blocks = -1;
   int coop_mode = 1;
+  bool coop_seed = true;
   bool coop_small = true;
   bool coopg_cross_on = true;
   bool small_on = true;
@@ -303,6 +304,10 @@
   double* d_rstream = nullptr;
   int64_t rstream_frags = 0;
   int coop_g0 = 0;
+  int coop_kds = 0;
+  double* d_trainfrag_s = nullptr;
+  int64_t tf_s_elems = 0;
+  int last_seeded = 0;
   int last_form = -1;
   int last_fit_form = -1;
   int last_nei_form = -1;
diff --git a/baybe_amd/csrc/bbh_coop.h b/baybe_amd/csrc/bbh_coop.h
--- a/baybe_amd/csrc/bbh_coop.h
+++ b/baybe_amd/csrc/bbh_coop.h
@@ -54,6 +54,7 @@
   const double* rstream;
   int64_t frags;
   int g0;
+  const double* na = nullptr;
 };
 
 __host__ __device__ constexpr int coop_frags_before(int G) { return 16 * (G * BBH_COOP_ROUNDS - (G * (G - 1)) / 2); }
@@ -61,7 +62,9 @@
 template <int G, int KD, int KVF, bool PRODUCE, int NT, bool OPEN = false>
 __device__ __forceinline__ void coop_group(const WaveCtx (&c)[NT], const double* rs, const double* tfn, const bbh_lds_double* kv_cur,
                                            bbh_lds_double* kv_mine_next, const bbh_lds_double* alpha_next, int tbn, int cw,
-                                           d4 (&acc)[NT][BBH_COOP_ROUNDS], d2 (&ring)[BBH_COOP_PAIRS], double (&accm)[NT]) {
+                                           d4 (&acc)[NT][BBH_COOP_ROUNDS], d2 (&ring)[BBH_COOP_PAIRS], double (&accm)[NT],
+                                           const bbh_lds_double* na_next = (const bbh_lds_double*)nullptr) {
+  constexpr bool SEED = (KVF & 8) != 0;
   constexpr int NP = BBH_COOP_PAIRS;
   constexpr int CNT = BBH_COOP_ROUNDS - G;
   constexpr int FULL = CNT - 1;
@@ -73,7 +76,11 @@
   double tfv[KD];
   d4 dsa[NT], dsb[NT];
   KvState<BBH_KV_NU> P;
-  double kv[NT][4], kvx[NT][4], kvn[NT][4], alv[4];
+  double kv[NT][4], kvx[NT][4], kvn[NT][4], alv[4], nav[4];
+  if constexpr (PRODUCE && SEED) {
+#pragma unroll
+    for (int r = 0; r < 4; r++) nav[r] = na_next[4 * r];
+  }
   if constexpr (PRODUCE) {
     static_for<0, KD>([&](auto kc) __attribute__((always_inline)) {
       constexpr int k = decltype(kc)::value;
@@ -144,7 +151,12 @@
         if constexpr (!BBH_COOP_ABLATE_KV) {
           static_for<0, NT>([&](auto tc_) __attribute__((always_inline)) {
             constexpr int t = decltype(tc_)::value;
-            kvp_dist<KD>(c[t], tfv, dsa[t], dsb[t]);
+            if constexpr (SEED) {
+              const d4 seed = {nav[0] + c[t].nbn, nav[1] + c[t].nbn, nav[2] + c[t].nbn, nav[3] + c[t].nbn};
+              kvp_dist_seeded<KD>(c[t], tfv, seed, dsa[t], dsb[t]);
+            } else {
+              kvp_dist<KD>(c[t], tfv, dsa[t], dsb[t]);
+            }
           });
         }
       }
@@ -172,10 +184,13 @@
 __global__ __launch_bounds__(256, (GMIN >= 6 ? 5 : GMIN >= 4 ? 4 : BBH_COOP_WAVES)) void bbh_coop_posterior_kernel(const CoopArgs ca) {
   const FusedArgs& a = ca.f;
   extern __shared__ __attribute__((aligned(16))) double s_mem[];
+  constexpr bool SEED = (KVF & 8) != 0;
+  static_assert(!SEED || (KVF & 6) == 0, "the seeded stream carries the Matern-5/2 constant");
   const int l = threadIdx.x & 63, w = __builtin_amdgcn_readfirstlane(threadIdx.x >> 6);
   const int cnd = l & 15, q = l >> 4;
   double* s_alpha = s_mem;
-  double* s_kv = s_alpha + 16 * a.nb;
+  double* s_na = s_alpha + 16 * a.nb;
+  double* s_kv = s_na + (SEED ? 16 * a.nb : 0);
   double* s_red = s_kv + NT * BBH_COOP_KV_TILE;
   const int64_t tile0 = (int64_t)blockIdx.x * (16 * NT);
 
@@ -186,6 +201,11 @@
   const double* xr[NT];
   double tfv0[KD];
   kvp_load<KD>(a.trainfrag + l, w, tfv0);
+  double na0[4];
+  if constexpr (SEED) {
+#pragma unroll
+    for (int r = 0; r < 4; r++) na0[r] = ca.na[16 * w + 4 * r + q];
+  }
 #pragma unroll
   for (int t = 0; t < NT; t++) {
     const int64_t row = (tile0 + 16 * t + cnd < a.N) ? tile0 + 16 * t + cnd : a.N - 1;
@@ -208,6 +228,8 @@
   }
   if (!(BBH_COOP_ABLATE_PRO & 1))
     for (int s = threadIdx.x; s < 16 * a.nb; s += 256) s_alpha[s] = a.meanB[(int64_t)s * 16];
+  if constexpr (SEED)
+    for (int s = threadIdx.x; s < 16 * a.nb; s += 256) s_na[s] = ca.na[s];
 #pragma unroll
   for (int t = 0; t < NT; t++) {
     double nbsum = 0.0;
@@ -217,17 +239,21 @@
       double v = 0.0;
       if (dim < a.dn) {
         v = (BBH_COOP_ABLATE_PRO & 2) ? 0.01 * (double)(dim + cnd) : fma(xval[t][k], xscl[k], xofs[k]);
+        if constexpr (SEED) v *= BBH_SQRT5;
         nbsum = fma(v, v, nbsum);
       }
       c[t].cf[k] = v;
     }
     nbsum += __shfl_xor(nbsum, 16, 64);
     nbsum += __shfl_xor(nbsum, 32, 64);
-#pragma unroll
-    for (int k = 0; k < KD; k++) {
-      if (4 * k + q == a.dn) c[t].cf[k] = 1.0;
-      if (4 * k + q == a.dn + 1) c[t].cf[k] = nbsum;
-    }
+    if constexpr (!SEED) {
+#pragma unroll
+      for (int k = 0; k < KD; k++) {
+        if (4 * k + q == a.dn) c[t].cf[k] = 1.0;
+        if (4 * k + q == a.dn + 1) c[t].cf[k] = nbsum;
+      }
+    }
+    c[t].nbn = nbsum;
     int tc = 0;
     if constexpr ((KVF & 1) != 0) {
       if (a.task_col >= 0) {
@@ -257,6 +283,7 @@
 
   bbh_lds_double* kvb = (bbh_lds_double*)(s_kv + l);
   const bbh_lds_double* alq = (const bbh_lds_double*)(s_alpha + q);
+  const bbh_lds_double* naq = (const bbh_lds_double*)(s_na + q);
   const int g0 = ca.g0;
   double accm[NT];
   d4 acc[NT][BBH_COOP_ROUNDS];
@@ -283,7 +310,12 @@
 #pragma unroll
       for (int t = 0; t < NT; t++) {
         d4 dsa, dsb;
-        kvp_dist<KD>(c[t], tfv, dsa, dsb);
+        if constexpr (SEED) {
+          const d4 seed = {na0[0] + c[t].nbn, na0[1] + c[t].nbn, na0[2] + c[t].nbn, na0[3] + c[t].nbn};
+          kvp_dist_seeded<KD>(c[t], tfv, seed, dsa, dsb);
+        } else {
+          kvp_dist<KD>(c[t], tfv, dsa, dsb);
+        }
         kv_all<KVF>(c[t], w, dsa, dsb, kv0[t]);
       }
     }
@@ -305,7 +337,7 @@
       const int tbn = 4 * (G + 1 - g0) + w;
       constexpr bool PRODUCE = G + 1 < BBH_COOP_ROUNDS;
       coop_group<G, KD, KVF, PRODUCE, NT>(c, rs, a.trainfrag + (int64_t)tbn * KD * 64, kvb + (G & 1) * 4 * 256,
-                                          kvb + (((G + 1) & 1) * 4 + w) * 256, alq + 16 * tbn, tbn, cw, acc, ring, accm);
+                                          kvb + (((G + 1) & 1) * 4 + w) * 256, alq + 16 * tbn, tbn, cw, acc, ring, accm, naq + 16 * tbn);
       rs += (int64_t)16 * (BBH_COOP_ROUNDS - G) * 64;
 #if !BBH_COOP_ABLATE_BARRIER
       if constexpr (PRODUCE) __syncthreads();
@@ -380,6 +412,8 @@
 bool bbh_coop_launch_a(int kd, int kind, bool has_tbl, dim3 grid, size_t lds, hipStream_t s, const CoopArgs& a);
 bool bbh_coop_launch_b(int kd, int kind, bool has_tbl, dim3 grid, size_t lds, hipStream_t s, const CoopArgs& a);
 bool bbh_coop_launch_small(int kd, int kind, bool has_tbl, dim3 grid, size_t lds, hipStream_t s, const CoopArgs& a);
+bool bbh_coop_seed_launch(int kds, bool has_tbl, dim3 grid, size_t lds, hipStream_t s, const CoopArgs& a, bool small_ok);
+bool bbh_coop_seed_launch_small(int kds, bool has_tbl, dim3 grid, size_t lds, hipStream_t s, const CoopArgs& a);
 
 #define BBH_COOP_DISPATCH_KD(KDV, NTV)                                                                                        \
   if (kd == KDV) {                                                                                                       \
diff --git a/baybe_amd/csrc/bbh_fused.h b/baybe_amd/csrc/bbh_fused.h
--- a/baybe_amd/csrc/bbh_fused.h
+++ b/baybe_amd/csrc/bbh_fused.h
@@ -68,6 +68,7 @@
   int nl, ncache;
   const bbh_lds_double* al;
   int kd, kind, T, tc, q, l, dn;
+  double nbn;
   double cf[16];
 };
 
@@ -247,6 +248,18 @@
 #endif
 }
 
+template <int KD>
+__device__ __forceinline__ void kvp_dist_seeded(const WaveCtx& c, const double (&tfv)[KD], const d4& seed, d4& da, d4& db) {
+  static_assert(BBH_CANDREG && !BBH_DIST_ASM, "the seeded distance GEMM reads the candidate fragments from registers");
+  da = seed;
+  db = (d4){0.0, 0.0, 0.0, 0.0};
+#pragma unroll
+  for (int k = 0; k < KD; k += 2) {
+    da = mfma_f64(tfv[k], c.cf[k], da);
+    if (k + 1 < KD) db = mfma_f64(tfv[k + 1], c.cf[k + 1], db);
+  }
+}
+
 #define BBH_KV_STEPS 18
 #ifndef BBH_KV_SQRT_NR
 #define BBH_KV_SQRT_NR 1
@@ -273,6 +286,8 @@
 __device__ __forceinline__ void kv_micro(KvState<NU>& P, const WaveCtx& c, int tb, int r0, const d4& da, const d4& db,
                                          double (&out)[4]) {
   constexpr bool HAS_TBL = (KVF & 1) != 0, RBFK = (KVF & 2) != 0;
+  constexpr bool PRESCALED = (KVF & 8) != 0;
+  constexpr double RND = 6755399441055744.0;
   constexpr bool M32K = (KVF & 4) != 0;
   constexpr double KC1 = M32K ? 3.0 : 5.0, KC2 = M32K ? 0.0 : 1.0 / 3.0;
   constexpr double LOG2E = 1.4426950408889634074, LN2_HI = 6.93147180369123816490e-01,
@@ -289,7 +304,7 @@
         if (RBFK)
           P.g[u] = __builtin_fmin(__builtin_fmax(0.5 * r2, 0.0), 800.0);
         else
-          P.t[u] = __builtin_fmax(KC1 * r2, 1e-300);
+          P.t[u] = __builtin_fmax(PRESCALED ? r2 : KC1 * r2, 1e-300);
         if (HAS_TBL) P.te[u] = c.taskext[16 * tb + 4 * (r0 + u) + c.q];
       }
       break;
@@ -348,26 +363,26 @@
 #endif
     case 7:
 #pragma unroll
-      BBH_KV_EACH P.kf[u] = __builtin_rint(P.g[u] * -LOG2E);
+      BBH_KV_EACH P.y[u] = fma(P.g[u], -LOG2E, RND);
       if (!RBFK) {
 #pragma unroll
         BBH_KV_EACH P.q[u] = M32K ? 1.0 : fma(P.g[u], KC2, 1.0);
+#pragma unroll
+        BBH_KV_EACH P.q[u] = fma(P.q[u], P.g[u], 1.0);
       }
       break;
     case 8:
 #pragma unroll
+      BBH_KV_EACH P.kf[u] = P.y[u] - RND;
+#pragma unroll
       BBH_KV_EACH P.t[u] = fma(P.kf[u], -LN2_HI, -P.g[u]);
-      if (!RBFK) {
-#pragma unroll
-        BBH_KV_EACH P.q[u] = fma(P.q[u], P.g[u], 1.0);
-      }
+#pragma unroll
+      BBH_KV_EACH P.t[u] = fma(P.kf[u], -LN2_LO, P.t[u]);
       break;
     case 9:
 #pragma unroll
-      BBH_KV_EACH P.t[u] = fma(P.kf[u], -LN2_LO, P.t[u]);
-#pragma unroll
       BBH_KV_EACH {
-        P.ki[u] = (int)P.kf[u];
+        P.ki[u] = __double2loint(P.y[u]);
         if (HAS_TBL) P.tv[u] = c.tbl[c.tc * c.T + P.te[u]];
       }
       break;
diff --git a/baybe_amd/csrc/bbh_fused_coop_c.hip b/baybe_amd/csrc/bbh_fused_coop_c.hip
--- /dev/null
+++ b/baybe_amd/csrc/bbh_fused_coop_c.hip
@@ -0,0 +1,24 @@
+#include "bbh_coop.h"
+
+#define BBH_COOP_SEED_KD(KDV)                                                                \
+  if (kds == KDV) {                                                                          \
+    if (grid.x == 0) return true;                                                            \
+    if (has_tbl)                                                                             \
+      hipLaunchKernelGGL((bbh_coop_posterior_kernel<KDV, 9, 1>), grid, dim3(256), lds, s, a); \
+    else                                                                                     \
+      hipLaunchKernelGGL((bbh_coop_posterior_kernel<KDV, 8, 1>), grid, dim3(256), lds, s, a); \
+    return true;                                                                             \
+  }
+
+bool bbh_coop_seed_launch(int kds, bool has_tbl, dim3 grid, size_t lds, hipStream_t s, const CoopArgs& a, bool small_ok) {
+  if (grid.x != 0 && a.g0 >= 4 && small_ok && bbh_coop_seed_launch_small(kds, has_tbl, grid, lds, s, a)) return true;
+  BBH_COOP_SEED_KD(2)
+  BBH_COOP_SEED_KD(3)
+  BBH_COOP_SEED_KD(4)
+  BBH_COOP_SEED_KD(5)
+  BBH_COOP_SEED_KD(6)
+  BBH_COOP_SEED_KD(7)
+  BBH_COOP_SEED_KD(8)
+  BBH_COOP_SEED_KD(12)
+  return false;
+}
diff --git a/baybe_amd/csrc/bbh_fused_coop_s.hip b/baybe_amd/csrc/bbh_fused_coop_s.hip
--- a/baybe_amd/csrc/bbh_fused_coop_s.hip
+++ b/baybe_amd/csrc/bbh_fused_coop_s.hip
@@ -1,13 +1,21 @@
 #include "bbh_coop.h"
 
-#define BBH_COOP_SMALL_KD(KDV)                                                                              \
+#define BBH_COOP_SMALL_KD_SEL(KDV, SIXV)                                                                    \
   if (kd == KDV) {                                                                                          \
     if (grid.x == 0) return true;                                                                           \
-    if (a.g0 >= 6 && has_tbl)                                                                 \
-      hipLaunchKernelGGL((bbh_coop_posterior_kernel<KDV, 1, 1, 6>), grid, dim3(256), lds, s, a);             \
-    else if (a.g0 >= 6)                                                                                     \
-      hipLaunchKernelGGL((bbh_coop_posterior_kernel<KDV, 0, 1, 6>), grid, dim3(256), lds, s, a);             \
-    else if (has_tbl)                                                                                       \
+    if constexpr (SIXV == 2) {                                                                              \
+      if (a.g0 >= 6 && has_tbl) {                                                                           \
+        hipLaunchKernelGGL((bbh_coop_posterior_kernel<KDV, 1, 1, (SIXV == 2 ? 6 : 4)>), grid, dim3(256), lds, s, a); \
+        return true;                                                                                        \
+      }                                                                                                     \
+    }                                                                                                       \
+    if constexpr (SIXV >= 1) {                                                                              \
+      if (a.g0 >= 6 && !has_tbl) {                                                                          \
+        hipLaunchKernelGGL((bbh_coop_posterior_kernel<KDV, 0, 1, (SIXV >= 1 ? 6 : 4)>), grid, dim3(256), lds, s, a); \
+        return true;                                                                                        \
+      }                                                                                                     \
+    }                                                                                                       \
+    if (has_tbl)                                                                                            \
       hipLaunchKernelGGL((bbh_coop_posterior_kernel<KDV, 1, 1, 4>), grid, dim3(256), lds, s, a);             \
     else                                                                                                    \
       hipLaunchKernelGGL((bbh_coop_posterior_kernel<KDV, 0, 1, 4>), grid, dim3(256), lds, s, a);             \
@@ -16,9 +24,42 @@
 
 bool bbh_coop_launch_small(int kd, int kind, bool has_tbl, dim3 grid, size_t lds, hipStream_t s, const CoopArgs& a) {
   if (kind != BBH_KERNEL_MATERN52) return false;
-  BBH_COOP_SMALL_KD(2)
-  BBH_COOP_SMALL_KD(4)
-  BBH_COOP_SMALL_KD(6)
-  BBH_COOP_SMALL_KD(8)
+  BBH_COOP_SMALL_KD_SEL(2, 2)
+  BBH_COOP_SMALL_KD_SEL(4, 2)
+  BBH_COOP_SMALL_KD_SEL(6, 1)
+  BBH_COOP_SMALL_KD_SEL(8, 0)
   return false;
 }
+
+#define BBH_COOP_SMALL_SEED_KD(KDV)                                                                         \
+  if (kds == KDV) {                                                                                         \
+    if (grid.x == 0) return true;                                                                           \
+    if (a.g0 >= 6 && has_tbl)                                                                 \
+      hipLaunchKernelGGL((bbh_coop_posterior_kernel<KDV, 9, 1, 6>), grid, dim3(256), lds, s, a);             \
+    else if (a.g0 >= 6)                                                                                     \
+      hipLaunchKernelGGL((bbh_coop_posterior_kernel<KDV, 8, 1, 6>), grid, dim3(256), lds, s, a);             \
+    else if (has_tbl)                                                                                       \
+      hipLaunchKernelGGL((bbh_coop_posterior_kernel<KDV, 9, 1, 4>), grid, dim3(256), lds, s, a);             \
+    else                                                                                                    \
+      hipLaunchKernelGGL((bbh_coop_posterior_kernel<KDV, 8, 1, 4>), grid, dim3(256), lds, s, a);             \
+    return true;                                                                                            \
+  }
+#define BBH_COOP_SMALL_SEED_KD4(KDV)                                                                        \
+  if (kds == KDV) {                                                                                         \
+    if (a.g0 >= 6) return false;                                                                            \
+    if (grid.x == 0) return true;                                                                           \
+    if (has_tbl)                                                                                            \
+      hipLaunchKernelGGL((bbh_coop_posterior_kernel<KDV, 9, 1, 4>), grid, dim3(256), lds, s, a);             \
+    else                                                                                                    \
+      hipLaunchKernelGGL((bbh_coop_posterior_kernel<KDV, 8, 1, 4>), grid, dim3(256), lds, s, a);             \
+    return true;                                                                                            \
+  }
+
+bool bbh_coop_seed_launch_small(int kds, bool has_tbl, dim3 grid, size_t lds, hipStream_t s, const CoopArgs& a) {
+  BBH_COOP_SMALL_SEED_KD(2)
+  BBH_COOP_SMALL_SEED_KD(3)
+  BBH_COOP_SMALL_SEED_KD4(4)
+  BBH_COOP_SMALL_SEED_KD4(5)
+  BBH_COOP_SMALL_SEED_KD4(6)
+  return false;
+}
diff --git a/baybe_amd/csrc/bbh_model.hip b/baybe_amd/csrc/bbh_model.hip
--- a/baybe_amd/csrc/bbh_model.hip
+++ b/baybe_amd/csrc/bbh_model.hip
@@ -348,6 +348,7 @@
 static void bbh_reset_model_state(bbh_handle* h) {
   h->coopg_ready = false;
   h->coop_ready = false;
+  h->coop_kds = 0;
   h->coop2_ready = false;
   h->small_nb = 0;
   if (h->fit_exec) hipGraphExecDestroy(h->fit_exec);
@@ -362,7 +363,7 @@
   void* ptrs[] = {h->d_xnT,   h->d_task,    h->d_ystd,      h->d_theta, h->d_K,     h->d_X,       h->d_M,
                   h->d_Q,     h->d_Q2,      h->d_D,         h->d_tmp,   h->d_r,     h->d_t,       h->d_alpha,
                   h->d_u,     h->d_w,       h->d_q,         h->d_partial, h->d_out, h->d_info,    h->d_trainfrag,
-                  h->d_rfrag, h->d_meanB,   h->d_sclofs,    h->d_numcol, h->d_tasktbl, h->d_taskext, h->d_beta, h->d_pass_off, h->d_pass_w, h->d_nmask, h->d_colfrag, h->d_pendT, h->d_colA, h->d_Mpart, h->d_trainfrag_f, h->d_sclofs_f};
+                  h->d_rfrag, h->d_meanB,   h->d_sclofs,    h->d_numcol, h->d_tasktbl, h->d_taskext, h->d_beta, h->d_pass_off, h->d_pass_w, h->d_nmask, h->d_colfrag, h->d_pendT, h->d_colA, h->d_Mpart, h->d_trainfrag_f, h->d_sclofs_f, h->d_trainfrag_s};
   for (void* p : ptrs)
     if (p) hipFree(p);
   bbh_rff_destroy(h);
@@ -374,6 +375,9 @@
   h->d_nmask = nullptr;
   h->d_pendT = h->d_colA = h->d_Mpart = nullptr;
   h->d_trainfrag_f = h->d_sclofs_f = nullptr;
+  h->d_trainfrag_s = nullptr;
+  h->tf_s_elems = 0;
+  h->coop_kds = 0;
   h->tf_f_elems = 0;
   h->coopg_ready = false;
   h->colA_elems = 0;
diff --git a/baybe_amd/csrc/bbh_panel.hip b/baybe_amd/csrc/bbh_panel.hip
--- a/baybe_amd/csrc/bbh_panel.hip
+++ b/baybe_amd/csrc/bbh_panel.hip
@@ -140,6 +140,43 @@
           out[((size_t)(tb - tb0) * kd + k) * 64 + qq * 16 + c16] = v;
         }
     }
+}
+
+static void host_pack_trainfrag_seeded(const bbh_handle* h, const double* pts, int64_t cnt, int64_t nb, int kds, std::vector<double>& out) {
+  const int dn = h->dn;
+  const double* ls = h->theta.data() + 3;
+  out.assign((size_t)nb * kds * 64 + (size_t)16 * nb, 0.0);
+  double* na = out.data() + (size_t)nb * kds * 64;
+  std::vector<double> a(dn);
+  for (int64_t tb = 0; tb < nb; tb++)
+    for (int c16 = 0; c16 < 16; c16++) {
+      const int64_t i = tb * 16 + c16;
+      if (i >= cnt) {
+        na[i] = 5e8;
+        continue;
+      }
+      double sum = 0.0;
+      for (int j = 0; j < dn; j++) {
+        a[j] = BBH_SQRT5 * ((pts[i * dn + j] - h->xcenter[j]) / ls[j]);
+        sum += a[j] * a[j];
+      }
+      na[i] = sum;
+      for (int dim = 0; dim < dn; dim++) out[((size_t)tb * kds + dim / 4) * 64 + (dim % 4) * 16 + c16] = -2.0 * a[dim];
+    }
+}
+
+static int bbh_coop_seed_kds(const bbh_handle* h, bool has_tbl, int g0) {
+  if (!h->sw.coop_seed || h->desc.kernel_kind != BBH_KERNEL_MATERN52) return 0;
+  int kds = (h->dn + 3) / 4;
+  kds = kds <= 8 ? (kds < 2 ? 2 : kds) : 12;
+  if (kds >= h->kd || 4 * kds < h->dn) return 0;
+  CoopArgs ask{};
+  ask.g0 = g0;
+  if (g0 >= 4 && h->sw.coop_small) {
+    if (bbh_coop_seed_launch_small(kds, has_tbl, dim3(0), 0, nullptr, ask)) return kds;
+    if (bbh_coop_launch_small(h->kd, h->desc.kernel_kind, has_tbl, dim3(0), 0, nullptr, ask)) return 0;
+  }
+  return bbh_coop_seed_launch(kds, has_tbl, dim3(0), 0, nullptr, ask, false) ? kds : 0;
 }
 
 static int bbh_coopg_kd(const bbh_handle* h) {
@@ -320,6 +357,19 @@
                          h->d_rstream);
       h->coop_g0 = g0;
       h->coop_ready = true;
+      h->coop_kds = bbh_coop_seed_kds(h, has_tbl0, g0);
+      if (h->coop_kds) {
+        std::vector<double> tfs;
+        host_pack_trainfrag_seeded(h, h->xn_host.data(), h->n, nb, h->coop_kds, tfs);
+        if (!h->d_trainfrag_s || h->tf_s_elems != (int64_t)tfs.size()) {
+          if (h->d_trainfrag_s) hipFree(h->d_trainfrag_s);
+          h->d_trainfrag_s = nullptr;
+          BBH_HIP_TRY(h, hipMalloc((void**)&h->d_trainfrag_s, sizeof(double) * tfs.size()));
+          h->tf_s_elems = (int64_t)tfs.size();
+        }
+        BBH_HIP_TRY(h, hipMemcpyAsync(h->d_trainfrag_s, tfs.data(), sizeof(double) * tfs.size(), hipMemcpyHostToDevice, s));
+        BBH_HIP_TRY(h, hipStreamSynchronize(s));
+      }
     }
   }
   h->coopg_ready = false;
@@ -581,9 +631,21 @@
     ca.rstream = h->d_rstream;
     ca.frags = h->rstream_frags;
     ca.g0 = h->coop_g0;
-    const size_t clds = sizeof(double) * (16 * (size_t)h->nb + (2 * 4 * 256 + 128));
+    ca.na = nullptr;
     const dim3 cgrid((unsigned)((N + 15) / 16));
-    bbh_coop_launch(kdc, a.kind, has_tbl, cgrid, clds, h->stream, ca, h->sw.coop_small);
+    h->last_seeded = h->coop_kds > 0;
+    if (h->coop_kds) {
+      ca.f.trainfrag = h->d_trainfrag_s;
+      ca.na = h->d_trainfrag_s + (size_t)h->nb * h->coop_kds * 64;
+      const size_t clds = sizeof(double) * (32 * (size_t)h->nb + (2 * 4 * 256 + 128));
+      if (!bbh_coop_seed_launch(h->coop_kds, has_tbl, cgrid, clds, h->stream, ca, h->sw.coop_small)) {
+        h->err = "cooperative posterior form: no seeded instantiation for this model although its operands were packed";
+        return -6;
+      }
+    } else {
+      const size_t clds = sizeof(double) * (16 * (size_t)h->nb + (2 * 4 * 256 + 128));
+      bbh_coop_launch(kdc, a.kind, has_tbl, cgrid, clds, h->stream, ca, h->sw.coop_small);
+    }
     h->last_form = 1;
     BBH_HIP_TRY(h, hipGetLastError());
     return 0;
diff --git a/baybe_amd/engine.py b/baybe_amd/engine.py
--- a/baybe_amd/engine.py
+++ b/baybe_amd/engine.py
@@ -924,6 +924,9 @@
     def posterior_kernel_form(self) -> str:
         return {0: "windowed", 1: "cooperative", 2: "materialised", 3: "cooperative-2sweep", 4: "cooperative-generic",
                 5: "register-resident", 6: "feature-space"}.get(self._lib.bbh_last_posterior_form(self._h), "none")
+
+    def posterior_distance_seeded(self) -> bool:
+        return self._lib.bbh_last_posterior_seeded(self._h) == 1
 
     def fit_evaluation_form(self) -> str:
         return {0: "launch", 1: "small", 2: "tiles+mt", 3: "tiles+mt-partial", 4: "tiles", 5: "gram+tiles", 6: "one-launch",
diff --git a/include/baybe_hip.h b/include/baybe_hip.h
--- a/include/baybe_hip.h
+++ b/include/baybe_hip.h
@@ -233,6 +233,7 @@
 int bbh_timing_enable(bbh_handle* h, int enable);
 int bbh_timing_read(bbh_handle* h, double* fused_ms_total, int64_t* fused_launches, int reset);
 int bbh_last_posterior_form(bbh_handle* h);
+int bbh_last_posterior_seeded(bbh_handle* h);
 int bbh_last_nei_form(bbh_handle* h);
 enum bbh_fit_form {
   BBH_FIT_FORM_LAUNCH = 0,
```

Measured after the change: 212.0 million candidates/s, median of 6. +1.5%, better.
